# gabeur/mmt

Measured on AMD Instinct MI355X. Metric: video-text pairs/sec (fwd+bwd+Adam), MSRVTT 7-expert d512 L4, higher is better.
Workload: dtype bf16; 1 GPU; configs[1]: MSRVTT jsfusion shape, 7 experts x 30 tokens, d512, L4, H4, I3072, batch 32/GPU, dropout 0.1, train mode, Adam; text tower replaced by synthetic (B,768) vectors; global_batch=32, seq_len=218, parallelism=dp1, hip_graphs=True, inputs=resident in HBM, input_slots=8, input_format=dense fp32 dict, text_tower=synthetic, grad_sync=single, grad_wire_dtype=fp32, grad_algo=allreduce, comm_log=False, collectives_captured=False, dense_rows=6976, full=False

## Files before the change

### include/mmt_hip.h

```cpp
#ifndef MMT_HIP_H_
#define MMT_HIP_H_
#include <stdint.h>

#ifdef __cplusplus
extern "C" {
#endif

#define MMT_ABI_VERSION 6
#define MMT_ROW_ALIGN 256

#define MMT_ERR_ARG (-1)
#define MMT_ERR_ALIGN (-2)

int mmt_abi_version(void);
const char* mmt_build_info(void);

enum {
  MMT_EPI_BF16 = 0,
  MMT_EPI_BIAS_BF16 = 1,
  MMT_EPI_BIAS_GELU = 2,
  MMT_EPI_BIAS_DROP_RES = 3,
  MMT_EPI_DGELU = 4,
  MMT_EPI_ADD_F32 = 5,
  MMT_EPI_F32 = 6,
// ... 95 lines not shown
                           uint32_t drop_key, uint32_t thr16, float drop_scale, const uint32_t* seed_dev,
                           const int32_t* sched_cu, int sched_B, int sched_H, int sched_tiles, int32_t* sched_work,
                           void* stream);
int mmt_ln_fwd_scatter(const float* z, const float* gamma, const float* beta, float eps, float* h32,
                       const int32_t* dst_rows, void* h16, float* mean, float* rstd, int rows, int d, void* stream);
int mmt_rows_gather(const float* src, const int32_t* rows, int n, int d, float* dst, const int32_t* idx_in,
                    int32_t* idx_out, void* stream);
int mmt_rows_scatter(const float* src, const int32_t* rows, int n, int d, float* dst, int accumulate, void* stream);
int mmt_table_grad_direct(const float* g, const int32_t* ids, int rows, int d, int vocab, const int32_t* n_rows_dev,
                          float* dtable, void* stream);
int mmt_embedding_grad(const float* g, const int32_t* ids, int n, int d, int vocab, int padding_idx,
                       const int32_t* n_rows_dev, float* dtable, void* stream);
int mmt_text_plan(const int64_t* input_ids, const int64_t* token_type_ids, const int64_t* position_ids,
                  const int64_t* attention_mask, int B, int W, int32_t* counts, int32_t* cu_seqlens, int32_t* n_rows_dev,
                  int32_t* ids, int32_t* types, int32_t* pos, int32_t* row_index, int32_t* cls_rows, void* stream);
int mmt_gemm_splitk_geometry(int M, int N, int K, int splits_requested, int* splits, int64_t* slab_stride);
int mmt_splitk_ln_fwd(const float* slabs, int splits, int64_t slab_stride, const float* bias, const float* res,
                      const int32_t* res_rows, const int32_t* rowidx, const int32_t* row_index, int32_t* rowidx_out,
                      uint32_t drop_key, uint32_t thr16, float drop_scale, const uint32_t* seed_dev, float* z_out,
                      const float* gamma, const float* beta, float eps, float* h32, void* h16, float* mean, float* rstd,
                      int rows, int d, void* stream);
int mmt_ln_bwd_slabs(const float* slabs, int splits, int64_t slab_stride, const float* res, const float* z,
                     const float* mean, const float* rstd, const float* gamma, float* dz, void* dy, float* partials,
                     int rows, int d, int drop_mode, const int32_t* row_index, uint32_t drop_key, uint32_t thr16,
                     float drop_scale, const uint32_t* seed_dev, void* stream);
int mmt_splitk_ln_fwd_ex(const float* slabs, int splits, int64_t slab_stride, const float* bias, const float* res,
                         const int32_t* res_rows, const int32_t* rowidx, const int32_t* row_index, int32_t* rowidx_out,
                         uint32_t drop_key, uint32_t thr16, float drop_scale, const uint32_t* seed_dev, float* z_out,
                         const float* gamma, const float* beta, float eps, float* h32, void* h16, float* mean, float* rstd,
                         int rows, int d, const int32_t* n_rows_dev, void* stream);
int mmt_ln_bwd_slabs_ex(const float* slabs, int splits, int64_t slab_stride, const float* res, const float* z,
                        const float* mean, const float* rstd, const float* gamma, float* dz, void* dy, float* partials,
                        int rows, int d, int drop_mode, const int32_t* n_rows_dev, const int32_t* row_index,
                        uint32_t drop_key, uint32_t thr16, float drop_scale, const uint32_t* seed_dev, void* stream);

int mmt_ln_bwd_rows_per_block(int rows);
int mmt_ln_bwd(const float* dout, const float* z, const float* mean, const float* rstd, const float* gamma,
               float* dz, void* dy, float* partials, int rows, int d, int drop_mode,
               const int32_t* n_rows_dev, const int32_t* row_index, uint32_t drop_key, uint32_t thr16,
               float drop_scale, const uint32_t* seed_dev, void* stream);
int mmt_col_reduce(const float* partials, int nblocks, int nvec, int d, float* out0, float* out1,
                   float* out2, float* out3, int accumulate, void* stream);
#define MMT_COLRED_MAX 32
typedef struct MmtColReduceJob {
  const float* partials;
  float* out[4];
  int32_t nblocks, nvec, nout, d;
} MmtColReduceJob;
int mmt_col_reduce_multi(const MmtColReduceJob* jobs, int n, void* stream);
int64_t mmt_table_grad_scratch_floats(int vocab, int d);
int mmt_table_grad(const float* g, const int32_t* ids, int rows, int d, int vocab,
                   const int32_t* n_rows_dev, float* scratch, float* dtable, int accumulate, void* stream);
int mmt_table_grad_partials(const float* g, const int32_t* ids, int rows, int d, int vocab,
                            const int32_t* n_rows_dev, float* scratch, void* stream);
int mmt_table_grad_partials_pair(const float* g, const int32_t* ids0, int vocab0, float* scratch0, const int32_t* ids1,
                                 int vocab1, float* scratch1, int rows, int d, const int32_t* n_rows_dev, void* stream);
int mmt_table_grad_chunks(void);
int mmt_colsum_bf16(const void* x, int64_t ld, int rows, int cols, const int32_t* n_rows_dev,
                    float* partials, void* stream);

int mmt_attn_fwd(const void* qkv, const int32_t* cu_seqlens, const float* mask_bias, void* ctx, float* lse,
                 int B, int S, int H, int d, float scale, uint32_t drop_key, uint32_t thr16,
                 float drop_scale, const uint32_t* seed_dev,
                 const int32_t* row_index, void* stream);
int mmt_attn_bwd_ex(const void* qkv, const int32_t* cu_seqlens, const float* mask_bias, const void* ctx,
                    const float* lse, const void* dctx, void* dqkv, float* delta, int delta_ready, int B, int S, int H,
                    int d, float scale, uint32_t drop_key, uint32_t thr16, float drop_scale,
                    const uint32_t* seed_dev, const int32_t* row_index, const int32_t* work, void* stream);
int64_t mmt_attn_schedule_words(int B, int S, int H);
int mmt_attn_schedule(const int32_t* cu_seqlens, int B, int S, int H, int32_t* work, void* stream);
int mmt_attn_bwd(const void* qkv, const int32_t* cu_seqlens, const float* mask_bias, const void* ctx,
                 const float* lse, const void* dctx, void* dqkv, float* delta, int B, int S, int H, int d,
                 float scale, uint32_t drop_key, uint32_t thr16, float drop_scale,
                 const uint32_t* seed_dev,
                 const int32_t* row_index, void* stream);
int mmt_attn_fwd_rows(const void* qkv, const int32_t* cu_seqlens, const float* mask_bias, const int32_t* qsel, int nq,
                      void* ctx, float* lse, int B, int S, int H, int d, float scale, uint32_t drop_key, uint32_t thr16,
                      float drop_scale, const uint32_t* seed_dev,
                 const int32_t* row_index, void* stream);
int mmt_attn_bwd_rows_ex(const void* qkv, const int32_t* cu_seqlens, const float* mask_bias, const int32_t* qsel, int nq,
                         const void* ctx, const float* lse, const void* dctx, void* dqkv, float* delta, int delta_ready,
                         int B, int S, int H, int d, float scale, uint32_t drop_key, uint32_t thr16, float drop_scale,
                         const uint32_t* seed_dev, const int32_t* row_index, void* stream);
int mmt_attn_bwd_rows(const void* qkv, const int32_t* cu_seqlens, const float* mask_bias, const int32_t* qsel, int nq,
                      const void* ctx, const float* lse, const void* dctx, void* dqkv, float* delta, int B, int S, int H,
                      int d, float scale, uint32_t drop_key, uint32_t thr16, float drop_scale,
                      const uint32_t* seed_dev,
                 const int32_t* row_index, void* stream);
int mmt_attn_dropout_mask(uint8_t* out, int B, int H, int S, uint32_t drop_key, uint32_t thr16,
                          const uint32_t* seed_dev, void* stream);

#define MMT_PACK_MAX 24
typedef struct MmtPackItem {
  const float* src;
  void* dst;
  void* dst_t;
  int32_t rows, cols, dst_ld, dst_t_ld, dst_t_rows, reserved;
} MmtPackItem;
int mmt_pack_weights(const MmtPackItem* items, int n, void* stream);
int mmt_adam_step(float* params, const float* grads, float* exp_avg, float* exp_avg_sq, int64_t count,
                  float lr, float beta1, float beta2, float eps, float weight_decay,
                  const int32_t* step_dev, const float* lr_dev, void* stream);

#define MMT_ADAM_SEG_MAX 160
typedef struct MmtAdamSeg {
  int64_t offset, count;
  void* dst;
  void* dst_t;
  int32_t rows, cols, dst_ld, dst_t_ld;
} MmtAdamSeg;
int mmt_adam_fused_blocks(const MmtAdamSeg* seg);
int mmt_adam_step_fused(float* params, const float* grads, float* exp_avg, float* exp_avg_sq,
                        const MmtAdamSeg* segs_host, const MmtAdamSeg* segs_dev, int n_segs, float lr, float beta1,
                        float beta2, float eps, float weight_decay, int32_t* step_dev, const float* lr_dev,
                        int bump_step, void* stream);

#define MMT_MAX_EXPERTS 16
typedef struct MmtExpertIO {
  const float* feat;
  const float* maxpool;
  const float* ind;
  const float* t;
  void* x;
  float* y;
  void* dy;
  int32_t D, Dpad, type_idx, rows_pad;
  const float* y_part[2];
  int32_t n_part, reserved;
} MmtExpertIO;
typedef struct MmtVideoSrc {
  int32_t* src_row;
  int32_t* src_cnt;
  int32_t* xsrc;
} MmtVideoSrc;
int mmt_video_plan(const MmtExpertIO* experts, int M, int B, int T, int pack, int max_pos, int32_t* counts,
                   int32_t* cu_seqlens, int32_t* n_rows_dev, int32_t* slot, int32_t* row_index, int32_t* type_ids,
                   int32_t* pos_ids, float* mask_bias, int32_t* agg_row, uint32_t* seed_bump, const MmtVideoSrc* src,
                   void* stream);
int mmt_video_cast(const MmtExpertIO* experts, int M, int B, int T, const MmtVideoSrc* src, void* stream);
int mmt_video_scatter(const MmtExpertIO* experts, int M, int B, int T, int d, const int32_t* n_rows_dev,
                      const int32_t* row_index, const MmtVideoSrc* src, float* features, void* stream);
int mmt_video_scatter_bwd(const MmtExpertIO* experts, int M, int B, int T, int d, const int32_t* n_rows_dev,
                          const int32_t* row_index, const MmtVideoSrc* src, const float* dfeatures, void* stream);

int mmt_readout_fwd(const float* last_hidden, const int32_t* agg_row, int BM, int d, float* vid_embds,
                    float* inv_norm, void* stream);
int mmt_readout_bwd(const float* vid_embds, const float* inv_norm, const float* dvid_embds,
                    const int32_t* agg_row, int BM, int d, float* dlast_hidden, void* stream);
int mmt_sims_fwd(const float* txt, const float* vid, const float* tw, const float* vw, int NT, int NV, int M,
                 int d, float* sims, float* dots, void* stream);
int mmt_sims_bwd(const float* txt, const float* vid, const float* tw, const float* vw, float* dots,
                 const float* dsims, int NT, int NV, int M, int d, float* dtxt, float* dvid, float* dtw,
                 float* dvw, void* stream);
int mmt_simloss_small_max_n(void);
int mmt_simloss_bwd_small(const float* txt, const float* vid, const float* tw, const float* vw, const float* sims,
                          const float* dots, int n, int M, int d, int kind, float margin, int fix_norm, float* loss,
                          float* dtxt, float* dvid, float* dtw, float* dvw, const float* inv_norm,
                          const int32_t* out_rows, float* dlast, void* stream);

int mmt_maxmargin(const float* sims, int n, float margin, int fix_norm, float* partial, float* loss,
                  float* grad, void* stream);
int mmt_infonce(const float* sims, int n, float* scratch, float* loss, float* grad, void* stream);

int64_t mmt_sims_eval_workspace_floats(int NT, int NV, int M, int d);
int mmt_sims_eval(const float* txt, const float* vid, const float* tw, const float* vw, int NT, int NV, int M, int d,
                  float* ws, float* sims, void* stream);
int mmt_retrieval_ranks(const float* sims, const uint8_t* qmask, int NQ, int NV, float* t2v_rank, float* v2t_rank,
                        float* scratch, void* stream);

int mmt_search_fold(const float* x, const float* w, int N, int M, int d, float* out, void* stream);
int mmt_search_fold_bf16(const float* x, const float* w, int N, int M, int d, uint16_t* out, void* stream);
int mmt_search_fold_split_bf16(const float* x, const float* w, int N, int M, int d, uint16_t* hi, uint16_t* lo,
                               void* stream);
int mmt_search_fold_fp8(const float* x, const float* w, int N, int M, int d, uint8_t* out, float* scale, void* stream);
int mmt_rows_topk(const float* sims, int64_t ld, const int32_t* rows, int NR, int NV, int k, uint64_t* ws, float* scores,
                  int64_t* index, void* stream);

#define MMT_SEARCH_FP32 0
#define MMT_SEARCH_BF16 1
#define MMT_SEARCH_FP8 2
#define MMT_SEARCH_SETS_NONE 0
#define MMT_SEARCH_SETS_QUERY 1
#define MMT_SEARCH_SETS_ITEM 2
typedef struct MmtSearchScan {
  const void* q;
  const void* q_lo;
  const float* qw;
  const void* g;
  const float* gw;
  const float* gscale;
  const uint32_t* subset;
  const int64_t* exclude;
  const uint64_t* after;
  const float* lse;
  const float* set_weights;
  int32_t storage;
  int32_t NQ;
  int32_t NV;
  int32_t M;
  int32_t d;
  int32_t E;
  float beta;
  int32_t sets;
  int32_t set_size;
  int32_t mode;
} MmtSearchScan;
#ifdef __cplusplus
static_assert(sizeof(MmtSearchScan) == 128, "MmtSearchScan: 11 pointers, then 10 four-byte fields");
#else
_Static_assert(sizeof(MmtSearchScan) == 128, "MmtSearchScan: 11 pointers, then 10 four-byte fields");
#endif

int64_t mmt_topk_workspace_keys(int NQ, int NV, int k);
int64_t mmt_rank_workspace_ints(int NQ, int NV, int T);
int64_t mmt_count_workspace_ints(int NQ, int NV, int T);
int64_t mmt_range_workspace_ints(int NQ, int NV);
int64_t mmt_col_lse_workspace_floats(int NB, int NV);
int64_t mmt_rescore_workspace_keys(int NQ, int C);
int64_t mmt_topk_pooled_workspace_keys(int NS, int C, int NV, int k);
int64_t mmt_count_pooled_workspace_ints(int NS, int C, int NV, int T);
int64_t mmt_topk_itemsets_workspace_keys(int NQ, int NT, int C, int k);
int64_t mmt_count_itemsets_workspace_ints(int NQ, int NT, int C, int T);
int mmt_search_topk(const MmtSearchScan* scan, int k, uint64_t* ws, float* scores, int64_t* index, void* stream);
int mmt_search_topk_groups(const MmtSearchScan* scan, int k, const int32_t* group_ids, uint64_t* ws, float* scores,
                           int64_t* groups, int64_t* items, void* stream);
int mmt_search_rank(const MmtSearchScan* scan, const int64_t* targets, int T, int32_t* ws, int32_t* greater,
                    int32_t* equal, void* stream);
int mmt_search_thresholds(const MmtSearchScan* scan, const int64_t* targets, int T, float* thr, void* stream);
int mmt_search_count(const MmtSearchScan* scan, const float* thr, int T, int32_t* ws, int32_t* greater, int32_t* equal,
                     void* stream);
int mmt_search_range_count(const MmtSearchScan* scan, const float* thr, int32_t* ws, int64_t* row_counts, void* stream);
int mmt_search_range_fill(const MmtSearchScan* scan, const float* thr, const int32_t* ws, const int64_t* offsets,
                          int64_t* indices, float* scores, void* stream);
int mmt_search_rescore(const MmtSearchScan* scan, const int64_t* candidates, int C, int k, uint64_t* ws, float* scores,
                       int64_t* index, void* stream);
int mmt_search_col_lse(const MmtSearchScan* scan, float beta, float* ws, float* state, int first, float* lse,
                       void* stream);

#define MMT_SEARCH_MAX_RK 32
int64_t mmt_col_topk_workspace_keys(int NB, int NV, int k);
int mmt_search_col_topk(const MmtSearchScan* scan, int k, int row0, uint64_t* ws, uint64_t* state, int first,
                        float* scores, int64_t* rows, float* mean, float mean_weight, void* stream);

#define MMT_SEARCH_MAX_DC 128
int mmt_search_pair_scores(const void* g, const float* gw, const float* gscale, int storage, int NV, int M, int d,
                           const int64_t* items, int R, int C, float* sims, void* stream);
int mmt_search_mmr(const int64_t* items, const float* rel, const float* sims, int R, int C, int k, float a, float b,
                   float* scores, int64_t* index, float* values, void* stream);

int64_t mmt_self_topk_workspace_keys(int R, int NV, int k);
int64_t mmt_self_range_workspace_ints(int R, int NV);
int mmt_search_self_topk(const void* a_rows, const float* a_weights, const float* a_scales, int NA, const int64_t* items,
                         const int64_t* self, int R, const void* g, const float* gw, const float* gscale, int NV,
                         const uint32_t* subset, int storage, int M, int d, int k, uint64_t* ws, float* scores,
                         int64_t* index, void* stream);
int mmt_search_self_range_count(const void* a_rows, const float* a_weights, const float* a_scales, int NA,
                                const int64_t* items, const int64_t* self, int R, const void* g, const float* gw,
                                const float* gscale, int NV, const uint32_t* subset, int storage, int M, int d,
                                const float* thr, int32_t* ws, int64_t* row_counts, void* stream);
int mmt_search_self_range_fill(const void* a_rows, const float* a_weights, const float* a_scales, int NA,
                               const int64_t* items, const int64_t* self, int R, const void* g, const float* gw,
                               const float* gscale, int NV, const uint32_t* subset, int storage, int M, int d,
                               const float* thr, const int32_t* ws, const int64_t* offsets, int64_t* indices, float* scores,
                               void* stream);

int64_t mmt_row_expsum_workspace_ints64(int NQ, int NV);
int mmt_search_row_expsum(const MmtSearchScan* scan, float beta, const float* xmax, int F, int64_t* ws, void* stream);

int mmt_search_subset_pack(const uint8_t* mask, int NV, uint32_t* words, void* stream);
int mmt_search_after_keys(const float* scores, const int64_t* first, int NQ, uint64_t* keys, void* stream);
int mmt_search_merge_lists(const float* scores, const int64_t* index, const int64_t* const* ids, int S, int NQ, int kin,
                           int kout, float* out_scores, int64_t* out_index, void* stream);
int mmt_search_merge_group_lists(const float* scores, const int64_t* groups, const int64_t* index, const int64_t* const* ids,
                                 int S, int NQ, int kin, int kout, float* out_scores, int64_t* out_groups, int64_t* out_items,
                                 void* stream);

int mmt_ls_fold_bf16(const float* x, const float* w, int R, int Rpad, int M, int d, void* out16, void* stream);
int mmt_transpose_bf16(const void* src, int64_t ld_src, int rows, int cols, void* dst, int64_t ld_dst, void* stream);
int mmt_ls_finish(float* S, int64_t ld, const float* tw, const float* vw, int b, int n, int M, void* stream);
int mmt_ls_col_blocks(int n);
int mmt_ls_diag(const float* S, int64_t ld, const float* tw, const float* vw, int b, int n, int M, int r0, float* diag_local,
                void* stream);
int mmt_ls_counts_ex(float* S, int64_t ld, const float* diag, const float* tw, const float* vw, const float* vw_t, int M, int finish, int b, int n,
                     int r0, float margin, int32_t* rowcnt, int32_t* colcnt, float* loss_part, void* stream);
int mmt_ls_counts(const float* S, int64_t ld, const float* diag, int b, int n, int r0, float margin, int32_t* rowcnt,
                  int32_t* colcnt, float* loss_part, void* stream);
int mmt_ls_grad(const float* S, int64_t ld, const float* diag, const float* tw, const float* vw, const int32_t* rowcnt,
                const int32_t* colcnt_total, int b, int n, int M, int r0, float margin, float inv_norm, void* G16,
                int64_t ldg, float* gs_part, void* stream);
int mmt_ls_grad_ex(const float* S, int64_t ld, const float* diag, const float* tw, const float* vw, const float* vw_t, const int32_t* rowcnt,
                   const int32_t* colcnt_total, int b, int n, int M, int r0, float margin, float inv_norm, void* G16,
                   int64_t ldg, float* gs_part, int raw, void* stream);
int mmt_ls_unfold(const float* P, int64_t ldp, const float* x, const float* w, const float* gsub, int R, int M, int d,
                  float* dx, float* dw, void* stream);

int mmt_ls_nce_col_blocks(int n);
int mmt_ls_nce_row_groups(int b);
int mmt_ls_nce_stats(const float* S, int64_t ld, const float* tw, const float* vw, const float* vw_t, int b, int n, int M, int r0,
                     float scale, float* row_part, float* col_part, void* stream);
int mmt_ls_nce_grad(const float* S, int64_t ld, const float* tw, const float* vw, const float* vw_t, const float* row_lse,
                    const float* col_lse, int b, int n, int M, int r0, float scale, float inv_n, void* G16, int64_t ldg,
                    float* gs_part, void* stream);

typedef struct MmtSgemm {
  const float* A[MMT_MAX_EXPERTS];
  const float* B[MMT_MAX_EXPERTS];
  float* C[MMT_MAX_EXPERTS];
  const float* bias[MMT_MAX_EXPERTS];
  int64_t sai, sak, sbj, sbk, ldc;
  int32_t batch, M, N, K;
  float beta;
  int32_t reserved;
} MmtSgemm;
int mmt_sgemm_batched(const MmtSgemm* g, void* stream);

typedef struct MmtTextHeads {
  const float *w1[MMT_MAX_EXPERTS], *b1[MMT_MAX_EXPERTS];
  const float *w2[MMT_MAX_EXPERTS], *b2[MMT_MAX_EXPERTS];
  const float *bn_gamma[MMT_MAX_EXPERTS], *bn_beta[MMT_MAX_EXPERTS];
  float *running_mean[MMT_MAX_EXPERTS], *running_var[MMT_MAX_EXPERTS];
  const float *moe_w[MMT_MAX_EXPERTS], *moe_b[MMT_MAX_EXPERTS];
  float *g_w1[MMT_MAX_EXPERTS], *g_b1[MMT_MAX_EXPERTS], *g_w2[MMT_MAX_EXPERTS], *g_b2[MMT_MAX_EXPERTS];
  float *g_bn_gamma[MMT_MAX_EXPERTS], *g_bn_beta[MMT_MAX_EXPERTS], *g_moe_w[MMT_MAX_EXPERTS], *g_moe_b[MMT_MAX_EXPERTS];
} MmtTextHeads;
int64_t mmt_text_heads_workspace_floats(int N, int M, int d);
typedef struct MmtVideoFront {
  const MmtExpertIO* experts;
  int32_t M, B, T, pack, max_pos, do_cast;
  int32_t *counts, *cu_seqlens, *n_rows_dev, *slot, *row_index, *type_ids, *pos_ids;
  float* mask_bias;
  int32_t* agg_row;
  uint32_t* seed_bump;
  const MmtVideoSrc* src;
} MmtVideoFront;
typedef struct MmtTextHeadsOpts {
  uint32_t moe_drop_key, moe_drop_thr16;
  float moe_drop_scale;
  int32_t reserved;
  const uint32_t* seed_dev;
  uint32_t* key_dev;
  int64_t* num_batches_tracked;
  const MmtVideoFront* video_front;
} MmtTextHeadsOpts;
int mmt_text_heads_fast(int N, int M, int d, int K);
int mmt_text_heads_fwd(const MmtTextHeads* h, const float* text, const float* text_moe, int N, int C, int M, int d,
                       int K, int use_bn, int training, float* ws, float* text_embds, float* text_weights,
                       const MmtTextHeadsOpts* opts, void* stream);
int mmt_text_heads_bwd(const MmtTextHeads* h, const float* text, const float* text_moe, const float* w1_all, int N,
                       int C, int M, int d, int K, int use_bn, int training, float* ws, const float* dtext_embds,
                       const float* text_weights, const float* dtext_weights, float* dtext, float* dtext_moe,
                       const MmtTextHeadsOpts* opts, void* stream);

typedef struct MmtBertLayer {
  const void *wqkv, *wqkv_t, *wo, *wo_t, *w1, *w1_t, *w2, *w2_t;
  const float *bqkv, *bo, *ln1_g, *ln1_b, *b1, *b2, *ln2_g, *ln2_b;
  float *g_wqkv, *g_bqkv, *g_wo, *g_bo, *g_ln1_g, *g_ln1_b, *g_w1, *g_b1, *g_w2, *g_b2, *g_ln2_g, *g_ln2_b;
} MmtBertLayer;

typedef struct MmtBertModel {
  int32_t hidden, layers, heads, inter, max_pos, type_vocab;
  float ln_eps, p_hidden, p_attn;
  int32_t reserved;
  const float *pos_emb, *type_emb, *emb_ln_g, *emb_ln_b;
  float *g_pos_emb, *g_type_emb, *g_emb_ln_g, *g_emb_ln_b;
  const MmtBertLayer* layer;
} MmtBertModel;

typedef struct MmtBertBatch {
  const float* features;
  const int32_t* type_ids;
  const int32_t* pos_ids;
  const float* mask_bias;
  const int32_t* cu_seqlens;
  const int32_t* row_index;
  const int32_t* n_rows_dev;
  const uint32_t* seed_dev;
  int32_t rows, rows_alloc, batch, seq;
  const int32_t* out_rows;
  int32_t n_out_per_sample;
  int32_t fork;
  void* side_stream;
  int32_t live_rows_hint;
} MmtBertBatch;

enum {
  MMT_FORK_WGRAD = 1,
  MMT_FORK_EARLY = 2,
  MMT_FORK_REDUCE = 4,
  MMT_FORK_JOIN = 8,
  MMT_RANGE_LAYERS_ONLY = 16
};

int mmt_stream_fork(void* from, void* to);

int64_t mmt_bert_workspace_bytes(const MmtBertModel* m, int rows_alloc);
int mmt_bert_tail_capacity(int rows_alloc);
int mmt_bert_forward(const MmtBertModel* m, const MmtBertBatch* b, void* ws, float* out_last, int training,
                     void* stream);
int mmt_bert_backward(const MmtBertModel* m, const MmtBertBatch* b, void* ws, float* dlast, float* dfeatures,
                      int training, void* stream);
int mmt_bert_backward_range(const MmtBertModel* m, const MmtBertBatch* b, void* ws, float* dlast, float* dfeatures,
                            int training, int l_hi, int l_lo, void* stream);

int mmt_probe_arm(void** start_events, void** stop_events, int n);
int mmt_probe_arm_site(int site, void** start_events, void** stop_events, int n);
int mmt_probe_count_site(int site);
int mmt_dropout_f32(const float* x, float* y, int64_t n, uint32_t drop_key, uint32_t thr16, float scale,
                    const uint32_t* seed_dev, uint32_t* key_save, const uint32_t* key_load, void* stream);
int mmt_debug_dispatch_probe(int blocks, int threads, int lds_bytes, int spin, float* sink, void* stream);
int mmt_probe_count(void);

#ifdef __cplusplus
}
#endif
#endif
```

### mmt_amd/_lib.py

```python
import ctypes
import os

_HERE = os.path.dirname(os.path.abspath(__file__))
LIB_PATH = os.environ.get('MMT_HIP_LIB') or os.path.join(_HERE, 'lib', 'libmmt_hip.so')

c_int, c_i64, c_u32, c_f32, c_vp = ctypes.c_int, ctypes.c_int64, ctypes.c_uint32, ctypes.c_float, ctypes.c_void_p


class MmtEpilogue(ctypes.Structure):
  _fields_ = [('bias', c_vp), ('res', c_vp), ('ldres', c_i64), ('out2', c_vp), ('ldout2', c_i64),
              ('aux', c_vp), ('ldaux', c_i64), ('colsum', c_vp), ('row_index', c_vp), ('seed_dev', c_vp),
              ('drop_key', c_u32), ('drop_thr16', c_u32), ('drop_scale', c_f32), ('reserved', ctypes.c_int32),
              ('dot_src', c_vp), ('lddot', c_i64), ('dot_out', c_vp), ('live_rows_hint', ctypes.c_int32)]


class MmtPackItem(ctypes.Structure):
  _fields_ = [('src', c_vp), ('dst', c_vp), ('dst_t', c_vp), ('rows', ctypes.c_int32), ('cols', ctypes.c_int32),
              ('dst_ld', ctypes.c_int32), ('dst_t_ld', ctypes.c_int32), ('dst_t_rows', ctypes.c_int32),
              ('reserved', ctypes.c_int32)]


class MmtAdamSeg(ctypes.Structure):
  _fields_ = [('offset', c_i64), ('count', c_i64), ('dst', c_vp), ('dst_t', c_vp), ('rows', ctypes.c_int32),
              ('cols', ctypes.c_int32), ('dst_ld', ctypes.c_int32), ('dst_t_ld', ctypes.c_int32)]


class MmtGemmItem(ctypes.Structure):
  _fields_ = [('A', c_vp), ('B', c_vp), ('C', c_vp), ('bias', c_vp), ('lda', c_i64), ('ldb', c_i64), ('ldc', c_i64),
              ('M', ctypes.c_int32), ('N', ctypes.c_int32), ('K', ctypes.c_int32), ('tile_begin', ctypes.c_int32),
              ('n_rows_dev', c_vp)]


class MmtWgradItem(ctypes.Structure):
  _fields_ = [('A', c_vp), ('B', c_vp), ('out', c_vp), ('bias_out', c_vp), ('lda', c_i64), ('ldb', c_i64), ('ldo', c_i64),
              ('N', ctypes.c_int32), ('K2', ctypes.c_int32), ('N_out', ctypes.c_int32), ('K2_out', ctypes.c_int32),
              ('tile_begin', ctypes.c_int32), ('reserved', ctypes.c_int32), ('slab', c_vp), ('bias_slab', c_vp),
              ('splits', ctypes.c_int32), ('reserved2', ctypes.c_int32), ('n_rows_dev', c_vp)]


class MmtWgradGroup(ctypes.Structure):
  _fields_ = [('item', MmtWgradItem * 16), ('n_rows_dev', c_vp), ('count', ctypes.c_int32), ('rows', ctypes.c_int32)]


class MmtColReduceJob(ctypes.Structure):
  _fields_ = [('partials', c_vp), ('out', c_vp * 4), ('nblocks', ctypes.c_int32), ('nvec', ctypes.c_int32),
              ('nout', ctypes.c_int32), ('d', ctypes.c_int32)]


class MmtVideoSrc(ctypes.Structure):
  _fields_ = [('src_row', c_vp), ('src_cnt', c_vp), ('xsrc', c_vp)]


class MmtExpertIO(ctypes.Structure):
  _fields_ = [('feat', c_vp), ('maxpool', c_vp), ('ind', c_vp), ('t', c_vp), ('x', c_vp), ('y', c_vp), ('dy', c_vp),
              ('D', ctypes.c_int32), ('Dpad', ctypes.c_int32), ('type_idx', ctypes.c_int32),
              ('rows_pad', ctypes.c_int32), ('y_part', c_vp * 2), ('n_part', ctypes.c_int32),
              ('reserved', ctypes.c_int32)]


_LAYER_PTRS = ['wqkv', 'wqkv_t', 'wo', 'wo_t', 'w1', 'w1_t', 'w2', 'w2_t',
               'bqkv', 'bo', 'ln1_g', 'ln1_b', 'b1', 'b2', 'ln2_g', 'ln2_b',
               'g_wqkv', 'g_bqkv', 'g_wo', 'g_bo', 'g_ln1_g', 'g_ln1_b', 'g_w1', 'g_b1', 'g_w2', 'g_b2',
               'g_ln2_g', 'g_ln2_b']


class MmtBertLayer(ctypes.Structure):
  _fields_ = [(n, c_vp) for n in _LAYER_PTRS]


class MmtBertModel(ctypes.Structure):
  _fields_ = ([(n, ctypes.c_int32) for n in ('hidden', 'layers', 'heads', 'inter', 'max_pos', 'type_vocab')] +
              [(n, c_f32) for n in ('ln_eps', 'p_hidden', 'p_attn')] + [('reserved', ctypes.c_int32)] +
              [(n, c_vp) for n in ('pos_emb', 'type_emb', 'emb_ln_g', 'emb_ln_b', 'g_pos_emb', 'g_type_emb',
                                   'g_emb_ln_g', 'g_emb_ln_b')] +
              [('layer', ctypes.POINTER(MmtBertLayer))])


class MmtBertBatch(ctypes.Structure):
  _fields_ = ([(n, c_vp) for n in ('features', 'type_ids', 'pos_ids', 'mask_bias', 'cu_seqlens', 'row_index',
                                   'n_rows_dev', 'seed_dev')] +
              [(n, ctypes.c_int32) for n in ('rows', 'rows_alloc', 'batch', 'seq')] +
              [('out_rows', c_vp), ('n_out_per_sample', ctypes.c_int32), ('fork', ctypes.c_int32),
               ('side_stream', c_vp), ('live_rows_hint', ctypes.c_int32)])


FORK_WGRAD, FORK_EARLY, FORK_REDUCE, FORK_JOIN, RANGE_LAYERS_ONLY = 1, 2, 4, 8, 16


_PTR16 = c_vp * 16


class MmtSgemm(ctypes.Structure):
  _fields_ = [('A', _PTR16), ('B', _PTR16), ('C', _PTR16), ('bias', _PTR16),
              ('sai', c_i64), ('sak', c_i64), ('sbj', c_i64), ('sbk', c_i64), ('ldc', c_i64),
              ('batch', ctypes.c_int32), ('M', ctypes.c_int32), ('N', ctypes.c_int32), ('K', ctypes.c_int32),
              ('beta', c_f32), ('reserved', ctypes.c_int32)]


_TEXT_HEAD_FIELDS = ['w1', 'b1', 'w2', 'b2', 'bn_gamma', 'bn_beta', 'running_mean', 'running_var', 'moe_w', 'moe_b',
                     'g_w1', 'g_b1', 'g_w2', 'g_b2', 'g_bn_gamma', 'g_bn_beta', 'g_moe_w', 'g_moe_b']


class MmtTextHeads(ctypes.Structure):
  _fields_ = [(n, _PTR16) for n in _TEXT_HEAD_FIELDS]


class MmtVideoFront(ctypes.Structure):
  _fields_ = [('experts', c_vp), ('M', ctypes.c_int32), ('B', ctypes.c_int32), ('T', ctypes.c_int32), ('pack', ctypes.c_int32),
              ('max_pos', ctypes.c_int32), ('do_cast', ctypes.c_int32), ('counts', c_vp), ('cu_seqlens', c_vp),
              ('n_rows_dev', c_vp), ('slot', c_vp), ('row_index', c_vp), ('type_ids', c_vp), ('pos_ids', c_vp),
              ('mask_bias', c_vp), ('agg_row', c_vp), ('seed_bump', c_vp), ('src', c_vp)]


class MmtTextHeadsOpts(ctypes.Structure):
  _fields_ = [('moe_drop_key', c_u32), ('moe_drop_thr16', c_u32), ('moe_drop_scale', c_f32), ('reserved', ctypes.c_int32),
              ('seed_dev', c_vp), ('key_dev', c_vp), ('num_batches_tracked', c_vp), ('video_front', c_vp)]


class MmtSearchScan(ctypes.Structure):
  _fields_ = ([(n, c_vp) for n in ('q', 'q_lo', 'qw', 'g', 'gw', 'gscale', 'subset', 'exclude', 'after', 'lse',
                                   'set_weights')] +
              [(n, ctypes.c_int32) for n in ('storage', 'NQ', 'NV', 'M', 'd', 'E')] + [('beta', c_f32)] +
              [(n, ctypes.c_int32) for n in ('sets', 'set_size', 'mode')])


SEARCH_FP32, SEARCH_BF16, SEARCH_FP8 = 0, 1, 2
SEARCH_SETS_NONE, SEARCH_SETS_QUERY, SEARCH_SETS_ITEM = 0, 1, 2
_SCAN = ctypes.POINTER(MmtSearchScan)

EPI = dict(BF16=0, BIAS_BF16=1, BIAS_GELU=2, BIAS_DROP_RES=3, DGELU=4, ADD_F32=5, F32=6, BIAS_F32=7)

SIGNATURES = {
    'mmt_abi_version': (c_int, []),
    'mmt_build_info': (ctypes.c_char_p, []),
    'mmt_gemm_nt_bf16': (c_int, [c_vp, c_i64, c_vp, c_i64, c_vp, c_i64, c_int, c_int, c_int, c_int,
                                 ctypes.POINTER(MmtEpilogue), c_vp, c_vp]),
    'mmt_gemm_select_tile': (c_int, [c_int] * 9),
    'mmt_gemm_tn_bf16': (c_int, [c_vp, c_i64, c_vp, c_i64, c_vp, c_int, c_int, c_int, c_int, c_vp, c_vp]),
    'mmt_gemm_nt_splitk_workspace_floats': (c_i64, [c_int, c_int, c_int]),
    'mmt_gemm_nt_splitk': (c_int, [c_vp, c_i64, c_vp, c_i64, c_vp, c_i64, c_int, c_int, c_int, c_int,
                                   ctypes.POINTER(MmtEpilogue), c_vp, c_vp]),
    'mmt_gemm_nn_bf16': (c_int, [c_vp, c_i64, c_vp, c_i64, c_vp, c_i64, c_int, c_int, c_int, c_int,
                                 ctypes.POINTER(MmtEpilogue), c_vp, c_vp]),
    'mmt_gemm_nn_splitk_ex': (c_int, [c_vp, c_i64, c_vp, c_i64, c_vp, c_i64, c_int, c_int, c_int, c_int,
                                      ctypes.POINTER(MmtEpilogue), c_vp, c_int, c_int, c_vp, c_int, c_vp]),
    'mmt_gemm_nt_splitk_ex': (c_int, [c_vp, c_i64, c_vp, c_i64, c_vp, c_i64, c_int, c_int, c_int, c_int,
                                      ctypes.POINTER(MmtEpilogue), c_vp, c_int, c_int, c_vp, c_int, c_vp]),
    'mmt_gemm_nt_grouped': (c_int, [ctypes.POINTER(MmtGemmItem), c_int, c_int, c_vp]),
    'mmt_wgrad_grouped': (c_int, [ctypes.POINTER(MmtWgradGroup), c_vp]),
    'mmt_reduce_slabs': (c_int, [c_vp, c_int, c_i64, c_vp, c_int, c_vp]),
    'mmt_reduce_slabs_pair': (c_int, [c_vp, c_i64, c_vp, c_vp, c_i64, c_vp, c_int, c_vp]),
    'mmt_ln_fwd': (c_int, [c_vp, c_vp, c_vp, c_f32, c_vp, c_vp, c_vp, c_vp, c_int, c_int, c_vp, c_vp]),
    'mmt_embed_ln_fwd': (c_int, [c_vp, c_vp, c_vp, c_vp, c_vp, c_vp, c_vp, c_vp, c_f32, c_vp, c_vp, c_vp, c_vp,
                                 c_int, c_int, c_vp, c_vp, c_u32, c_u32, c_f32, c_vp, c_vp]),
    'mmt_embed_ln_fwd_sched': (c_int, [c_vp, c_vp, c_vp, c_vp, c_vp, c_vp, c_vp, c_vp, c_f32, c_vp, c_vp, c_vp, c_vp,
                                 c_int, c_int, c_vp, c_vp, c_u32, c_u32, c_f32, c_vp, c_vp, c_int, c_int, c_int, c_vp, c_vp]),
    'mmt_ln_bwd_rows_per_block': (c_int, [c_int]),
    'mmt_gemm_splitk_geometry': (c_int, [c_int, c_int, c_int, c_int, c_vp, c_vp]),
    'mmt_splitk_ln_fwd': (c_int, [c_vp, c_int, c_i64, c_vp, c_vp, c_vp, c_vp, c_vp, c_vp, c_u32, c_u32, c_f32, c_vp, c_vp, c_vp,
                                  c_vp, c_f32, c_vp, c_vp, c_vp, c_vp, c_int, c_int, c_vp]),
    'mmt_ln_bwd_slabs': (c_int, [c_vp, c_int, c_i64, c_vp, c_vp, c_vp, c_vp, c_vp, c_vp, c_vp, c_vp, c_int, c_int, c_int, c_vp,
                                 c_u32, c_u32, c_f32, c_vp, c_vp]),
    'mmt_splitk_ln_fwd_ex': (c_int, [c_vp, c_int, c_i64, c_vp, c_vp, c_vp, c_vp, c_vp, c_vp, c_u32, c_u32, c_f32, c_vp, c_vp, c_vp,
                                     c_vp, c_f32, c_vp, c_vp, c_vp, c_vp, c_int, c_int, c_vp, c_vp]),
    'mmt_ln_bwd_slabs_ex': (c_int, [c_vp, c_int, c_i64, c_vp, c_vp, c_vp, c_vp, c_vp, c_vp, c_vp, c_vp, c_int, c_int, c_int, c_vp,
                                    c_vp, c_u32, c_u32, c_f32, c_vp, c_vp]),
    'mmt_ln_bwd': (c_int, [c_vp, c_vp, c_vp, c_vp, c_vp, c_vp, c_vp, c_vp, c_int, c_int, c_int, c_vp, c_vp,
                           c_u32, c_u32, c_f32, c_vp, c_vp]),
    'mmt_col_reduce': (c_int, [c_vp, c_int, c_int, c_int, c_vp, c_vp, c_vp, c_vp, c_int, c_vp]),
    'mmt_col_reduce_multi': (c_int, [ctypes.POINTER(MmtColReduceJob), c_int, c_vp]),
    'mmt_table_grad_partials': (c_int, [c_vp, c_vp, c_int, c_int, c_int, c_vp, c_vp, c_vp]),
    'mmt_table_grad_chunks': (c_int, []),
    'mmt_table_grad_partials_pair': (c_int, [c_vp, c_vp, c_int, c_vp, c_vp, c_int, c_vp, c_int, c_int, c_vp, c_vp]),
    'mmt_table_grad_scratch_floats': (c_i64, [c_int, c_int]),
    'mmt_table_grad': (c_int, [c_vp, c_vp, c_int, c_int, c_int, c_vp, c_vp, c_vp, c_int, c_vp]),
    'mmt_attn_fwd': (c_int, [c_vp, c_vp, c_vp, c_vp, c_vp, c_int, c_int, c_int, c_int, c_f32, c_u32, c_u32,
                             c_f32, c_vp, c_vp, c_vp]),
    'mmt_attn_bwd': (c_int, [c_vp, c_vp, c_vp, c_vp, c_vp, c_vp, c_vp, c_vp, c_int, c_int, c_int, c_int, c_f32,
                             c_u32, c_u32, c_f32, c_vp, c_vp, c_vp]),
    'mmt_attn_bwd_ex': (c_int, [c_vp, c_vp, c_vp, c_vp, c_vp, c_vp, c_vp, c_vp, c_int, c_int, c_int, c_int, c_int, c_f32,
                                c_u32, c_u32, c_f32, c_vp, c_vp, c_vp, c_vp]),
    'mmt_attn_schedule_words': (c_i64, [c_int, c_int, c_int]),
    'mmt_attn_schedule': (c_int, [c_vp, c_int, c_int, c_int, c_vp, c_vp]),
    'mmt_attn_bwd_rows_ex': (c_int, [c_vp, c_vp, c_vp, c_vp, c_int, c_vp, c_vp, c_vp, c_vp, c_vp, c_int, c_int, c_int, c_int,
                                     c_int, c_f32, c_u32, c_u32, c_f32, c_vp, c_vp, c_vp]),
    'mmt_attn_fwd_rows': (c_int, [c_vp, c_vp, c_vp, c_vp, c_int, c_vp, c_vp, c_int, c_int, c_int, c_int, c_f32, c_u32, c_u32,
                                  c_f32, c_vp, c_vp, c_vp]),
    'mmt_attn_bwd_rows': (c_int, [c_vp, c_vp, c_vp, c_vp, c_int, c_vp, c_vp, c_vp, c_vp, c_vp, c_int, c_int, c_int, c_int,
                                  c_f32, c_u32, c_u32, c_f32, c_vp, c_vp, c_vp]),
    'mmt_ln_fwd_scatter': (c_int, [c_vp, c_vp, c_vp, c_f32, c_vp, c_vp, c_vp, c_vp, c_vp, c_int, c_int, c_vp]),
    'mmt_rows_gather': (c_int, [c_vp, c_vp, c_int, c_int, c_vp, c_vp, c_vp, c_vp]),
    'mmt_rows_scatter': (c_int, [c_vp, c_vp, c_int, c_int, c_vp, c_int, c_vp]),
    'mmt_embedding_grad': (c_int, [c_vp, c_vp, c_int, c_int, c_int, c_int, c_vp, c_vp, c_vp]),
    'mmt_text_plan': (c_int, [c_vp, c_vp, c_vp, c_vp, c_int, c_int, c_vp, c_vp, c_vp, c_vp, c_vp, c_vp, c_vp, c_vp, c_vp]),
    'mmt_table_grad_direct': (c_int, [c_vp, c_vp, c_int, c_int, c_int, c_vp, c_vp, c_vp]),
    'mmt_attn_dropout_mask': (c_int, [c_vp, c_int, c_int, c_int, c_u32, c_u32, c_vp, c_vp]),
    'mmt_reduce_slabs_2d': (c_int, [c_vp, c_int, c_int, c_int, c_int, c_vp, c_int, c_vp]),
    'mmt_colsum_bf16': (c_int, [c_vp, c_i64, c_int, c_int, c_vp, c_vp, c_vp]),
    'mmt_pack_weights': (c_int, [ctypes.POINTER(MmtPackItem), c_int, c_vp]),
    'mmt_dropout_f32': (c_int, [c_vp, c_vp, c_i64, c_u32, c_u32, c_f32, c_vp, c_vp, c_vp, c_vp]),
    'mmt_debug_dispatch_probe': (c_int, [c_int, c_int, c_int, c_int, c_vp, c_vp]),
    'mmt_adam_step': (c_int, [c_vp, c_vp, c_vp, c_vp, c_i64, c_f32, c_f32, c_f32, c_f32, c_f32, c_vp, c_vp, c_vp]),
    'mmt_adam_fused_blocks': (c_int, [ctypes.POINTER(MmtAdamSeg)]),
    'mmt_adam_step_fused': (c_int, [c_vp, c_vp, c_vp, c_vp, ctypes.POINTER(MmtAdamSeg), c_vp, c_int, c_f32, c_f32, c_f32,
                                    c_f32, c_f32, c_vp, c_vp, c_int, c_vp]),
    'mmt_video_plan': (c_int, [ctypes.POINTER(MmtExpertIO), c_int, c_int, c_int, c_int, c_int, c_vp, c_vp, c_vp, c_vp,
                               c_vp, c_vp, c_vp, c_vp, c_vp, c_vp, ctypes.POINTER(MmtVideoSrc), c_vp]),
    'mmt_video_cast': (c_int, [ctypes.POINTER(MmtExpertIO), c_int, c_int, c_int, ctypes.POINTER(MmtVideoSrc), c_vp]),
    'mmt_video_scatter': (c_int, [ctypes.POINTER(MmtExpertIO), c_int, c_int, c_int, c_int, c_vp, c_vp,
                                  ctypes.POINTER(MmtVideoSrc), c_vp, c_vp]),
    'mmt_video_scatter_bwd': (c_int, [ctypes.POINTER(MmtExpertIO), c_int, c_int, c_int, c_int, c_vp, c_vp,
                                      ctypes.POINTER(MmtVideoSrc), c_vp, c_vp]),
    'mmt_readout_fwd': (c_int, [c_vp, c_vp, c_int, c_int, c_vp, c_vp, c_vp]),
    'mmt_readout_bwd': (c_int, [c_vp, c_vp, c_vp, c_vp, c_int, c_int, c_vp, c_vp]),
    'mmt_sims_fwd': (c_int, [c_vp, c_vp, c_vp, c_vp, c_int, c_int, c_int, c_int, c_vp, c_vp, c_vp]),
    'mmt_sims_bwd': (c_int, [c_vp, c_vp, c_vp, c_vp, c_vp, c_vp, c_int, c_int, c_int, c_int, c_vp, c_vp, c_vp, c_vp,
                             c_vp]),
    'mmt_sims_eval_workspace_floats': (c_i64, [c_int, c_int, c_int, c_int]),
    'mmt_sims_eval': (c_int, [c_vp, c_vp, c_vp, c_vp, c_int, c_int, c_int, c_int, c_vp, c_vp, c_vp]),
    'mmt_retrieval_ranks': (c_int, [c_vp, c_vp, c_int, c_int, c_vp, c_vp, c_vp, c_vp]),
    'mmt_search_fold': (c_int, [c_vp, c_vp, c_int, c_int, c_int, c_vp, c_vp]),
    'mmt_topk_workspace_keys': (c_i64, [c_int, c_int, c_int]),
    'mmt_rows_topk': (c_int, [c_vp, c_i64, c_vp, c_int, c_int, c_int, c_vp, c_vp, c_vp, c_vp]),
    'mmt_search_fold_bf16': (c_int, [c_vp, c_vp, c_int, c_int, c_int, c_vp, c_vp]),
    'mmt_search_fold_split_bf16': (c_int, [c_vp, c_vp, c_int, c_int, c_int, c_vp, c_vp, c_vp]),
    'mmt_rank_workspace_ints': (c_i64, [c_int, c_int, c_int]),
    'mmt_search_subset_pack': (c_int, [c_vp, c_int, c_vp, c_vp]),
    'mmt_count_workspace_ints': (c_i64, [c_int, c_int, c_int]),
    'mmt_search_merge_lists': (c_int, [c_vp, c_vp, c_vp, c_int, c_int, c_int, c_int, c_vp, c_vp, c_vp]),
    'mmt_col_lse_workspace_floats': (c_i64, [c_int, c_int]),
    'mmt_range_workspace_ints': (c_i64, [c_int, c_int]),
    'mmt_search_fold_fp8': (c_int, [c_vp, c_vp, c_int, c_int, c_int, c_vp, c_vp, c_vp]),
    'mmt_search_merge_group_lists': (c_int, [c_vp, c_vp, c_vp, c_vp, c_int, c_int, c_int, c_int, c_vp, c_vp, c_vp, c_vp]),
    'mmt_topk_pooled_workspace_keys': (c_i64, [c_int, c_int, c_int, c_int]),
    'mmt_count_pooled_workspace_ints': (c_i64, [c_int, c_int, c_int, c_int]),
    'mmt_topk_itemsets_workspace_keys': (c_i64, [c_int, c_int, c_int, c_int]),
    'mmt_count_itemsets_workspace_ints': (c_i64, [c_int, c_int, c_int, c_int]),
    'mmt_rescore_workspace_keys': (c_i64, [c_int, c_int]),
    'mmt_search_after_keys': (c_int, [c_vp, c_vp, c_int, c_vp, c_vp]),
    'mmt_search_topk': (c_int, [_SCAN, c_int, c_vp, c_vp, c_vp, c_vp]),
    'mmt_search_topk_groups': (c_int, [_SCAN, c_int, c_vp, c_vp, c_vp, c_vp, c_vp, c_vp]),
    'mmt_search_rank': (c_int, [_SCAN, c_vp, c_int, c_vp, c_vp, c_vp, c_vp]),
    'mmt_search_thresholds': (c_int, [_SCAN, c_vp, c_int, c_vp, c_vp]),
    'mmt_search_count': (c_int, [_SCAN, c_vp, c_int, c_vp, c_vp, c_vp, c_vp]),
    'mmt_search_range_count': (c_int, [_SCAN, c_vp, c_vp, c_vp, c_vp]),
    'mmt_search_range_fill': (c_int, [_SCAN, c_vp, c_vp, c_vp, c_vp, c_vp, c_vp]),
    'mmt_search_rescore': (c_int, [_SCAN, c_vp, c_int, c_int, c_vp, c_vp, c_vp, c_vp]),
    'mmt_search_col_lse': (c_int, [_SCAN, c_f32, c_vp, c_vp, c_int, c_vp, c_vp]),
    'mmt_col_topk_workspace_keys': (c_i64, [c_int, c_int, c_int]),
    'mmt_search_col_topk': (c_int, [_SCAN, c_int, c_int, c_vp, c_vp, c_int, c_vp, c_vp, c_vp, c_f32, c_vp]),
    'mmt_search_pair_scores': (c_int, [c_vp, c_vp, c_vp, c_int, c_int, c_int, c_int, c_vp, c_int, c_int, c_vp, c_vp]),
    'mmt_search_mmr': (c_int, [c_vp, c_vp, c_vp, c_int, c_int, c_int, c_f32, c_f32, c_vp, c_vp, c_vp, c_vp]),
    'mmt_self_topk_workspace_keys': (c_i64, [c_int, c_int, c_int]),
    'mmt_self_range_workspace_ints': (c_i64, [c_int, c_int]),
    'mmt_search_self_topk': (c_int, [c_vp, c_vp, c_vp, c_int, c_vp, c_vp, c_int, c_vp, c_vp, c_vp, c_int, c_vp, c_int, c_int,
                                     c_int, c_int, c_vp, c_vp, c_vp, c_vp]),
    'mmt_search_self_range_count': (c_int, [c_vp, c_vp, c_vp, c_int, c_vp, c_vp, c_int, c_vp, c_vp, c_vp, c_int, c_vp, c_int,
                                            c_int, c_int, c_vp, c_vp, c_vp, c_vp]),
    'mmt_search_self_range_fill': (c_int, [c_vp, c_vp, c_vp, c_int, c_vp, c_vp, c_int, c_vp, c_vp, c_vp, c_int, c_vp, c_int,
                                           c_int, c_int, c_vp, c_vp, c_vp, c_vp, c_vp, c_vp]),
    'mmt_row_expsum_workspace_ints64': (c_i64, [c_int, c_int]),
    'mmt_search_row_expsum': (c_int, [_SCAN, c_f32, c_vp, c_int, c_vp, c_vp]),
    'mmt_ls_fold_bf16': (c_int, [c_vp, c_vp, c_int, c_int, c_int, c_int, c_vp, c_vp]),
    'mmt_transpose_bf16': (c_int, [c_vp, c_i64, c_int, c_int, c_vp, c_i64, c_vp]),
    'mmt_ls_finish': (c_int, [c_vp, c_i64, c_vp, c_vp, c_int, c_int, c_int, c_vp]),
    'mmt_ls_col_blocks': (c_int, [c_int]),
    'mmt_ls_diag': (c_int, [c_vp, c_i64, c_vp, c_vp, c_int, c_int, c_int, c_int, c_vp, c_vp]),
    'mmt_ls_counts_ex': (c_int, [c_vp, c_i64, c_vp, c_vp, c_vp, c_vp, c_int, c_int, c_int, c_int, c_int, c_f32, c_vp, c_vp, c_vp, c_vp]),
    'mmt_ls_counts': (c_int, [c_vp, c_i64, c_vp, c_int, c_int, c_int, c_f32, c_vp, c_vp, c_vp, c_vp]),
    'mmt_ls_grad': (c_int, [c_vp, c_i64, c_vp, c_vp, c_vp, c_vp, c_vp, c_int, c_int, c_int, c_int, c_f32, c_f32, c_vp, c_i64,
                            c_vp, c_vp]),
    'mmt_ls_grad_ex': (c_int, [c_vp, c_i64, c_vp, c_vp, c_vp, c_vp, c_vp, c_vp, c_int, c_int, c_int, c_int, c_f32, c_f32, c_vp, c_i64,
                            c_vp, c_int, c_vp]),
    'mmt_ls_unfold': (c_int, [c_vp, c_i64, c_vp, c_vp, c_vp, c_int, c_int, c_int, c_vp, c_vp, c_vp]),
    'mmt_ls_nce_col_blocks': (c_int, [c_int]),
    'mmt_ls_nce_row_groups': (c_int, [c_int]),
    'mmt_ls_nce_stats': (c_int, [c_vp, c_i64, c_vp, c_vp, c_vp, c_int, c_int, c_int, c_int, c_f32, c_vp, c_vp, c_vp]),
    'mmt_ls_nce_grad': (c_int, [c_vp, c_i64, c_vp, c_vp, c_vp, c_vp, c_vp, c_int, c_int, c_int, c_int, c_f32, c_f32, c_vp, c_i64,
                                c_vp, c_vp]),
    'mmt_simloss_small_max_n': (c_int, []),
    'mmt_simloss_bwd_small': (c_int, [c_vp, c_vp, c_vp, c_vp, c_vp, c_vp, c_int, c_int, c_int, c_int, c_f32, c_int, c_vp, c_vp,
                                      c_vp, c_vp, c_vp, c_vp, c_vp, c_vp, c_vp]),
    'mmt_maxmargin': (c_int, [c_vp, c_int, c_f32, c_int, c_vp, c_vp, c_vp, c_vp]),
    'mmt_infonce': (c_int, [c_vp, c_int, c_vp, c_vp, c_vp, c_vp]),
    'mmt_bert_tail_capacity': (c_int, [c_int]),
    'mmt_bert_workspace_bytes': (c_i64, [ctypes.POINTER(MmtBertModel), c_int]),
    'mmt_bert_forward': (c_int, [ctypes.POINTER(MmtBertModel), ctypes.POINTER(MmtBertBatch), c_vp, c_vp, c_int, c_vp]),
    'mmt_bert_backward': (c_int, [ctypes.POINTER(MmtBertModel), ctypes.POINTER(MmtBertBatch), c_vp, c_vp, c_vp, c_int,
                                  c_vp]),
    'mmt_bert_backward_range': (c_int, [ctypes.POINTER(MmtBertModel), ctypes.POINTER(MmtBertBatch), c_vp, c_vp, c_vp,
                                        c_int, c_int, c_int, c_vp]),
    'mmt_stream_fork': (c_int, [c_vp, c_vp]),
    'mmt_sgemm_batched': (c_int, [ctypes.POINTER(MmtSgemm), c_vp]),
    'mmt_text_heads_workspace_floats': (c_i64, [c_int, c_int, c_int]),
    'mmt_text_heads_fast': (c_int, [c_int, c_int, c_int, c_int]),
    'mmt_text_heads_fwd': (c_int, [ctypes.POINTER(MmtTextHeads), c_vp, c_vp, c_int, c_int, c_int, c_int, c_int, c_int,
                                   c_int, c_vp, c_vp, c_vp, ctypes.POINTER(MmtTextHeadsOpts), c_vp]),
    'mmt_text_heads_bwd': (c_int, [ctypes.POINTER(MmtTextHeads), c_vp, c_vp, c_vp, c_int, c_int, c_int, c_int, c_int,
                                   c_int, c_int, c_vp, c_vp, c_vp, c_vp, c_vp, c_vp, ctypes.POINTER(MmtTextHeadsOpts),
                                   c_vp]),
    'mmt_probe_arm': (c_int, [c_vp, c_vp, c_int]),
    'mmt_probe_count': (c_int, []),
    'mmt_probe_arm_site': (c_int, [c_int, c_vp, c_vp, c_int]),
    'mmt_probe_count_site': (c_int, [c_int]),
}

_lib = None


def lib():
  global _lib
  if _lib is None:
    if not os.path.exists(LIB_PATH):
      raise RuntimeError(
          'libmmt_hip.so is missing (%s): run `python -m mmt_amd.build` (hipcc, gfx950). '
          'There is no CPU fallback for the MMT hot path.' % LIB_PATH)
    handle = ctypes.CDLL(LIB_PATH)
    for name, (res, args) in SIGNATURES.items():
      fn = getattr(handle, name)
      fn.restype = res
      fn.argtypes = args
    if handle.mmt_abi_version() != 6:
      raise RuntimeError('libmmt_hip.so ABI mismatch')
    _lib = handle
  return _lib


def check(rc, what):
  if rc != 0:
    raise RuntimeError('%s failed with code %d' % (what, rc))
```

### mmt_amd/csrc/simloss.hip

```cpp
#include "mmt_common.h"
#include "../../include/mmt_hip.h"

#define MAXM MMT_MAX_EXPERTS

__global__ __launch_bounds__(256) void readout_fwd_kernel(const float* __restrict__ last, const int32_t* __restrict__ agg_row,
                                                          int BM, int d, float* __restrict__ out, float* __restrict__ inv_norm) {
  const int lane = threadIdx.x & 63, wave = threadIdx.x >> 6;
  for (int i = blockIdx.x * 4 + wave; i < BM; i += gridDim.x * 4) {
    const float* src = last + (int64_t)agg_row[i] * d;
    float ss = 0.f;
    for (int c = lane * 4; c < d; c += 256) {
      const f32x4 v = *(const f32x4*)(src + c);
      ss += v[0] * v[0] + v[1] * v[1] + v[2] * v[2] + v[3] * v[3];
    }
    const float inv = 1.0f / fmaxf(sqrtf(wave_sum(ss)), 1e-12f);
    for (int c = lane * 4; c < d; c += 256) *(f32x4*)(out + (int64_t)i * d + c) = *(const f32x4*)(src + c) * inv;
    if (lane == 0) inv_norm[i] = inv;
  }
}

__global__ __launch_bounds__(256) void readout_bwd_kernel(const float* __restrict__ emb, const float* __restrict__ inv_norm,
                                                          const float* __restrict__ demb, const int32_t* __restrict__ agg_row,
                                                          int BM, int d, float* __restrict__ dlast) {
  const int lane = threadIdx.x & 63, wave = threadIdx.x >> 6;
  for (int i = blockIdx.x * 4 + wave; i < BM; i += gridDim.x * 4) {
    float dot = 0.f;
    for (int c = lane * 4; c < d; c += 256) {
      const f32x4 y = *(const f32x4*)(emb + (int64_t)i * d + c), g = *(const f32x4*)(demb + (int64_t)i * d + c);
      dot += y[0] * g[0] + y[1] * g[1] + y[2] * g[2] + y[3] * g[3];
    }
    dot = wave_sum(dot);
    const float inv = inv_norm[i];
    float* dst = dlast + (int64_t)agg_row[i] * d;
    for (int c = lane * 4; c < d; c += 256) {
      const f32x4 y = *(const f32x4*)(emb + (int64_t)i * d + c), g = *(const f32x4*)(demb + (int64_t)i * d + c);
      *(f32x4*)(dst + c) = (g - y * dot) * inv;
    }
  }
}

__global__ __launch_bounds__(256) void sims_fwd_kernel(const float* __restrict__ txt, const float* __restrict__ vid,
                                                       const float* __restrict__ tw, const float* __restrict__ vw, int NT,
                                                       int NV, int M, int d, float* __restrict__ sims,
                                                       float* __restrict__ dots) {
  extern __shared__ __attribute__((aligned(16))) float ts[];
  const int t = blockIdx.x, lane = threadIdx.x & 63, wave = threadIdx.x >> 6;
  for (int i = threadIdx.x * 4; i < M * d; i += 1024) *(f32x4*)(ts + i) = *(const f32x4*)(txt + (int64_t)t * M * d + i);
  __syncthreads();
  for (int v = blockIdx.y * 4 + wave; v < NV; v += gridDim.y * 4) {
    float nrm = 0.f;
    for (int m = 0; m < M; ++m) nrm += tw[t * M + m] * vw[v * M + m];
    if (nrm == 0.f) nrm = 1e-5f;
    float s = 0.f;
    for (int m = 0; m < M; ++m) {
      float acc = 0.f;
      for (int c = lane * 4; c < d; c += 256) {
        const f32x4 x = *(const f32x4*)(ts + m * d + c), y = *(const f32x4*)(vid + ((int64_t)v * M + m) * d + c);
        acc += x[0] * y[0] + x[1] * y[1] + x[2] * y[2] + x[3] * y[3];
      }
      const float dm = wave_sum(acc);
      s += tw[t * M + m] * vw[v * M + m] / nrm * dm;
      if (lane == 0) dots[((int64_t)t * NV + v) * M + m] = dm;
    }
    if (lane == 0) sims[(int64_t)t * NV + v] = s;
  }
}

#define SF_WAVES 16
#define SF_VCHUNK 8
__global__ __launch_bounds__(64 * SF_WAVES) void sims_fwd_small_kernel(const float* __restrict__ txt, const float* __restrict__ vid,
                                                                       const float* __restrict__ tw, const float* __restrict__ vw,
                                                                       int NT, int NV, int M, int d, float* __restrict__ sims,
                                                                       float* __restrict__ dots) {
  extern __shared__ __attribute__((aligned(16))) float ts[];
  float* drow = ts + M * d;
  const int t = blockIdx.x, v0 = blockIdx.y * SF_VCHUNK, lane = threadIdx.x & 63, wave = threadIdx.x >> 6;
  const int nv = min(SF_VCHUNK, NV - v0);
  for (int i = threadIdx.x * 4; i < M * d; i += 256 * SF_WAVES) *(f32x4*)(ts + i) = *(const f32x4*)(txt + (int64_t)t * M * d + i);
  __syncthreads();
  const int npair = nv * M;
  for (int p = wave; p < npair; p += 2 * SF_WAVES) {
    const int p1 = p + SF_WAVES;
    const bool two = p1 < npair;
    const int m0 = p % M, m1 = two ? p1 % M : 0;
    const float* y0 = vid + ((int64_t)v0 * M + p) * d;
    const float* y1 = vid + ((int64_t)v0 * M + (two ? p1 : p)) * d;
    float a0 = 0.f, a1 = 0.f;
    for (int c = lane * 4; c < d; c += 256) {
      const f32x4 u0 = *(const f32x4*)(y0 + c), u1 = *(const f32x4*)(y1 + c);
      const f32x4 x0 = *(const f32x4*)(ts + m0 * d + c), x1 = *(const f32x4*)(ts + m1 * d + c);
      a0 += x0[0] * u0[0] + x0[1] * u0[1] + x0[2] * u0[2] + x0[3] * u0[3];
      a1 += x1[0] * u1[0] + x1[1] * u1[1] + x1[2] * u1[2] + x1[3] * u1[3];
    }
#pragma unroll
    for (int o = 32; o > 0; o >>= 1) { a0 += __shfl_xor(a0, o, 64); a1 += __shfl_xor(a1, o, 64); }
    if (lane == 0) {
      drow[p] = a0;
      dots[((int64_t)t * NV + v0) * M + p] = a0;
      if (two) { drow[p1] = a1; dots[((int64_t)t * NV + v0) * M + p1] = a1; }
    }
  }
  __syncthreads();
  if ((int)threadIdx.x < nv) {
    const int v = v0 + threadIdx.x;
    float nrm = 0.f, sacc = 0.f;
    for (int m = 0; m < M; ++m) nrm += tw[t * M + m] * vw[v * M + m];
    if (nrm == 0.f) nrm = 1e-5f;
    for (int m = 0; m < M; ++m) sacc += tw[t * M + m] * vw[v * M + m] / nrm * drow[threadIdx.x * M + m];
    sims[(int64_t)t * NV + v] = sacc;
  }
}

#define SB_WAVES 8
struct SimLossArgs {
  const float *txt, *vid, *tw, *vw, *sims, *dots;
  int n, M, d, kind, fix_norm;
  float margin;
  float *loss, *dtxt, *dvid, *dtw, *dvw;
  const float* inv_norm; const int32_t* out_rows; float* dlast;
};
__global__ __launch_bounds__(64 * SB_WAVES) void simloss_bwd_small_kernel(SimLossArgs a) {
  extern __shared__ __attribute__((aligned(16))) float sl[];
  const int n = a.n, M = a.M, d = a.d;
  float* S = sl;
  float* lse_r = S + n * n;
  float* lse_c = lse_r + n;
  float* gself = lse_c + n;
  float* racc = sl + ((n * n + 3 * n + 3) & ~3) + 4;
  float* rw = racc + SB_WAVES * d;
  float* twl = rw + SB_WAVES;
  float* vwl = twl + n * M;
  const int side = blockIdx.z, self = blockIdx.x, m = blockIdx.y;
  const int tid = threadIdx.x, lane = tid & 63, wave = tid >> 6;
  for (int i = tid; i < n * n; i += 64 * SB_WAVES) S[i] = a.sims[i];
  for (int i = tid; i < n * M; i += 64 * SB_WAVES) { twl[i] = a.tw[i]; vwl[i] = a.vw[i]; }
  __syncthreads();
  const float norm = a.kind == 0 ? (a.fix_norm ? 2.0f * n * (n - 1) : 2.0f * n * n) : (float)n;
  if (a.kind == 1) {
    for (int k = tid; k < 2 * n; k += 64 * SB_WAVES) {
      const int r = k % n;
      const bool col = k >= n;
      float mx = -INFINITY;
      for (int c = 0; c < n; ++c) mx = fmaxf(mx, col ? S[c * n + r] : S[r * n + c]);
      float sum = 0.f;
      for (int c = 0; c < n; ++c) sum += expf((col ? S[c * n + r] : S[r * n + c]) - mx);
      (col ? lse_c : lse_r)[r] = mx + logf(sum);
    }
    __syncthreads();
  }
  auto g_entry = [&](int t, int v) -> float {
    const float stv = S[t * n + v];
    if (a.kind == 1) return (expf(stv - lse_r[t]) + expf(stv - lse_c[v]) - (t == v ? 2.f : 0.f)) / norm;
    if (t != v) return ((a.margin - S[t * n + t] + stv > 0.f ? 1.f : 0.f) + (a.margin - S[v * n + v] + stv > 0.f ? 1.f : 0.f)) / norm;
    int cnt = 0;
    for (int c = 0; c < n; ++c) {
      if (c == t) continue;
      cnt += (a.margin - stv + S[t * n + c] > 0.f) + (a.margin - stv + S[c * n + t] > 0.f);
    }
    return -(float)cnt / norm;
  };
  for (int o = tid; o < n; o += 64 * SB_WAVES) gself[o] = side == 0 ? g_entry(self, o) : g_entry(o, self);
  if (side == 0 && self == 0 && m == 0 && wave == 0) {
    float acc = 0.f;
    if (a.kind == 1) {
      for (int k = lane; k < n; k += 64) acc += (lse_r[k] + lse_c[k] - 2.0f * S[k * n + k]) / norm;
    } else {
      for (int e = lane; e < n * n; e += 64) {
        const int r = e / n, c = e % n;
        if (r == c && a.fix_norm) continue;
        acc += (fmaxf(a.margin - S[r * n + r] + S[e], 0.f) + fmaxf(a.margin - S[c * n + c] + S[e], 0.f)) / norm;
      }
    }
    acc = wave_sum(acc);
    if (lane == 0) *a.loss = acc;
  }
  __syncthreads();
  float* __restrict__ dx = side == 0 ? a.dtxt : a.dvid;
  float* __restrict__ dwt = side == 0 ? a.dtw : a.dvw;
  const float* other = side == 0 ? a.vid : a.txt;
  f32x4 acc[4];
#pragma unroll
  for (int c = 0; c < 4; ++c) acc[c] = (f32x4){0.f, 0.f, 0.f, 0.f};
  float dws = 0.f;
  const float* wo = side == 0 ? vwl : twl;
  for (int o0 = wave; o0 < n; o0 += 2 * SB_WAVES) {
    float coef[2];
    f32x4 rowv[2][4];
#pragma unroll
    for (int q = 0; q < 2; ++q) {
      const int o = o0 + q * SB_WAVES;
      coef[q] = 0.f;
#pragma unroll
      for (int c = 0; c < 4; ++c) rowv[q][c] = (f32x4){0.f, 0.f, 0.f, 0.f};
      if (o >= n) continue;
      const int t = side == 0 ? self : o, v = side == 0 ? o : self;
      const float g = gself[o];
      const float* dm = a.dots + ((int64_t)t * n + v) * M;
      float nrm = 0.f, gw = 0.f;
      for (int j = 0; j < M; ++j) nrm += twl[t * M + j] * vwl[v * M + j];
      const bool zero = nrm == 0.f;
      if (zero) nrm = 1e-5f;
      for (int j = 0; j < M; ++j) gw += g * dm[j] * twl[t * M + j] * vwl[v * M + j] / nrm;
      const float w = twl[t * M + m] * vwl[v * M + m] / nrm;
      const float da = zero ? g * dm[m] / nrm : (g * dm[m] - gw) / nrm;
      dws += da * wo[o * M + m];
      coef[q] = g * w;
#pragma unroll
      for (int c = 0; c < 4; ++c) {
        const int col = c * 256 + lane * 4;
        if (col < d) rowv[q][c] = *(const f32x4*)(other + ((int64_t)o * M + m) * d + col);
      }
    }
#pragma unroll
    for (int q = 0; q < 2; ++q)
#pragma unroll
      for (int c = 0; c < 4; ++c) acc[c] += rowv[q][c] * coef[q];
  }
#pragma unroll
  for (int c = 0; c < 4; ++c) {
    const int col = c * 256 + lane * 4;
    if (col < d) *(f32x4*)(racc + wave * d + col) = acc[c];
  }
  if (lane == 0) rw[wave] = dws;
  __syncthreads();
  const bool readout = side == 1 && a.dlast != nullptr;
  const int64_t row = (int64_t)self * M + m;
  float part = 0.f;
  float gx[2] = {0.f, 0.f};
#pragma unroll
  for (int u = 0; u < 2; ++u) {
    const int i = tid + u * 64 * SB_WAVES;
    if (i < d) {
      float sum = 0.f;
#pragma unroll
      for (int w = 0; w < SB_WAVES; ++w) sum += racc[w * d + i];
      if (dx) dx[row * d + i] = sum;
      if (readout) part += sum * a.vid[row * d + i];
      gx[u] = sum;
    }
  }
  if (tid == 0 && dwt) {
    float sum = 0.f;
    for (int w = 0; w < SB_WAVES; ++w) sum += rw[w];
    dwt[self * M + m] = sum;
  }
  if (readout) {
    part = wave_sum(part);
    __syncthreads();
    if (lane == 0) racc[wave] = part;
    __syncthreads();
    float dot = 0.f;
    for (int w = 0; w < SB_WAVES; ++w) dot += racc[w];
// ... 111 lines not shown
  }
#pragma unroll
  for (int m = 0; m < MAXM; ++m) {
    const float r = wave_sum(acc[m]);
    if (lane == 0) red[wave][m] = r;
  }
  __syncthreads();
  if (threadIdx.x < M) dw[self * M + threadIdx.x] = red[0][threadIdx.x] + red[1][threadIdx.x] + red[2][threadIdx.x] +
                                                    red[3][threadIdx.x];
}

static int sims_fwd_large(const float* txt, const float* vid, const float* tw, const float* vw, int NT, int NV, int M, int d,
                          float* sims, float* dots, void* stream) {
  MmtSgemm g = {};
  g.batch = M; g.M = NT; g.N = NV; g.K = d;
  g.sai = (int64_t)M * d; g.sak = 1; g.sbj = (int64_t)M * d; g.sbk = 1; g.ldc = NV;
  for (int m = 0; m < M; ++m) { g.A[m] = txt + (int64_t)m * d; g.B[m] = vid + (int64_t)m * d; g.C[m] = dots + (int64_t)m * NT * NV; }
  int rc = mmt_sgemm_batched(&g, stream);
  if (rc) return rc;
  hipLaunchKernelGGL(sims_combine_kernel, dim3((NV + 255) / 256, NT), dim3(256), 0, (hipStream_t)stream, dots, tw, vw, NT, NV,
                     M, sims);
  return (int)hipGetLastError();
}

static int sims_bwd_large(const float* txt, const float* vid, const float* tw, const float* vw, float* dots,
                          const float* dsims, int NT, int NV, int M, int d, float* dtxt, float* dvid, float* dtw,
                          float* dvw, void* stream) {
  hipStream_t s = (hipStream_t)stream;
  hipLaunchKernelGGL(sims_weights_bwd_kernel<0>, dim3(NV), dim3(256), 0, s, dots, dsims, tw, vw, NT, NV, M, dvw);
  hipLaunchKernelGGL(sims_weights_bwd_kernel<1>, dim3(NT), dim3(256), 0, s, dots, dsims, tw, vw, NT, NV, M, dtw);
  const int64_t plane = (int64_t)NT * NV;
  MmtSgemm g = {};
  g.batch = M; g.M = NT; g.N = d; g.K = NV;
  g.sai = NV; g.sak = 1; g.sbj = 1; g.sbk = (int64_t)M * d; g.ldc = (int64_t)M * d;
  for (int m = 0; m < M; ++m) { g.A[m] = dots + m * plane; g.B[m] = vid + (int64_t)m * d; g.C[m] = dtxt + (int64_t)m * d; }
  int rc = mmt_sgemm_batched(&g, stream);
  if (rc) return rc;
  g = {};
  g.batch = M; g.M = NV; g.N = d; g.K = NT;
  g.sai = 1; g.sak = NV; g.sbj = 1; g.sbk = (int64_t)M * d; g.ldc = (int64_t)M * d;
  for (int m = 0; m < M; ++m) { g.A[m] = dots + m * plane; g.B[m] = txt + (int64_t)m * d; g.C[m] = dvid + (int64_t)m * d; }
  return mmt_sgemm_batched(&g, stream);
}

__global__ __launch_bounds__(256) void maxmargin_kernel(const float* __restrict__ s, int n, float margin, int fix_norm,
                                                        float* __restrict__ partial, float* __restrict__ G) {
  __shared__ float redf[4];
  __shared__ int redi[4];
  const int k = blockIdx.x, lane = threadIdx.x & 63, wave = threadIdx.x >> 6;
  const float skk = s[(int64_t)k * n + k];
  const float norm = fix_norm ? 2.0f * n * (n - 1) : 2.0f * n * n;
  float acc = 0.f;
  int cnt = 0;
  for (int c = threadIdx.x; c < n; c += 256) {
    const bool diag = c == k;
    if (diag && fix_norm) continue;
    const float h1 = margin - skk + s[(int64_t)k * n + c];
    const float h2 = margin - skk + s[(int64_t)c * n + k];
    const float h2g = margin - s[(int64_t)c * n + c] + s[(int64_t)k * n + c];
    acc += fmaxf(h1, 0.f) + fmaxf(h2, 0.f);
    cnt += (h1 > 0.f) + (h2 > 0.f);
    if (!diag) G[(int64_t)k * n + c] = ((h1 > 0.f ? 1.f : 0.f) + (h2g > 0.f ? 1.f : 0.f)) / norm;
  }
  acc = wave_sum(acc);
  for (int o = 32; o > 0; o >>= 1) cnt += __shfl_xor(cnt, o, 64);
  if (lane == 0) { redf[wave] = acc; redi[wave] = cnt; }
  __syncthreads();
  if (threadIdx.x == 0) {
    partial[k] = (redf[0] + redf[1] + redf[2] + redf[3]) / norm;
    const int total = redi[0] + redi[1] + redi[2] + redi[3];
    const int self_terms = fix_norm ? 0 : (margin > 0.f ? 2 : 0);
    G[(int64_t)k * n + k] = -(float)(total - self_terms) / norm;
  }
}

__global__ void sum_partials_kernel(const float* __restrict__ partial, int n, float* __restrict__ out) {
  __shared__ float red[4];
  float acc = 0.f;
  for (int i = threadIdx.x; i < n; i += 256) acc += partial[i];
  acc = wave_sum(acc);
  if ((threadIdx.x & 63) == 0) red[threadIdx.x >> 6] = acc;
  __syncthreads();
  if (threadIdx.x == 0) *out = red[0] + red[1] + red[2] + red[3];
}

__global__ __launch_bounds__(256) void infonce_lse_kernel(const float* __restrict__ s, int n, float* __restrict__ lse_row,
                                                          float* __restrict__ lse_col, float* __restrict__ partial) {
  __shared__ float red[2][4];
  const int k = blockIdx.x, lane = threadIdx.x & 63, wave = threadIdx.x >> 6;
  float mr = -INFINITY, mc = -INFINITY;
  for (int c = threadIdx.x; c < n; c += 256) { mr = fmaxf(mr, s[(int64_t)k * n + c]); mc = fmaxf(mc, s[(int64_t)c * n + k]); }
  mr = wave_max(mr); mc = wave_max(mc);
  if (lane == 0) { red[0][wave] = mr; red[1][wave] = mc; }
  __syncthreads();
  mr = fmaxf(fmaxf(red[0][0], red[0][1]), fmaxf(red[0][2], red[0][3]));
  mc = fmaxf(fmaxf(red[1][0], red[1][1]), fmaxf(red[1][2], red[1][3]));
  __syncthreads();
  float sr = 0.f, sc = 0.f;
  for (int c = threadIdx.x; c < n; c += 256) { sr += expf(s[(int64_t)k * n + c] - mr); sc += expf(s[(int64_t)c * n + k] - mc); }
  sr = wave_sum(sr); sc = wave_sum(sc);
  if (lane == 0) { red[0][wave] = sr; red[1][wave] = sc; }
  __syncthreads();
  if (threadIdx.x == 0) {
    const float lr = mr + logf(red[0][0] + red[0][1] + red[0][2] + red[0][3]);
    const float lc = mc + logf(red[1][0] + red[1][1] + red[1][2] + red[1][3]);
    lse_row[k] = lr; lse_col[k] = lc;
    partial[k] = (lr + lc - 2.0f * s[(int64_t)k * n + k]) / n;
  }
}
__global__ void infonce_grad_kernel(const float* __restrict__ s, int n, const float* __restrict__ lse_row,
                                    const float* __restrict__ lse_col, float* __restrict__ G) {
  const int64_t i = blockIdx.x * (int64_t)blockDim.x + threadIdx.x;
  if (i >= (int64_t)n * n) return;
  const int r = (int)(i / n), c = (int)(i % n);
  G[i] = (expf(s[i] - lse_row[r]) + expf(s[i] - lse_col[c]) - (r == c ? 2.f : 0.f)) / n;
}

extern "C" int mmt_readout_fwd(const float* last_hidden, const int32_t* agg_row, int BM, int d, float* vid_embds,
                               float* inv_norm, void* stream) {
  if (!last_hidden || !agg_row || !vid_embds || !inv_norm || BM <= 0 || d % 4) return MMT_ERR_ARG;
  hipLaunchKernelGGL(readout_fwd_kernel, dim3((BM + 3) / 4), dim3(256), 0, (hipStream_t)stream, last_hidden, agg_row,
                     BM, d, vid_embds, inv_norm);
  return (int)hipGetLastError();
}

extern "C" int mmt_readout_bwd(const float* vid_embds, const float* inv_norm, const float* dvid_embds,
                               const int32_t* agg_row, int BM, int d, float* dlast_hidden, void* stream) {
  if (!vid_embds || !inv_norm || !dvid_embds || !agg_row || !dlast_hidden || BM <= 0 || d % 4) return MMT_ERR_ARG;
  hipLaunchKernelGGL(readout_bwd_kernel, dim3((BM + 3) / 4), dim3(256), 0, (hipStream_t)stream, vid_embds, inv_norm,
                     dvid_embds, agg_row, BM, d, dlast_hidden);
  return (int)hipGetLastError();
}

extern "C" int mmt_sims_fwd(const float* txt, const float* vid, const float* tw, const float* vw, int NT, int NV, int M,
                            int d, float* sims, float* dots, void* stream) {
  if (!txt || !vid || !tw || !vw || !sims || !dots || NT <= 0 || NV <= 0 || M <= 0 || M > MAXM || d % 4 || d > 1024)
    return MMT_ERR_ARG;
  if (NT >= LARGE_N || NV >= LARGE_N) return sims_fwd_large(txt, vid, tw, vw, NT, NV, M, d, sims, dots, stream);
  const size_t lds = (size_t)M * d * sizeof(float);
  if (lds > 64 * 1024) return MMT_ERR_ARG;
  if (lds + (size_t)SF_VCHUNK * M * sizeof(float) <= 64 * 1024) {
    hipLaunchKernelGGL(sims_fwd_small_kernel, dim3(NT, (NV + SF_VCHUNK - 1) / SF_VCHUNK), dim3(64 * SF_WAVES),
                       lds + (size_t)SF_VCHUNK * M * sizeof(float), (hipStream_t)stream, txt, vid, tw, vw, NT, NV, M, d, sims,
                       dots);
    return (int)hipGetLastError();
  }
  int gy = (NV + 3) / 4;
  if (gy > 16) gy = 16;
  hipLaunchKernelGGL(sims_fwd_kernel, dim3(NT, gy), dim3(256), lds, (hipStream_t)stream, txt, vid, tw, vw, NT, NV, M, d,
                     sims, dots);
  return (int)hipGetLastError();
}

extern "C" int mmt_simloss_small_max_n(void) { return LARGE_N - 1; }

extern "C" int mmt_simloss_bwd_small(const float* txt, const float* vid, const float* tw, const float* vw, const float* sims,
                                     const float* dots, int n, int M, int d, int kind, float margin, int fix_norm,
                                     float* loss, float* dtxt, float* dvid, float* dtw, float* dvw, const float* inv_norm,
                                     const int32_t* out_rows, float* dlast, void* stream) {
  if (!txt || !vid || !tw || !vw || !sims || !dots || !loss || n <= 1 || n >= LARGE_N || M <= 0 || M > MAXM || d % 4 ||
      d > 1024 || (kind != 0 && kind != 1))
    return MMT_ERR_ARG;
  if (dlast && !inv_norm) return MMT_ERR_ARG;
  SimLossArgs a = {txt, vid, tw, vw, sims, dots, n, M, d, kind, fix_norm, margin, loss, dtxt, dvid, dtw, dvw, inv_norm, out_rows,
                   dlast};
  const size_t lds = ((size_t)(((n * n + 3 * n + 3) & ~3) + 4) + (size_t)SB_WAVES * d + SB_WAVES + 2 * (size_t)n * M) * sizeof(float);
  static bool configured = false;
  if (!configured) {
    hipError_t rc = hipFuncSetAttribute((const void*)simloss_bwd_small_kernel, hipFuncAttributeMaxDynamicSharedMemorySize,
                                        (int)((63 * 63 + 2 * 63 + 64 + SB_WAVES * 1024 + SB_WAVES + 2 * 63 * MAXM) * sizeof(float)));
    if (rc != hipSuccess) return (int)rc;
    configured = true;
  }
  hipLaunchKernelGGL(simloss_bwd_small_kernel, dim3(n, M, 2), dim3(64 * SB_WAVES), lds, (hipStream_t)stream, a);
  return (int)hipGetLastError();
}

extern "C" int mmt_sims_bwd(const float* txt, const float* vid, const float* tw, const float* vw, float* dots,
                            const float* dsims, int NT, int NV, int M, int d, float* dtxt, float* dvid, float* dtw,
                            float* dvw, void* stream) {
  if (!txt || !vid || !tw || !vw || !dots || !dsims || !dtxt || !dvid || !dtw || !dvw) return MMT_ERR_ARG;
  if (NT <= 0 || NV <= 0 || M <= 0 || M > MAXM || d % 4 || d > 1024) return MMT_ERR_ARG;
  if (NT >= LARGE_N || NV >= LARGE_N)
    return sims_bwd_large(txt, vid, tw, vw, dots, dsims, NT, NV, M, d, dtxt, dvid, dtw, dvw, stream);
  hipLaunchKernelGGL(sims_bwd_kernel, dim3(NT > NV ? NT : NV, M, 2), dim3(256), 0, (hipStream_t)stream, txt, vid, tw, vw, dots,
                     dsims, NT, NV, M, d, dtxt, dtw, dvid, dvw);
  return (int)hipGetLastError();
}

extern "C" int mmt_maxmargin(const float* sims, int n, float margin, int fix_norm, float* partial, float* loss,
                             float* grad, void* stream) {
  if (!sims || !partial || !loss || !grad || n <= 1) return MMT_ERR_ARG;
  hipLaunchKernelGGL(maxmargin_kernel, dim3(n), dim3(256), 0, (hipStream_t)stream, sims, n, margin, fix_norm, partial,
                     grad);
  hipLaunchKernelGGL(sum_partials_kernel, dim3(1), dim3(256), 0, (hipStream_t)stream, partial, n, loss);
  return (int)hipGetLastError();
}

extern "C" int mmt_infonce(const float* sims, int n, float* scratch, float* loss, float* grad, void* stream) {
  if (!sims || !scratch || !loss || !grad || n <= 0) return MMT_ERR_ARG;
  hipLaunchKernelGGL(infonce_lse_kernel, dim3(n), dim3(256), 0, (hipStream_t)stream, sims, n, scratch, scratch + n,
                     scratch + 2 * n);
  hipLaunchKernelGGL(sum_partials_kernel, dim3(1), dim3(256), 0, (hipStream_t)stream, scratch + 2 * n, n, loss);
  const int64_t nn = (int64_t)n * n;
  hipLaunchKernelGGL(infonce_grad_kernel, dim3((unsigned)((nn + 255) / 256)), dim3(256), 0, (hipStream_t)stream, sims, n,
                     scratch, scratch + n, grad);
  return (int)hipGetLastError();
}
```

### mmt_amd/csrc/texthead2.hip

```cpp
#include "mmt_common.h"
#include "../../include/mmt_hip.h"
#include "video_front.h"

typedef __attribute__((ext_vector_type(16))) float f32x16;

#define TH_W 16
#define TH_T (64 * TH_W)
#define TH_TMAX 8

struct ThArgs {
  MmtTextHeads h;
  const float* text; const float* text_moe;
  float* ws;
  float* text_embds; float* text_weights;
  const float* de; const float* tw; const float* dtw;
  float* dtext_moe;
  int N, C, M, d, K, use_bn, training;
  uint32_t drop_key, thr16; float drop_scale;
  const uint32_t* seed_dev; uint32_t* key_dev; long long* nbt;
};

struct ThWs { float *y, *x1, *mean, *rstd, *dyg, *dz, *dlogit, *sg, *o, *part; };
__host__ __device__ inline ThWs th_layout(float* ws, int N, int M, int d) {
  const int64_t nmd = (int64_t)N * M * d, md = (int64_t)M * d;
// ... 99 lines not shown
  const int n = bid - gemm_blocks;
  unsigned key = 0;
  if (!a.text_moe && a.thr16) {
    key = eff_key(a.drop_key, a.seed_dev);
    if (n == 0 && tid == 0 && a.key_dev) *a.key_dev = key;
  }
  float* logit = sm.colv[0];
  for (int m = wave; m < a.M; m += TH_W) {
    float s = 0.f;
    for (int k4 = lane * 4; k4 < a.K; k4 += 256) {
      const f32x4 x = moe_input4(a, key, n, k4), ww = *(const f32x4*)(a.h.moe_w[m] + k4);
      s += x[0] * ww[0] + x[1] * ww[1] + x[2] * ww[2] + x[3] * ww[3];
    }
    s = wave_sum(s);
    if (lane == 0) logit[m] = s + a.h.moe_b[m][0];
  }
  __syncthreads();
  if (tid == 0) {
    float mx = -INFINITY, sum = 0.f, l1 = 0.f;
    for (int m = 0; m < a.M; ++m) mx = fmaxf(mx, logit[m]);
    for (int m = 0; m < a.M; ++m) sum += __expf(logit[m] - mx);
    for (int m = 0; m < a.M; ++m) { logit[m] = __expf(logit[m] - mx) / sum; l1 += fabsf(logit[m]); }
    for (int m = 0; m < a.M; ++m) a.text_weights[(int64_t)n * a.M + m] = logit[m] / fmaxf(l1, 1e-12f);
  }
}

__global__ __launch_bounds__(TH_T) void th_fwd1_kernel(ThArgs a) {
  extern __shared__ __attribute__((aligned(16))) unsigned char th_smem_raw[];
  th_fwd1_block(a, (int)blockIdx.x, *(ThSmem*)th_smem_raw);
}

struct CastSplit { int32_t begin[MMT_MAX_EXPERTS + 1]; };
static_assert(sizeof(ThArgs) + sizeof(VideoPlanArgs) + 64 <= 4096 && sizeof(ThArgs) + sizeof(VideoCastArgs) + sizeof(CastSplit) + 64 <= 4096,
              "kernel arguments: 4 KiB");
__global__ __launch_bounds__(TH_T) void th_fwd1_plan_kernel(ThArgs a, VideoPlanArgs p, int th_blocks) {
  extern __shared__ __attribute__((aligned(16))) unsigned char th_smem_raw[];
  if ((int)blockIdx.x < th_blocks) {
    th_fwd1_block(a, (int)blockIdx.x, *(ThSmem*)th_smem_raw);
    return;
  }
  if (threadIdx.x >= 256) return;
  video_plan_block(p, (int)blockIdx.x - th_blocks, (int)threadIdx.x, (float*)th_smem_raw);
}

__device__ __forceinline__ void th_fwd2_block(const ThArgs& a, const int bid, ThSmem& sm) {
  const int tid = threadIdx.x, lane = tid & 63, wave = tid >> 6, l31 = lane & 31, h = lane >> 5;
  const int ct = a.d / 32;
  const int m = bid / ct, jt = bid % ct, j0 = jt * 32;
  const ThWs w = th_layout(a.ws, a.N, a.M, a.d);
  if (bid == 0 && tid < a.M && a.nbt && a.use_bn && a.training) a.nbt[tid] += 1;
  const int per = k_slice(a.d), kbeg = wave * per, kend = min(a.d, kbeg + per);
  const f32x16 acc = mm_nt_slice(w.y + ((int64_t)min(l31, a.N - 1) * a.M + m) * a.d, l31 < a.N,
                                 a.h.w2[m] + (int64_t)(j0 + l31) * a.d, true, kbeg, kend, h);
  float v = splitk_reduce(sm, acc, wave, lane);
  {
    const int n = tile_row(wave, lane);
    v += a.h.b2[m][j0 + l31];
    sm.tile[0][n][l31] = n < a.N ? v : 0.f;
    if (n < a.N) w.x1[((int64_t)n * a.M + m) * a.d + j0 + l31] = v;
  }
  __syncthreads();
  if (a.use_bn) {
    const int r = tid & 31, c = tid >> 5, col = j0 + c;
    float mean, rstd;
    if (a.training) {
      const float x = r < a.N ? sm.tile[0][r][c] : 0.f;
      mean = half_wave_sum(x) / a.N;
      const float dev = r < a.N ? x - mean : 0.f;
      const float q = half_wave_sum(dev * dev);
      const float var = q / a.N;
      rstd = 1.0f / sqrtf(var + 1e-5f);
      if (r == 0 && a.h.running_mean[m]) {
        a.h.running_mean[m][col] = 0.9f * a.h.running_mean[m][col] + 0.1f * mean;
        a.h.running_var[m][col] = 0.9f * a.h.running_var[m][col] + 0.1f * (a.N > 1 ? q / (a.N - 1) : var);
      }
    } else {
      mean = a.h.running_mean[m][col];
      rstd = 1.0f / sqrtf(a.h.running_var[m][col] + 1e-5f);
    }
    if (r == 0) {
      w.mean[(int64_t)m * a.d + col] = mean;
      w.rstd[(int64_t)m * a.d + col] = rstd;
      sm.colv[0][c] = mean;
      sm.colv[1][c] = rstd;
    }
  }
  __syncthreads();
  const int n = tid >> 5, j = tid & 31, col = j0 + j;
  float o = 0.f;
  if (n < a.N) {
    float z = sm.tile[0][n][j];
    if (a.use_bn) z = (z - sm.colv[0][j]) * sm.colv[1][j] * a.h.bn_gamma[m][col] + a.h.bn_beta[m][col];
    const float sg = 1.0f / (1.0f + __expf(-z));
    const int64_t p = ((int64_t)n * a.M + m) * a.d + col;
    o = w.y[p] * sg;
    w.sg[p] = sg;
    w.o[p] = o;
  }
  float sq = o * o;
#pragma unroll
  for (int s = 16; s > 0; s >>= 1) sq += __shfl_xor(sq, s, 64);
  if (j == 0 && n < a.N) w.part[((int64_t)n * a.M + m) * ct + jt] = sq;
}

__global__ __launch_bounds__(TH_T) void th_fwd2_kernel(ThArgs a) {
  extern __shared__ __attribute__((aligned(16))) unsigned char th_smem_raw[];
  th_fwd2_block(a, (int)blockIdx.x, *(ThSmem*)th_smem_raw);
}

__global__ __launch_bounds__(TH_T) void th_fwd2_cast_kernel(ThArgs a, VideoCastArgs c, int th_blocks, CastSplit cs, int M,
                                                            uint32_t* seed_bump) {
  extern __shared__ __attribute__((aligned(16))) unsigned char th_smem_raw[];
  if (blockIdx.x == 0 && threadIdx.x == 0 && seed_bump) *seed_bump += 1u;
  if ((int)blockIdx.x < th_blocks) {
    th_fwd2_block(a, (int)blockIdx.x, *(ThSmem*)th_smem_raw);
    return;
  }
  const int r = (int)blockIdx.x - th_blocks;
  int ex = 0;
#pragma unroll 1
  for (int q = 1; q < M; ++q)
    if (r >= cs.begin[q]) ex = q;
  video_cast_block(c, ex, r - cs.begin[ex], cs.begin[ex + 1] - cs.begin[ex], (int)threadIdx.x, TH_T, 0, 2);
}

__device__ __forceinline__ void th_fwd3_block(const ThArgs& a, const int bid) {
  const int lane = threadIdx.x & 63, wave = threadIdx.x >> 6;
  const int ct = a.d / 32;
  const ThWs w = th_layout(a.ws, a.N, a.M, a.d);
  const int r = bid * 4 + wave;
  if (r >= a.N * a.M) return;
  const int n = r / a.M, m = r % a.M;
  const float ss = wave_sum(lane < ct ? w.part[(int64_t)r * ct + lane] : 0.f);
  const float inv = 1.0f / fmaxf(sqrtf(ss), 1e-12f);
  const int64_t src = (int64_t)r * a.d, dst = (((int64_t)(n / a.C) * a.M + m) * a.C + n % a.C) * a.d;
  for (int c = lane * 4; c < a.d; c += 256) *(f32x4*)(a.text_embds + dst + c) = *(const f32x4*)(w.o + src + c) * inv;
}

__global__ __launch_bounds__(256) void th_fwd3_kernel(ThArgs a) { th_fwd3_block(a, (int)blockIdx.x); }

__global__ __launch_bounds__(256) void th_fwd3_cast_kernel(ThArgs a, VideoCastArgs c, int th_blocks, CastSplit cs, int M) {
  if ((int)blockIdx.x < th_blocks) {
    th_fwd3_block(a, (int)blockIdx.x);
    return;
  }
  const int r = (int)blockIdx.x - th_blocks;
  int ex = 0;
#pragma unroll 1
  for (int q = 1; q < M; ++q)
    if (r >= cs.begin[q]) ex = q;
  video_cast_block(c, ex, r - cs.begin[ex], cs.begin[ex + 1] - cs.begin[ex], (int)threadIdx.x, 256, 1, 2);
}

__global__ __launch_bounds__(256) void th_bwd1_kernel(ThArgs a) {
  __shared__ float dl[MMT_MAX_EXPERTS];
  const int tid = threadIdx.x, lane = tid & 63, wave = tid >> 6;
  const ThWs w = th_layout(a.ws, a.N, a.M, a.d);
  const int row_blocks = (a.N * a.M + 3) / 4;
  if ((int)blockIdx.x < row_blocks) {
    const int r = blockIdx.x * 4 + wave;
    if (r >= a.N * a.M) return;
    const int n = r / a.M, m = r % a.M;
    const int64_t src = (int64_t)r * a.d, dst = (((int64_t)(n / a.C) * a.M + m) * a.C + n % a.C) * a.d;
    f32x4 o[4], g[4];
    float ss = 0.f, dot = 0.f;
#pragma unroll
    for (int c = 0; c < 4; ++c) {
      const int col = c * 256 + lane * 4;
      o[c] = g[c] = (f32x4){0.f, 0.f, 0.f, 0.f};
      if (col < a.d) {
        o[c] = *(const f32x4*)(w.o + src + col);
        g[c] = *(const f32x4*)(a.de + dst + col);
      }
#pragma unroll
      for (int k = 0; k < 4; ++k) { ss += o[c][k] * o[c][k]; dot += g[c][k] * o[c][k]; }
    }
    const float nrm = sqrtf(wave_sum(ss));
    const float inv = 1.0f / fmaxf(nrm, 1e-12f);
    const float proj = nrm > 1e-12f ? wave_sum(dot) * inv * inv : 0.f;
#pragma unroll
    for (int c = 0; c < 4; ++c) {
      const int col = c * 256 + lane * 4;
      if (col < a.d) {
        const f32x4 sg = *(const f32x4*)(w.sg + src + col), yy = *(const f32x4*)(w.y + src + col);
        f32x4 dy_, dz_;
#pragma unroll
        for (int k = 0; k < 4; ++k) {
          const float dox = (g[c][k] - o[c][k] * proj) * inv;
          dy_[k] = dox * sg[k];
          dz_[k] = dox * yy[k] * sg[k] * (1.0f - sg[k]);
        }
        *(f32x4*)(w.dyg + src + col) = dy_;
        *(f32x4*)(w.dz + src + col) = dz_;
      }
    }
    return;
  }
  const int n = blockIdx.x - row_blocks;
  if (wave == 0) {
    const float t = lane < a.M ? a.tw[(int64_t)n * a.M + lane] : 0.f, dv = lane < a.M ? a.dtw[(int64_t)n * a.M + lane] : 0.f;
    const float dot = wave_sum(t * dv);
    if (lane < a.M) {
      dl[lane] = t * (dv - dot);
      w.dlogit[(int64_t)n * a.M + lane] = dl[lane];
    }
  }
  __syncthreads();
  if (!a.dtext_moe) return;
  const unsigned key = (!a.text_moe && a.thr16 && a.key_dev) ? *a.key_dev : 0u;
  for (int k4 = tid * 4; k4 < a.K; k4 += 1024) {
    f32x4 s = {0.f, 0.f, 0.f, 0.f};
    for (int m = 0; m < a.M; ++m) s += *(const f32x4*)(a.h.moe_w[m] + k4) * dl[m];
    if (!a.text_moe && a.thr16) {
      bool kp[4];
      keep4(key, (unsigned long long)n * (unsigned)a.K + (unsigned)k4, a.thr16, kp);
#pragma unroll
      for (int e = 0; e < 4; ++e) s[e] = kp[e] ? s[e] * a.drop_scale : 0.f;
    }
    *(f32x4*)(a.dtext_moe + (int64_t)n * a.K + k4) = s;
  }
}

__device__ __forceinline__ void tn_load(float (&b)[16], const float* __restrict__ G, int64_t ldg, int N, int l31, int h) {
#pragma unroll
  for (int kk = 0; kk < 16; ++kk) {
    const int k = 2 * kk + h;
    const float g = G[(int64_t)min(k, N - 1) * ldg + l31];
    b[kk] = k < N ? g : 0.f;
  }
}
__device__ __forceinline__ f32x16 tn_mma(const float (*T)[33], const float (&b)[16], int l31, int h) {
  f32x16 acc;
#pragma unroll
  for (int r = 0; r < 16; ++r) acc[r] = 0.f;
#pragma unroll
  for (int kk = 0; kk < 16; ++kk) acc = __builtin_amdgcn_mfma_f32_32x32x2f32(T[2 * kk + h][l31], b[kk], acc, 0, 0, 0);
  return acc;
}
__device__ __forceinline__ void store_tile(const f32x16& acc, float* __restrict__ out, int64_t ldo, int l31, int h) {
#pragma unroll
  for (int r = 0; r < 16; ++r) out[(int64_t)((r & 3) + 8 * (r >> 2) + 4 * h) * ldo + l31] = acc[r];
}

__global__ __launch_bounds__(TH_T) void th_bwd2_kernel(ThArgs a) {
  extern __shared__ __attribute__((aligned(16))) unsigned char th_smem_raw[];
  ThSmem& sm = *(ThSmem*)th_smem_raw;
  const int tid = threadIdx.x, lane = tid & 63, wave = tid >> 6, l31 = lane & 31, h = lane >> 5;
  const int ct = a.d / 32;
  const int m = blockIdx.x / ct, j0 = (blockIdx.x % ct) * 32;
  const ThWs w = th_layout(a.ws, a.N, a.M, a.d);
  const int n = tid >> 5, j = tid & 31, col = j0 + j;
  const int64_t p = ((int64_t)n * a.M + m) * a.d + col;
  const bool live = n < a.N;
  const float dzv = live ? w.dz[p] : 0.f;
  float dx = dzv;
  const bool gw2 = a.h.g_w2[m] != nullptr;
  float yb0[16], yb1[16];
  if (gw2 && wave < ct) tn_load(yb0, w.y + (int64_t)m * a.d + wave * 32, (int64_t)a.M * a.d, a.N, l31, h);
  if (gw2 && wave + TH_W < ct) tn_load(yb1, w.y + (int64_t)m * a.d + (wave + TH_W) * 32, (int64_t)a.M * a.d, a.N, l31, h);
  if (a.use_bn) {
    const float mu = w.mean[(int64_t)m * a.d + col], rs = w.rstd[(int64_t)m * a.d + col], ga = a.h.bn_gamma[m][col];
    const float xh = live ? (w.x1[p] - mu) * rs : 0.f;
    sm.tile[0][n][j] = dzv;
    sm.tile[1][n][j] = dzv * xh;
    __syncthreads();
    {
      const int r = tid & 31, c = tid >> 5;
      const float s1 = half_wave_sum(sm.tile[0][r][c]), s2 = half_wave_sum(sm.tile[1][r][c]);
      if (r == 0) {
        sm.colv[0][c] = s1;
        sm.colv[1][c] = s2;
        if (a.h.g_bn_beta[m]) a.h.g_bn_beta[m][j0 + c] = s1;
        if (a.h.g_bn_gamma[m]) a.h.g_bn_gamma[m][j0 + c] = s2;
      }
    }
    __syncthreads();
    if (a.training) dx = ga * rs * (dzv - sm.colv[0][j] / a.N - xh * sm.colv[1][j] / a.N);
    else dx = ga * rs * dzv;
    if (!live) dx = 0.f;
  }
  if (live) w.dz[p] = dx;
  sm.tile[2][n][j] = dx;
  __syncthreads();
  {
    const float sb = half_wave_sum(sm.tile[2][tid & 31][tid >> 5]);
    if ((tid & 31) == 0 && a.h.g_b2[m]) a.h.g_b2[m][j0 + (tid >> 5)] = sb;
  }
  if (gw2) {
    if (wave < ct) store_tile(tn_mma(sm.tile[2], yb0, l31, h), a.h.g_w2[m] + (int64_t)j0 * a.d + wave * 32, a.d, l31, h);
    if (wave + TH_W < ct)
      store_tile(tn_mma(sm.tile[2], yb1, l31, h), a.h.g_w2[m] + (int64_t)j0 * a.d + (wave + TH_W) * 32, a.d, l31, h);
  }
}

__global__ __launch_bounds__(TH_T) void th_bwd3_kernel(ThArgs a) {
  extern __shared__ __attribute__((aligned(16))) unsigned char th_smem_raw[];
  ThSmem& sm = *(ThSmem*)th_smem_raw;
  const int tid = threadIdx.x, lane = tid & 63, wave = tid >> 6, l31 = lane & 31, h = lane >> 5;
  const int ct = a.d / 32, gemm_blocks = a.M * ct;
  const ThWs w = th_layout(a.ws, a.N, a.M, a.d);
  if ((int)blockIdx.x >= gemm_blocks) {
    const int kb_n = (a.K + 4 * TH_T - 1) / (4 * TH_T);
    const int q = blockIdx.x - gemm_blocks, m = q / kb_n, k4 = ((q % kb_n) * TH_T + tid) * 4;
    const unsigned key = (!a.text_moe && a.thr16 && a.key_dev) ? *a.key_dev : 0u;
    if (k4 < a.K && a.h.g_moe_w[m]) {
      f32x4 s = {0.f, 0.f, 0.f, 0.f};
#pragma unroll 8
      for (int n = 0; n < a.N; ++n) s += moe_input4(a, key, n, k4) * w.dlogit[(int64_t)n * a.M + m];
      *(f32x4*)(a.h.g_moe_w[m] + k4) = s;
    }
    if (q % kb_n == 0 && tid == 0 && a.h.g_moe_b[m]) {
      float s = 0.f;
      for (int n = 0; n < a.N; ++n) s += w.dlogit[(int64_t)n * a.M + m];
      a.h.g_moe_b[m][0] = s;
    }
    return;
  }
  const int m = blockIdx.x / ct, j0 = (blockIdx.x % ct) * 32;
  const int per = k_slice(a.d), kbeg = wave * per, kend = min(a.d, kbeg + per);
  const bool gw1 = a.h.g_w1[m] != nullptr;
  const int kt_n = a.K / 32;
  float tb0[16], tb1[16];
  {
    const float* ap = w.dz + ((int64_t)min(l31, a.N - 1) * a.M + m) * a.d;
    const bool iok = l31 < a.N;
    const float* bp = a.h.w2[m] + j0 + l31;
    f32x4 av[TH_TMAX], bv[TH_TMAX];
#pragma unroll
    for (int t = 0; t < TH_TMAX; ++t) {
      const int k0 = kbeg + 8 * t + 4 * h;
      av[t] = bv[t] = (f32x4){0.f, 0.f, 0.f, 0.f};
      if (k0 + 3 < kend) {
        if (iok) av[t] = *(const f32x4*)(ap + k0);
#pragma unroll
        for (int u = 0; u < 4; ++u) bv[t][u] = bp[(int64_t)(k0 + u) * a.d];
      }
    }
    f32x16 acc;
#pragma unroll
    for (int r = 0; r < 16; ++r) acc[r] = 0.f;
#pragma unroll
    for (int t = 0; t < TH_TMAX; ++t) {
      if (kbeg + 8 * t < kend) {
#pragma unroll
        for (int u = 0; u < 4; ++u) acc = __builtin_amdgcn_mfma_f32_32x32x2f32(av[t][u], bv[t][u], acc, 0, 0, 0);
      }
    }
    const int n = tile_row(wave, lane);
    const int64_t p = ((int64_t)n * a.M + m) * a.d + j0 + l31;
    const float dyg0 = n < a.N ? w.dyg[p] : 0.f;
    if (gw1 && wave < kt_n) tn_load(tb0, a.text + wave * 32, a.K, a.N, l31, h);
    if (gw1 && wave + TH_W < kt_n) tn_load(tb1, a.text + (wave + TH_W) * 32, a.K, a.N, l31, h);
    float v = splitk_reduce_then(sm, acc, wave, lane, dyg0);
    if (n < a.N) {
      w.dyg[p] = v;
    } else {
      v = 0.f;
    }
    sm.tile[2][n][l31] = v;
  }
  __syncthreads();
  {
    const float sb = half_wave_sum(sm.tile[2][tid & 31][tid >> 5]);
    if ((tid & 31) == 0 && a.h.g_b1[m]) a.h.g_b1[m][j0 + (tid >> 5)] = sb;
  }
  if (gw1) {
    if (wave < kt_n) store_tile(tn_mma(sm.tile[2], tb0, l31, h), a.h.g_w1[m] + (int64_t)j0 * a.K + wave * 32, a.K, l31, h);
    if (wave + TH_W < kt_n)
      store_tile(tn_mma(sm.tile[2], tb1, l31, h), a.h.g_w1[m] + (int64_t)j0 * a.K + (wave + TH_W) * 32, a.K, l31, h);
  }
}

extern "C" int mmt_text_heads_fast(int N, int M, int d, int K) {
  return N >= 1 && N <= 32 && M >= 1 && M <= MMT_MAX_EXPERTS && d % 32 == 0 && d >= 32 && d <= 1024 && K % 32 == 0 &&
         K >= 32 && K <= 1024;
}

static int th_configure() {
  static bool done = false;
  if (done) return 0;
  const void* fns[] = {(const void*)th_fwd1_kernel, (const void*)th_fwd2_kernel, (const void*)th_bwd2_kernel,
                       (const void*)th_bwd3_kernel, (const void*)th_fwd1_plan_kernel, (const void*)th_fwd2_cast_kernel};
  for (const void* f : fns) {
    hipError_t rc = hipFuncSetAttribute(f, hipFuncAttributeMaxDynamicSharedMemorySize, (int)sizeof(ThSmem));
    if (rc != hipSuccess) return (int)rc;
  }
  done = true;
  return 0;
}

static void th_fill(ThArgs& a, const MmtTextHeads* h, const float* text, const float* text_moe, int N, int C, int M, int d,
                    int K, int use_bn, int training, float* ws, const MmtTextHeadsOpts* o) {
  a = {};
  a.h = *h;
  a.text = text; a.text_moe = text_moe; a.ws = ws;
  a.N = N; a.C = C; a.M = M; a.d = d; a.K = K; a.use_bn = use_bn; a.training = training;
  if (o) {
    a.drop_key = o->moe_drop_key; a.thr16 = o->moe_drop_thr16; a.drop_scale = o->moe_drop_scale;
    a.seed_dev = o->seed_dev; a.key_dev = o->key_dev; a.nbt = (long long*)o->num_batches_tracked;
  }
}

int mmt_text_heads_fwd_small(const MmtTextHeads* h, const float* text, const float* text_moe, int N, int C, int M, int d,
                             int K, int use_bn, int training, float* ws, float* text_embds, float* text_weights,
                             const MmtTextHeadsOpts* opts, hipStream_t s) {
  if (int rc = th_configure()) return rc;
  ThArgs a;
  th_fill(a, h, text, text_moe, N, C, M, d, K, use_bn, training, ws, opts);
  a.text_embds = text_embds; a.text_weights = text_weights;
  if (!text_moe && a.thr16 && (!a.seed_dev || !a.key_dev)) return MMT_ERR_ARG;
  const int gemm_blocks = M * (d / 32);
  const int blocks1 = gemm_blocks + (text_weights ? N : 0);
  const MmtVideoFront* vf = opts ? opts->video_front : nullptr;
  if (vf) {
    VideoPlanArgs p;
    if (int e = video_plan_args(p, vf->experts, vf->M, vf->B, vf->T, vf->pack, vf->max_pos, vf->counts, vf->cu_seqlens,
                                vf->n_rows_dev, vf->slot, vf->row_index, vf->type_ids, vf->pos_ids, vf->mask_bias, vf->agg_row,
                                nullptr, vf->src))
      return e;
    if ((size_t)vf->M * vf->T * sizeof(float) > sizeof(ThSmem)) return MMT_ERR_ARG;
    VideoCastArgs c = {};
    CastSplit cs = {};
    int cast_blocks = 0;
    if (vf->do_cast) {
      if (int e = video_cast_args(c, vf->experts, vf->M, vf->B, vf->T, vf->src)) return e;
      int64_t wsum = 0;
      for (int i = 0; i < vf->M; ++i) wsum += vf->experts[i].Dpad;
      for (int i = 0; i < vf->M; ++i) {
        cs.begin[i] = cast_blocks;
        const int64_t share = (400 * (int64_t)vf->experts[i].Dpad + wsum - 1) / wsum;
        cast_blocks += (int)(share < 1 ? 1 : share);
      }
      cs.begin[vf->M] = cast_blocks;
    }
    hipLaunchKernelGGL(th_fwd1_plan_kernel, dim3(blocks1 + vf->B), dim3(TH_T), sizeof(ThSmem), s, a, p, blocks1);
    hipLaunchKernelGGL(th_fwd2_cast_kernel, dim3(gemm_blocks + cast_blocks), dim3(TH_T), sizeof(ThSmem), s, a, c, gemm_blocks,
                       cs, vf->M, vf->seed_bump);
    if (cast_blocks) {
      CastSplit c3 = cs;
      for (int i = 0; i <= vf->M; ++i) c3.begin[i] = cs.begin[i] * 4;
      hipLaunchKernelGGL(th_fwd3_cast_kernel, dim3((N * M + 3) / 4 + 4 * cast_blocks), dim3(256), 0, s, a, c, (N * M + 3) / 4, c3,
                         vf->M);
      return (int)hipGetLastError();
    }
  } else {
    hipLaunchKernelGGL(th_fwd1_kernel, dim3(blocks1), dim3(TH_T), sizeof(ThSmem), s, a);
    hipLaunchKernelGGL(th_fwd2_kernel, dim3(gemm_blocks), dim3(TH_T), sizeof(ThSmem), s, a);
  }
  hipLaunchKernelGGL(th_fwd3_kernel, dim3((N * M + 3) / 4), dim3(256), 0, s, a);
  return (int)hipGetLastError();
}

int mmt_text_heads_bwd_small(const MmtTextHeads* h, const float* text, const float* text_moe, int N, int C, int M, int d,
                             int K, int use_bn, int training, float* ws, const float* dtext_embds, const float* text_weights,
                             const float* dtext_weights, float* dtext_moe, const MmtTextHeadsOpts* opts, hipStream_t s) {
  if (int rc = th_configure()) return rc;
  ThArgs a;
  th_fill(a, h, text, text_moe, N, C, M, d, K, use_bn, training, ws, opts);
  a.de = dtext_embds; a.tw = text_weights; a.dtw = dtext_weights; a.dtext_moe = dtext_moe;
  const bool moe = text_weights && dtext_weights;
  const int gemm_blocks = M * (d / 32);
  hipLaunchKernelGGL(th_bwd1_kernel, dim3((N * M + 3) / 4 + (moe ? N : 0)), dim3(256), 0, s, a);
  hipLaunchKernelGGL(th_bwd2_kernel, dim3(gemm_blocks), dim3(TH_T), sizeof(ThSmem), s, a);
  const int kb_n = (K + 4 * TH_T - 1) / (4 * TH_T);
  hipLaunchKernelGGL(th_bwd3_kernel, dim3(gemm_blocks + (moe ? M * kb_n : 0)), dim3(TH_T), sizeof(ThSmem), s, a);
  return (int)hipGetLastError();
}
```

### mmt_amd/model.py

```python
import collections
import ctypes
import re
import types

import torch
import torch.nn.functional as F
from torch import nn

from . import _lib, ops
from ._lib import MmtExpertIO, MmtTextHeads, MmtTextHeadsOpts, MmtVideoFront, MmtVideoSrc, check
from .bert import BertModel, EngineBatch
from .feature_store import RaggedFeatures
from .flat import FlatParams


def _round_up(x, m):
  return (x + m - 1) // m * m


class ReduceDim(nn.Module):

  def __init__(self, input_dimension, output_dimension):
    super().__init__()
    self.fc = nn.Linear(input_dimension, output_dimension)

  def forward(self, x):
    return F.normalize(self.fc(x), dim=-1)


class ContextGating(nn.Module):

  def __init__(self, dimension, add_batch_norm=True):
    super().__init__()
    self.fc = nn.Linear(dimension, dimension)
    self.add_batch_norm = add_batch_norm
    self.batch_norm = nn.BatchNorm1d(dimension)

  def forward(self, x):
    x1 = self.fc(x)
    if self.add_batch_norm:
      x1 = self.batch_norm(x1)
    return F.glu(torch.cat((x, x1), 1), 1)


class GatedEmbeddingUnit(nn.Module):

  def __init__(self, input_dimension, output_dimension, use_bn, normalize):
    super().__init__()
    self.fc = nn.Linear(input_dimension, output_dimension)
    self.cg = ContextGating(output_dimension, add_batch_norm=use_bn)
    self.normalize = normalize

  def forward(self, x):
    x = self.cg(self.fc(x))
    if self.normalize:
      x = F.normalize(x, dim=-1)
    return x


class _VideoTokensFn(torch.autograd.Function):

  @staticmethod
  def forward(ctx, net, plan, *params):
    ctx.net, ctx.plan, ctx.generation = net, plan, plan.generation
    return net._video_tokens_forward(plan)

  @staticmethod
  def backward(ctx, dfeat):
    if ctx.plan.generation != ctx.generation:
      raise RuntimeError('mmt_amd.CENet: video-token buffers were overwritten by a later forward')
    return (None, None) + tuple(ctx.net._video_tokens_backward(ctx.plan, dfeat.contiguous()))


class _ReadoutFn(torch.autograd.Function):

  @staticmethod
  def forward(ctx, last, agg_row, bm, compact=False, stash=None):
    ctx.compact = compact
    d = last.shape[1]
    out = torch.empty(bm, d, device=last.device, dtype=torch.float32)
    inv = torch.empty(bm, device=last.device, dtype=torch.float32)
    check(_lib.lib().mmt_readout_fwd(ops._p(last), ops._p(agg_row), bm, d, ops._p(out), ops._p(inv), ops._stream()),
          'mmt_readout_fwd')
    ctx.save_for_backward(out, inv, agg_row)
    ctx.shape = last.shape
    if stash is not None:
      stash.update(readout_inv=inv, readout_rows=None if compact else agg_row, readout_compact=compact)
    return out

  @staticmethod
  def backward(ctx, dout):
    out, inv, agg_row = ctx.saved_tensors
    dlast = (torch.empty if ctx.compact else torch.zeros)(ctx.shape, device=out.device, dtype=torch.float32)
    check(_lib.lib().mmt_readout_bwd(ops._p(out), ops._p(inv), ops._p(dout.contiguous()), ops._p(agg_row),
                                     out.shape[0], out.shape[1], ops._p(dlast), ops._stream()), 'mmt_readout_bwd')
    return dlast, None, None, None, None


class _SimsFn(torch.autograd.Function):

  @staticmethod
  def forward(ctx, txt, vid, tw, vw):
    nt, m, d = txt.shape
    nv = vid.shape[0]
    txt, vid, tw, vw = (x.detach().contiguous().float() for x in (txt, vid, tw, vw))
    sims = torch.empty(nt, nv, device=txt.device, dtype=torch.float32)
    dots = torch.empty(nt, nv, m, device=txt.device, dtype=torch.float32)
    check(_lib.lib().mmt_sims_fwd(ops._p(txt), ops._p(vid), ops._p(tw), ops._p(vw), nt, nv, m, d, ops._p(sims),
                                  ops._p(dots), ops._stream()), 'mmt_sims_fwd')
    ctx.save_for_backward(txt, vid, tw, vw, dots)
    return sims

  @staticmethod
  def backward(ctx, dsims):
    txt, vid, tw, vw, dots = ctx.saved_tensors
    nt, m, d = txt.shape
    nv = vid.shape[0]
    dtxt, dvid, dtw, dvw = (torch.empty_like(x) for x in (txt, vid, tw, vw))
    check(_lib.lib().mmt_sims_bwd(ops._p(txt), ops._p(vid), ops._p(tw), ops._p(vw), ops._p(dots),
                                  ops._p(dsims.contiguous().float()), nt, nv, m, d, ops._p(dtxt), ops._p(dvid),
                                  ops._p(dtw), ops._p(dvw), ops._stream()), 'mmt_sims_bwd')
    return dtxt, dvid, dtw, dvw


class _MoeDropoutFn(torch.autograd.Function):
  SITE_KEY = 0x7e57d0a1

  @staticmethod
  def forward(ctx, x, p, seed_dev):
    x = x.contiguous().float()
    y = torch.empty_like(x)
    ctx.key = torch.empty(1, dtype=torch.int32, device=x.device)
    ctx.thr, ctx.scale = ops.dropout_params(p)
    check(_lib.lib().mmt_dropout_f32(ops._p(x), ops._p(y), x.numel(), _MoeDropoutFn.SITE_KEY, ctx.thr, ctx.scale,
                                     ops._p(seed_dev), ops._p(ctx.key), None, ops._stream()), 'mmt_dropout_f32')
    return y

  @staticmethod
  def backward(ctx, g):
    g = g.contiguous().float()
    gx = torch.empty_like(g)
    check(_lib.lib().mmt_dropout_f32(ops._p(g), ops._p(gx), g.numel(), _MoeDropoutFn.SITE_KEY, ctx.thr, ctx.scale, None,
                                     None, ops._p(ctx.key), ops._stream()), 'mmt_dropout_f32')
    return gx, None, None


class _TextHeadsFn(torch.autograd.Function):

  @staticmethod
  def forward(ctx, net, text, text_moe, caps, moe_drop_p, *params):
    tm = None if text_moe is None else text_moe.detach().contiguous().float()
    out = net._text_heads_forward(text.detach().contiguous().float(), tm, caps, moe_drop_p)
    ctx.net, ctx.caps, ctx.generation, ctx.training = net, caps, net._th_generation, net.training
    ctx.need_dtext = text.requires_grad
    ctx.need_dmoe = text_moe is not None and text_moe.requires_grad
    net._th_needs_input_grad = ctx.need_dtext or ctx.need_dmoe
    return out

  @staticmethod
  def backward(ctx, de, dtw):
    net = ctx.net
    if net._th_generation != ctx.generation:
      raise RuntimeError('mmt_amd.CENet: text-head buffers were overwritten by a later forward')
    dtext, dmoe, grads = net._text_heads_backward(ctx.caps, de, dtw, ctx.need_dtext, ctx.need_dmoe, ctx.training)
    return (None, dtext, dmoe, None, None) + tuple(grads)


def cross_view_similarity(vid_embds, text_embds, vid_weights, text_weights, merge='avg'):
  b, m, d = vid_embds.shape
  c = text_embds.shape[2]
  dev = vid_embds.device
  on_cpu = not vid_embds.is_cuda
  if on_cpu:
    if not torch.cuda.is_available():
      raise RuntimeError('mmt_amd similarity needs a GPU (no CPU fallback)')
    vid_embds, text_embds, vid_weights, text_weights = (x.cuda() for x in (vid_embds, text_embds, vid_weights,
                                                                           text_weights))
  txt = text_embds.permute(0, 2, 1, 3).reshape(b * c, m, d)
  sims = _SimsFn.apply(txt, vid_embds, text_weights.reshape(b * c, m), vid_weights.reshape(b, m))
  if c > 1:
    if merge == 'avg':
      sims = sims.view(b, c, b).mean(1)
    elif merge != 'indep':
      raise ValueError('unrecognised merge mode: {}'.format(merge))
  return sims.to(dev) if on_cpu else sims


def sharded_cross_view_inner_product(vid_embds, text_embds, vid_weights, text_weights, subspaces,
                                     merge_caption_similiarities='avg'):
  vid = torch.stack([vid_embds[mod] for mod in subspaces], 1)
  b = vid.shape[0]
  txt = torch.stack([text_embds[mod].reshape(b, -1, vid.shape[-1]) for mod in subspaces], 1)
  c = txt.shape[2]
  return cross_view_similarity(vid, txt, vid_weights.reshape(b, -1), text_weights.reshape(b, c, -1),
                               merge_caption_similiarities)


class _VideoPlan:
  KSPLIT = 768

  def __init__(self, net, bsz, t, device):
    mods, dims = net.modalities, net.expert_dims
    m = len(mods)
    self.batch, self.tokens, self.seq = bsz, t, 1 + m * (t + 1)
    self.rows = bsz * self.seq
    self.rows_alloc = ops.pad_rows(self.rows)
    self.generation = 0
    self.front_done = -1
    i32 = dict(device=device, dtype=torch.int32)
    self.counts = torch.zeros(bsz, **i32)
    self.cu = torch.zeros(bsz + 1, **i32)
    self.n_rows = torch.zeros(1, **i32)
    self.slot = torch.zeros(self.rows, **i32)
    self.row_index = torch.zeros(self.rows_alloc, **i32)
    self.type_ids = torch.zeros(self.rows_alloc, **i32)
    self.pos_ids = torch.zeros(self.rows_alloc, **i32)
    self.mask_bias = torch.zeros(self.rows_alloc, device=device, dtype=torch.float32)
    self.agg_row = torch.zeros(bsz * m, **i32)
    self.src_row = torch.zeros(self.rows_alloc, **i32)
    self.src_cnt = torch.zeros(m, **i32)
    self.xsrc = torch.zeros(m, bsz * t, **i32)
    self.src = MmtVideoSrc()
    self.src.src_row, self.src.src_cnt, self.src.xsrc = (x.data_ptr() for x in (self.src_row, self.src_cnt, self.xsrc))
    self.compact_rows = None
    self.features = None
    self.src_rows = bsz * (t + 1)
    self.src_rows_pad = _round_up(self.src_rows, 128)
    d = net.same_dim
    self.x, self.y, self.dy, self.y_part = {}, {}, {}, {}
    self.zero_bias = torch.zeros(d, device=device, dtype=torch.float32)
    chunks = {mod: min(3, -(-_round_up(dims[mod]['dim'], 128) // self.KSPLIT)) for mod in mods}
    if sum(chunks.values()) > 16:
      chunks = {mod: 1 for mod in mods}
    self.xin = {}
    self.precast = False
    for mod in mods:
      dpad = _round_up(dims[mod]['dim'], 128)
      self.x[mod] = torch.zeros(self.src_rows_pad, dpad, device=device, dtype=torch.bfloat16)
      self.y[mod] = torch.zeros(self.src_rows_pad, d, device=device, dtype=torch.float32)
      self.dy[mod] = torch.zeros(self.src_rows_pad, d, device=device, dtype=torch.bfloat16)
      self.y_part[mod] = [torch.zeros(self.src_rows_pad, d, device=device, dtype=torch.float32)
                          for _ in range(chunks[mod] - 1)]
    self.io = (MmtExpertIO * m)()
    self.inputs = None


class CENet(nn.Module):

  def __init__(self, l2renorm, expert_dims, tokenizer, keep_missing_modalities, test_caption_mode,
# ... 118 lines not shown
    self._flat = FlatParams(named)
    self._th_generation = 0
    self._th_ws = {}
    self._nbt = None
    self.vid_bert.register_shadows(self._flat)
    for mod in self.modalities:
      dim = expert_dims[mod]['dim']
      self._flat.add_shadow(('reduce', mod), [self.video_dim_reduce[mod].fc.weight], same_dim, dim,
                            k_pad=_round_up(dim, 128))
    self.vid_bert.attach_flat(self._flat)
    self._plans = {}
    self._stages = None

  def __str__(self):
    n = sum(p.numel() for p in self.parameters() if p.requires_grad)
    return super().__str__() + '\nTrainable parameters: {}'.format(n)

  def grad_regions(self, split_bottom=False):
    f, vb = self._flat, self.vid_bert
    n_layers = vb.config.num_hidden_layers
    named = vb.engine_named_params()
    per_layer = [[p for n, p in named if n.startswith('encoder.layer.%d.' % l)] for l in range(n_layers)]
    emb = [p for n, p in named if n.startswith('embeddings.')]
    top = list(self._text_head_params()) if self._native_text_heads else []
    if n_layers >= 2:
      top = per_layer[n_layers - 1] + top
    out = [('top', f.span(top))] if top else []
    for l in range(n_layers - 2, 0, -1):
      out.append(('layer%d' % l, f.span(per_layer[l])))
    if split_bottom and n_layers >= 2:
      out.append(('layer0', f.span(per_layer[0])))
      out.append(('bottom', f.span(self._reduce_params() + emb)))
    else:
      out.append(('bottom', f.span(self._reduce_params() + emb + per_layer[0])))
    return out

  @staticmethod
  def count_live_rows(features_ind):
    first = next(iter(features_ind.values()))
    total = int(first.shape[0])
    for ind in features_ind.values():
      total += int(ind.shape[0]) + int((torch.as_tensor(ind) != 0).sum())
    return total

  @staticmethod
  def count_live_tokens(token_ids):
    return int((torch.as_tensor(token_ids)[..., 1] != 0).sum())

  def engine_params(self):
    return self._flat.params

  def flats(self):
    out = [self._flat]
    if self._native_text_tower:
      out.append(self.txt_bert.build_flat())
    return out

  def _reduce_params(self):
    out = []
    for mod in self.modalities:
      out += [self.video_dim_reduce[mod].fc.weight, self.video_dim_reduce[mod].fc.bias]
    return out

  def _prepare(self, device):
    if self._flat.ensure(device):
      self.vid_bert._structs = {}
      self._th_ws = {}
    self._flat.pack()
    if torch.is_grad_enabled():
      self._flat.select_grad_buffer()
    self.vid_bert._ensure_ready(device)

  def _video_tokens_forward(self, plan):
    L, m, d = _lib.lib(), len(self.modalities), self.same_dim
    io, stream = plan.io, ops._stream()
    max_pos = self.vid_bert_params['max_position_embeddings'] - 1
    vb = self.vid_bert
    bump = vb._seed_dev if (plan.bump_seed and vb._seed_dev is not None) else None
    vb._seed_bumped = bump is not None
    if plan.front_done != plan.generation:
      check(L.mmt_video_plan(io, m, plan.batch, plan.tokens, int(self.pack_tokens), max_pos, ops._p(plan.counts),
                             ops._p(plan.cu), ops._p(plan.n_rows), ops._p(plan.slot), ops._p(plan.row_index),
                             ops._p(plan.type_ids), ops._p(plan.pos_ids), ops._p(plan.mask_bias), ops._p(plan.agg_row),
                             ops._p(bump), ctypes.byref(plan.src), stream), 'mmt_video_plan')
      if not plan.precast:
        check(L.mmt_video_cast(io, m, plan.batch, plan.tokens, ctypes.byref(plan.src), stream), 'mmt_video_cast')
    items, index = [], []
    for i, mod in enumerate(self.modalities):
      x, w = plan.xin[mod], self._flat.shadow(('reduce', mod))[0]
      outs = [plan.y[mod]] + plan.y_part[mod]
      step = _round_up(-(-x.shape[1] // len(outs)), 64)
      for c, out in enumerate(outs):
        k0 = c * step
        k1 = x.shape[1] if c == len(outs) - 1 else k0 + step
        items.append((x[:, k0:k1], w[:, k0:k1], out, self.video_dim_reduce[mod].fc.bias if c == 0 else plan.zero_bias))
        index.append(i)
    ops.gemm_nt_grouped(items, m=plan.src_rows, n_rows_dev=plan.src_cnt, n_rows_index=index)
    feats = torch.empty(plan.rows_alloc, d, device=plan.slot.device, dtype=torch.float32)
    check(L.mmt_video_scatter(io, m, plan.batch, plan.tokens, d, ops._p(plan.n_rows), ops._p(plan.row_index),
                              ctypes.byref(plan.src), ops._p(feats), stream), 'mmt_video_scatter')
    return feats

  def _video_front(self, plan):
    vb = self.vid_bert
    bump = vb._seed_dev if (plan.bump_seed and vb._seed_dev is not None) else None
    f = MmtVideoFront()
    f.experts = ctypes.addressof(plan.io)
    f.M, f.B, f.T, f.pack = len(self.modalities), plan.batch, plan.tokens, int(self.pack_tokens)
    f.max_pos, f.do_cast = self.vid_bert_params['max_position_embeddings'] - 1, int(not plan.precast)
    for name, t in (('counts', plan.counts), ('cu_seqlens', plan.cu), ('n_rows_dev', plan.n_rows), ('slot', plan.slot),
                    ('row_index', plan.row_index), ('type_ids', plan.type_ids), ('pos_ids', plan.pos_ids),
                    ('mask_bias', plan.mask_bias), ('agg_row', plan.agg_row)):
      setattr(f, name, t.data_ptr())
    f.seed_bump = bump.data_ptr() if bump is not None else None
    f.src = ctypes.addressof(plan.src)
    return f

  def _video_tokens_backward(self, plan, dfeat, side_stream=None):
    L, m, d = _lib.lib(), len(self.modalities), self.same_dim
    stream = ops._stream()
    check(L.mmt_video_scatter_bwd(plan.io, m, plan.batch, plan.tokens, d, ops._p(plan.n_rows), ops._p(plan.row_index),
                                  ctypes.byref(plan.src), ops._p(dfeat), stream), 'mmt_video_scatter_bwd')
    grad_buf = self._flat.current_grad()
    grads, items = [], []
    for mod in self.modalities:
      fc = self.video_dim_reduce[mod].fc
      gw, gb = self._flat.view(fc.weight, grad_buf), self._flat.view(fc.bias, grad_buf)
      items.append((plan.dy[mod], plan.xin[mod], gw, gb))
      grads += [gw if fc.weight.requires_grad else None, gb if fc.bias.requires_grad else None]
    if side_stream is not None:
      side_stream.wait_stream(torch.cuda.current_stream())
      with torch.cuda.stream(side_stream):
        ops.wgrad_grouped(items, plan.src_rows, item_rows_dev=plan.src_cnt)
    else:
      ops.wgrad_grouped(items, plan.src_rows, item_rows_dev=plan.src_cnt)
    return grads

  def video_embeddings(self, features, features_t, features_ind, features_maxpool, plan=None):
    if plan is None:
      plan = self._video_prepare(features, features_t, features_ind, features_maxpool)
    mods, bsz, dev = self.modalities, plan.batch, plan.slot.device
    feats = _VideoTokensFn.apply(self, plan, *self._reduce_params())
    batch = EngineBatch(None, plan.type_ids, plan.pos_ids if self.pos_enc != 'none' else None, plan.mask_bias,
                        plan.rows, bsz, plan.seq, cu_seqlens=plan.cu,
                        row_index=plan.row_index if self.pack_tokens else None,
                        n_rows_dev=plan.n_rows if self.pack_tokens else None,
                        out_rows=plan.agg_row if self.tail_rows_only else None, n_out_per_sample=len(mods))
    hint = self.live_rows_hint
    if hint is None and isinstance(features, RaggedFeatures):
      hint = bsz + sum(int(v) for v in features.live.values())
    batch.live_rows_hint = int(hint or 0) if self.pack_tokens else 0
    last = self.vid_bert.run_engine(batch, feats)
    self._stages = dict(plan=plan, feats=feats, batch=batch, last=last) if last.requires_grad else None
    if self.vid_bert.compact_output(batch, plan.rows_alloc):
      if plan.compact_rows is None:
        plan.compact_rows = torch.arange(bsz * len(mods), device=dev, dtype=torch.int32)
      vid = _ReadoutFn.apply(last, plan.compact_rows, bsz * len(mods), True, self._stages)
    else:
      vid = _ReadoutFn.apply(last, plan.agg_row, bsz * len(mods), False, self._stages)
    vid = vid.view(bsz, len(mods), self.same_dim)
    if self._stages is not None:
      self._stages['vid_embds'] = vid
    return vid

  def _video_prepare(self, features, features_t, features_ind, features_maxpool):
    mods = self.modalities
    ragged = features if isinstance(features, RaggedFeatures) else None
    if ragged is not None:
      if not self.pack_tokens:
        raise NotImplementedError('RaggedFeatures carry no padded rows: they need pack_tokens=True')
      if [n for n, _ in ragged.layout.experts] != mods or any(
          d != self.expert_dims[n]['dim'] for n, d in ragged.layout.experts):
        raise ValueError('RaggedFeatures experts %r do not match the model\'s %r' % (ragged.layout.experts, mods))
      dev, bsz, t = ragged.device, ragged.batch, ragged.tokens
      if dev.type != 'cuda':
        raise RuntimeError('mmt_amd.CENet runs on the GPU only (no CPU fallback)')
      features_ind, features_t = ragged.ind, ragged.t
    else:
      f0 = features[mods[0]]
      if not f0.is_cuda:
        raise RuntimeError('mmt_amd.CENet runs on the GPU only (no CPU fallback)')
      dev = f0.device
      bsz, t = f0.shape[0], f0.shape[1]
      for mod in mods:
        if features[mod].shape[1] != t:
          raise NotImplementedError('all experts must share max_expert_tokens (as in every published config)')
    self._prepare(dev)
    key = (bsz, t, dev)
    plan = self._plans.get(key)
    if plan is None:
      plan = self._plans[key] = _VideoPlan(self, bsz, t, dev)
    plan.generation += 1
    keep = []
    for i, mod in enumerate(mods):
      io = plan.io[i]
      if ragged is not None:
        tensors = [x.detach().to(device=dev, dtype=torch.float32).contiguous() for x in (features_ind[mod], features_t[mod])]
        x = ragged.x[mod]
        if x.shape != plan.x[mod].shape:
          raise ValueError('RaggedFeatures layout does not match the model (rows/K padding)')
        keep.append(tensors + [x])
        io.feat = io.maxpool = None
        io.ind, io.t = (v.data_ptr() for v in tensors)
      else:
        tensors = [features[mod], features_maxpool[mod], features_ind[mod], features_t[mod]]
        tensors = [x.detach().to(device=dev, dtype=torch.float32).contiguous() for x in tensors]
        keep.append(tensors)
        x = plan.x[mod]
        io.feat, io.maxpool, io.ind, io.t = (v.data_ptr() for v in tensors)
      plan.xin[mod] = x
      io.x, io.y, io.dy = x.data_ptr(), plan.y[mod].data_ptr(), plan.dy[mod].data_ptr()
      io.D, io.Dpad = self.expert_dims[mod]['dim'], x.shape[1]
      io.n_part = len(plan.y_part[mod])
      for c, part in enumerate(plan.y_part[mod]):
        io.y_part[c] = part.data_ptr()
      io.type_idx, io.rows_pad = self.expert_dims[mod]['idx'], plan.src_rows_pad
    plan.inputs = keep
    plan.precast = ragged is not None
    plan.bump_seed = self.vid_bert.training and torch.is_grad_enabled()
    return plan

  def _text_head_params(self):
    out = [self.text_GU[mod].fc.weight for mod in self.modalities]
    for mod in self.modalities:
      gu = self.text_GU[mod]
      out += [gu.fc.bias, gu.cg.fc.weight, gu.cg.fc.bias, gu.cg.batch_norm.weight, gu.cg.batch_norm.bias]
    if self.txt_wgh == 'emb':
      for mod in self.modalities:
        out += [self.moe_fc_txt[mod].weight, self.moe_fc_txt[mod].bias]
    return out

  def _text_heads_struct(self, grad_buf):
    f, h = self._flat, MmtTextHeads()
    for i, mod in enumerate(self.modalities):
      gu, bn = self.text_GU[mod], self.text_GU[mod].cg.batch_norm
      pairs = dict(w1=gu.fc.weight, b1=gu.fc.bias, w2=gu.cg.fc.weight, b2=gu.cg.fc.bias, bn_gamma=bn.weight,
                   bn_beta=bn.bias)
      if self.txt_wgh == 'emb':
        pairs.update(moe_w=self.moe_fc_txt[mod].weight, moe_b=self.moe_fc_txt[mod].bias)
      for name, p in pairs.items():
        getattr(h, name)[i] = f.ptr(p)
        if grad_buf is not None and p.requires_grad:
          getattr(h, 'g_' + name)[i] = f.ptr(p, grad_buf)
      h.running_mean[i] = bn.running_mean.data_ptr()
      h.running_var[i] = bn.running_var.data_ptr()
    return h

  def _text_heads_fast(self, n, k):
    return bool(_lib.lib().mmt_text_heads_fast(n, len(self.modalities), self.same_dim, k))

  def _text_heads_opts(self, moe_drop_p, nbt):
    o = MmtTextHeadsOpts()
    if moe_drop_p > 0.0:
      if self._th_key is None or self._th_key.device != self.vid_bert._seed_dev.device:
        self._th_key = torch.zeros(1, dtype=torch.int32, device=self.vid_bert._seed_dev.device)
      o.moe_drop_key = _MoeDropoutFn.SITE_KEY
      o.moe_drop_thr16, o.moe_drop_scale = ops.dropout_params(moe_drop_p)
      o.seed_dev, o.key_dev = self.vid_bert._seed_dev.data_ptr(), self._th_key.data_ptr()
    if nbt is not None:
      o.num_batches_tracked = nbt.data_ptr()
    return o

  _th_key = None
  _pending_front = None
  _th_front = None
  front_fuse = True

  def _text_heads_forward(self, text, text_moe, caps, moe_drop_p=0.0):
    n, k = text.shape
    m, d = len(self.modalities), self.same_dim
    L = _lib.lib()
    key = (n, text.device)
    ws = self._th_ws.get(key)
    if ws is None:
      ws = self._th_ws[key] = torch.zeros(L.mmt_text_heads_workspace_floats(n, m, d), device=text.device)
    self._th_generation += 1
    self._th_text, self._th_text_moe = text, text_moe
    use_bn = int(self.txt_pro == 'gbn')
    fast = self._text_heads_fast(n, k)
    if moe_drop_p > 0.0 and not fast:
      raise RuntimeError('on-the-fly MoE dropout needs the small-batch text-head kernels')
    nbt = None
    if self.training and use_bn:
      if n <= 1:
        raise ValueError('Expected more than 1 value per channel when training')
      if self._nbt is None or self._nbt.device != text.device or any(
          self.text_GU[mod].cg.batch_norm.num_batches_tracked.data_ptr() != self._nbt[i].data_ptr()
          for i, mod in enumerate(self.modalities)):
        vals = [int(self.text_GU[mod].cg.batch_norm.num_batches_tracked) for mod in self.modalities]
        self._nbt = torch.tensor(vals, dtype=torch.long, device=text.device)
        for i, mod in enumerate(self.modalities):
          self.text_GU[mod].cg.batch_norm.num_batches_tracked.data = self._nbt[i]
      if fast:
        nbt = self._nbt
      else:
        self._nbt.add_(1)
    embds = torch.empty(n // caps, m, caps, d, device=text.device, dtype=torch.float32)
    tw = torch.empty(n // caps, caps, m, device=text.device, dtype=torch.float32) if self.txt_wgh == 'emb' else None
    h = self._text_heads_struct(None)
    self._th_opts = self._text_heads_opts(moe_drop_p, nbt)
    front_plan, self._pending_front = self._pending_front, None
    if front_plan is not None and fast:
      self._th_front = self._video_front(front_plan)
      self._th_opts.video_front = ctypes.addressof(self._th_front)
      front_plan.front_done = front_plan.generation
    check(L.mmt_text_heads_fwd(ctypes.byref(h), ops._p(text), ops._p(text_moe), n, caps, m, d, k, use_bn, int(self.training), ops._p(ws),
                               ops._p(embds), ops._p(tw), ctypes.byref(self._th_opts), ops._stream()), 'mmt_text_heads_fwd')
    if tw is None:
      tw = torch.full((n // caps, caps, m), 1.0 / m, device=text.device)
    self._th_tw = tw
    return embds, tw

  def _text_heads_backward(self, caps, de, dtw, need_dtext, need_dmoe, training):
    text, text_moe = self._th_text, self._th_text_moe
    n, k = text.shape
    m, d = len(self.modalities), self.same_dim
    L = _lib.lib()
    grad_buf = self._flat.current_grad()
    h = self._text_heads_struct(grad_buf)
    dtext = torch.empty_like(text) if need_dtext else None
    dmoe = torch.empty_like(text) if (need_dmoe and text_moe is not None) else None
    w1_all = self._flat.ptr(self.text_GU[self.modalities[0]].fc.weight)
    has_moe = self.txt_wgh == 'emb'
    opts = self._th_opts
    fused_drop = opts.moe_drop_thr16 != 0 and text_moe is None
    dmoe_fused = torch.empty_like(text) if (fused_drop and need_dtext and has_moe) else None
    bwd_opts = MmtTextHeadsOpts.from_buffer_copy(opts)
    bwd_opts.num_batches_tracked = None
    bwd_opts.video_front = None
    check(L.mmt_text_heads_bwd(ctypes.byref(h), ops._p(text), ops._p(text_moe), ctypes.c_void_p(w1_all), n, caps, m, d, k,
                               int(self.txt_pro == 'gbn'), int(training), ops._p(self._th_ws[(n, text.device)]),
                               ops._p(de.contiguous()), ops._p(self._th_tw) if has_moe else None,
                               ops._p(dtw.contiguous()) if has_moe and dtw is not None else None, ops._p(dtext),
                               ops._p(dmoe_fused if dmoe_fused is not None else dmoe), ctypes.byref(bwd_opts), ops._stream()),
          'mmt_text_heads_bwd')
    if dmoe_fused is not None and dtw is not None:
      dtext.add_(dmoe_fused)
    grads = [self._flat.view(p, grad_buf) if p.requires_grad else None for p in self._text_head_params()]
    return dtext, dmoe, grads

  def text_features(self, token_ids, device):
    b, c, w, f = token_ids.size()
    if getattr(self.txt_bert, 'ignores_token_inputs', False):
      out = self.txt_bert(None)
      return out[0][:, 0] if self.post_agg == 'cls' else (torch.max(out[0][:, 1:], 1)[0] if self.post_agg == 'mxp'
                                                          else torch.mean(out[0][:, 1:], 1))
    if self._native_text_tower:
      hint = self.text_live_rows_hint
      if hint is None and not token_ids.is_cuda:
        hint = self.count_live_tokens(token_ids)
      self.txt_bert.live_rows_hint = hint
    tok = token_ids.view(b * c, w, f).to(device)
    input_ids = tok[:, :, 0].long()
    attention_mask = tok[:, :, 1].long()
    position_ids = torch.arange(w, device=device).unsqueeze(0).expand(b * c, w)
    token_type_ids = torch.zeros_like(input_ids)
    out = self.txt_bert(input_ids, attention_mask=attention_mask, token_type_ids=token_type_ids,
                        position_ids=position_ids, head_mask=None)
    last_layer = out[0]
    if self.post_agg == 'cls':
      return last_layer[:, 0]
    if self.post_agg == 'mxp':
      return torch.max(last_layer[:, 1:], 1)[0]
    return torch.mean(last_layer[:, 1:], 1)

  def compute_weights_from_emb(self, embd):
    embd = self.moe_txt_dropout(embd)
    b, k, d = embd.size()
    flat = embd.view(b * k, d)
    w = torch.cat([self.moe_fc_txt[mod](flat) for mod in self.modalities], dim=-1)
    return F.softmax(w, dim=1).view(b, k, len(self.modalities))

  def forward(self, token_ids, features, features_t, features_ind, features_avgpool, features_maxpool,
              query_masks, out='conf', device=None, debug=None):
    dev = (features.device if isinstance(features, RaggedFeatures) else features[self.modalities[0]].device) \
        if device is None else torch.device(device)
    if dev.type != 'cuda':
      raise RuntimeError('mmt_amd.CENet runs on the GPU only (no CPU fallback)')
    b, c = token_ids.size(0), token_ids.size(1)
    m = len(self.modalities)
    text = self.text_features(token_ids, dev)
    self._prepare(dev)
    plan = self._video_prepare(features, features_t, features_ind, features_maxpool)
    side = None
    self._pending_front = None
    if self._native_text_heads:
      cur = torch.cuda.current_stream(dev)
      if self.overlap_text_heads:
        side = self._side_streams.get(dev)
        if side is None:
          side = self._side_streams[dev] = torch.cuda.Stream(device=dev)
        side.wait_stream(cur)
      with torch.cuda.stream(side if side is not None else cur):
        text_moe, moe_drop_p = None, 0.0
        if self.txt_wgh == 'emb' and self.training and self.moe_txt_dropout.training and self.moe_txt_dropout.p > 0:
          if self.vid_bert._seed_dev is not None and self._text_heads_fast(text.shape[0], text.shape[1]):
            moe_drop_p = float(self.moe_txt_dropout.p)
          elif text.numel() % 4 == 0 and self.vid_bert._seed_dev is not None:
            text_moe = _MoeDropoutFn.apply(text, self.moe_txt_dropout.p, self.vid_bert._seed_dev)
          else:
            text_moe = self.moe_txt_dropout(text)
        if self.front_fuse and side is None:
          self._pending_front = plan
        text_embds, text_weights = _TextHeadsFn.apply(self, text, text_moe, c, moe_drop_p, *self._text_head_params())
        self._pending_front = None
    else:
      text_embd = [self.text_GU[mod](text).view(b, c, -1) for mod in self.modalities]
      tv = text.view(b, c, -1)
      text_weights = self.compute_weights_from_emb(tv) if self.txt_wgh == 'emb' else torch.ones(b, c, m, device=dev)
      text_weights = F.normalize(text_weights, p=1, dim=-1)
      text_embds = torch.stack([F.normalize(t, dim=-1) for t in text_embd], 1)
    vid_embds = self.video_embeddings(features, features_t, features_ind, features_maxpool, plan=plan)
    if side is not None:
      cur.wait_stream(side)
      for t in (text_embds, text_weights):
        t.record_stream(cur)
    vw_key = (b, m, dev)
    vid_weights = self._vid_weights.get(vw_key)
    if vid_weights is None:
      vid_weights = self._vid_weights[vw_key] = torch.full((b, m), 1.0 / m, device=dev)
    merge = 'avg' if self.training else self.test_caption_mode
    self.merge_caption_similarities = merge
    if out == 'conf':
      return {'modalities': self.modalities,
              'cross_view_conf_matrix': cross_view_similarity(vid_embds, text_embds, vid_weights, text_weights, merge)}
    return {'vid_embds': vid_embds, 'text_embds': text_embds, 'vid_weights': vid_weights,
            'text_weights': text_weights}
```

### mmt_amd/train_step.py

```python
import time
import torch
import torch.distributed as dist

import os

from . import dist as mdist
from . import _lib
from .feature_store import RaggedFeatures
from .model import cross_view_similarity
from .optim import FlatAdam


_QUIESCE_WARNED = False


def _pending_nccl_works():
  import pickle
  try:
    from torch._C._distributed_c10d import _dump_nccl_trace
    if int(os.environ.get('TORCH_NCCL_TRACE_BUFFER_SIZE', '2000')) <= 0:
      return None
    active = pickle.loads(_dump_nccl_trace(True, False, True)).get('entries', [])
    if active:
      return len(active)
    seen = pickle.loads(_dump_nccl_trace(True, False, False)).get('entries', [])
    return 0 if seen else None
  except Exception:
    return None


class FlatMinibatch(dict):

  def __init__(self, minibatch, device, pin_memory=False):
    super().__init__()
    leaves = []
    self.ragged = []

    def walk(d, out):
      for k, v in d.items():
        if isinstance(v, dict):
          out[k] = {}
          walk(v, out[k])
        elif torch.is_tensor(v):
          leaves.append((out, k, v))
        elif isinstance(v, RaggedFeatures):
          out[k] = RaggedFeatures(v.layout, device, pin_memory).copy_from(v, non_blocking=False)
          self.ragged.append(k)
        else:
          out[k] = v

    walk(minibatch, self)
    off = 0
    spans = []
    for _, _, v in leaves:
      off = (off + 255) // 256 * 256
      spans.append(off)
      off += v.numel() * v.element_size()
    self.flat = torch.zeros(max(off, 1), dtype=torch.uint8, device=device,
                            pin_memory=bool(pin_memory) and torch.device(device).type == 'cpu')
    for (out, k, v), o in zip(leaves, spans):
      n = v.numel() * v.element_size()
      view = self.flat[o:o + n].view(v.dtype).view(v.shape)
      view.copy_(v)
      out[k] = view


def _clone_tree(src):
  if isinstance(src, FlatMinibatch):
    return FlatMinibatch(src, src.flat.device)
  out = {}
  for k, v in src.items():
    if isinstance(v, dict):
      out[k] = _clone_tree(v)
    elif torch.is_tensor(v):
      out[k] = v.clone()
    elif isinstance(v, RaggedFeatures):
      out[k] = RaggedFeatures(v.layout, v.device).copy_from(v, non_blocking=False)
    else:
      out[k] = v
  return out


def _copy_tree(dst, src):
  for k, v in src.items():
    if isinstance(v, dict):
      _copy_tree(dst[k], v)
    elif torch.is_tensor(v):
      dst[k].copy_(v, non_blocking=True)
    elif isinstance(v, RaggedFeatures):
      dst[k].copy_from(v)


FORK_WGRAD, FORK_EARLY, FORK_REDUCE = _lib.FORK_WGRAD, _lib.FORK_EARLY, _lib.FORK_REDUCE
FORK_ADAM = 16
FORK_TEXT = 32
FORK_TOKENS = 64
FORK_ALL = FORK_WGRAD | FORK_REDUCE | FORK_ADAM | FORK_TEXT | FORK_TOKENS
FORK_DEFAULT = 0


class GraphedTrainStep:
  _rider_on = False

  def __init__(self, model, loss_fn, minibatch, lr=5e-5, group=None, use_graphs=True, warmup_steps=3,
               overlap_grad_sync=None, force_collectives=False, grad_dtype=None, capture_collectives=False, fork=None,
               grad_algo='allreduce', split_bottom=True, input_slots=1, bind_inputs=None, shard_optimizer=False,
               host_feed=None, adam_riders=None, live_rows=None):
    if adam_riders:
      raise ValueError('adam_riders: removed; measured slower, see DESIGN §7')
    self.model, self.loss_fn, self.group = model, loss_fn, group
    if fork is None:
      fork = FORK_DEFAULT
    self.fork = int(fork)
    self._side = None
    self._fork_on = False
    self._keep = []
    self.world = dist.get_world_size(group) if dist.is_initialized() else 1
    self.rank = dist.get_rank(group) if dist.is_initialized() else 0
    if live_rows is not None and hasattr(model, 'live_rows_hint'):
      model.live_rows_hint = int(live_rows)
    self._sig, self._by_sig, self._sig_cache = None, {}, {}
    self._force_coll = bool(force_collectives) and dist.is_initialized()
    self._multi = self.world > 1 or self._force_coll
    self._want_stages = self._multi if overlap_grad_sync is None else bool(overlap_grad_sync)
    self.staged = False
    self.static = minibatch
    self._statics = [minibatch]
    self._bind = bind_inputs
    self._caps = None
    self._slot_ev = None
    self._host_feed = list(host_feed) if host_feed else None
    self._feed_stream = None
    self._next_upload = None
    self._done_ev = None
    self.capture_collectives = bool(capture_collectives)
    self._cap_mode = 'thread_local' if dist.is_initialized() else 'global'
    self._one_graph = False
    self._pool = None
    self._staging = None
    flats = model.flats() if hasattr(model, 'flats') else [model._flat]
    flat_ids = {id(p) for f in flats for p in f.params}
    rest = [p for p in model.parameters() if p.requires_grad and id(p) not in flat_ids]
    self.opt_flats = [FlatAdam(f, lr=lr) for f in flats]
    self.opt_flat = self.opt_flats[0]
    self._rest_lr = None
    if rest:
      dev0 = rest[0].device
      if use_graphs and dev0.type == 'cuda':
        self._rest_lr = torch.tensor(float(lr), device=dev0, dtype=torch.float32)
      self.opt_rest = torch.optim.Adam(rest, lr=self._rest_lr if self._rest_lr is not None else lr, capturable=use_graphs)
    else:
      self.opt_rest = None
    self.grad_dtype = grad_dtype
    self.grad_algo, self._split_bottom = grad_algo, bool(split_bottom)
    self.shard_opt = bool(shard_optimizer) and self.world > 1
    if shard_optimizer and grad_algo != 'rs_ag':
      raise ValueError("shard_optimizer needs grad_algo='rs_ag' (the shards are what the reduce-scatter leaves on a rank)")
    self._wire = mdist.WireBuffer(grad_dtype, grad_algo)
    self.syncs = [mdist.GradSync(f, rest if i == 0 else (), group, grad_dtype=grad_dtype, algo=grad_algo)
                  for i, f in enumerate(flats)]
    self._opt_of = {id(o.flat): o for o in self.opt_flats}
    self._whole_regions = {'flat%d' % i: (o.flat, 0, o.flat.count) for i, o in enumerate(self.opt_flats)}
    self._rest_sync = mdist.GradSync(None, rest, group) if self.shard_opt else None
    self._shard_spans = []
    self._exposed = []
    self.sync = self.syncs[0]
    self._extra_flats = flats[1:]
    self.use_graphs = use_graphs
    self.loss = None
    self._graphs = None
    self._stream = torch.cuda.Stream()
    self._stream.wait_stream(torch.cuda.current_stream())
    with torch.cuda.stream(self._stream):
      snap = self._snapshot() if warmup_steps > 0 else None
      for i in range(warmup_steps):
        self._eager_step()
        if i == 0 and (self._want_stages or self.fork):
          ok = self._stageable([p for p in rest if p.grad is not None])
          self.staged = ok and self._want_stages
          if not ok or len(flats) > 1 or not hasattr(model, '_text_heads_backward'):
            self.fork = 0
          if self.fork:
            self._side = torch.cuda.Stream()
            if self.fork & FORK_TEXT:
              model.overlap_text_heads = True
              model._side_streams[next(model.parameters()).device] = self._side
            self._fork_on = True
      if snap is not None:
        self._restore(snap)
    torch.cuda.current_stream().wait_stream(self._stream)
    if use_graphs:
      if int(input_slots) > 1:
        self._statics += [_clone_tree(minibatch) for _ in range(int(input_slots) - 1)]
        if self._host_feed is not None and len(self._host_feed) != len(self._statics):
          raise ValueError('host_feed: one pinned FlatMinibatch per input slot')
      self._capture_slots()
      self._sig = self._tile_signature(getattr(model, 'live_rows_hint', None))

  def _capture_slots(self):
    self._n_capture_sets = getattr(self, '_n_capture_sets', 0) + 1
    if len(self._statics) > 1:
      self._caps = []
      for si, st in enumerate(self._statics):
        self.static = st
        if self._host_feed is not None:
          nx = (si + 1) % len(self._statics)
          self._next_upload = (self._statics[nx], self._host_feed[nx])
        if self._bind:
          self._bind(st)
        self._capture()
        if self._pool is None:
          g0 = self._graphs[0]
          self._pool = g0.pool()
        self._caps.append((self._graphs, self._e, self.loss, self._one_graph))
      self.static = self._statics[0]
      if self._bind:
        self._bind(self.static)
      self._graphs, self._e, self.loss, self._one_graph = self._caps[0]
    else:
      self._capture()

  def _tile_signature(self, live_rows):
    m = self.model
    vb = getattr(m, 'vid_bert', None)
    if live_rows is None or vb is None or not getattr(m, 'pack_tokens', False) or not getattr(m, '_plans', None):
      return None
    hit = self._sig_cache.get(int(live_rows))
    if hit is not None:
      return hit
    L, E = _lib.lib(), _lib.EPI
    rows = next(iter(m._plans.values())).rows
    d, I = vb.config.hidden_size, vb.config.intermediate_size
    shapes = [(E['BIAS_BF16'], 3 * d, d, 0), (E['BIAS_DROP_RES'], d, d, 0), (E['BIAS_GELU'], I, d, 0), (E['BIAS_DROP_RES'], d, I, 0),
              (E['DGELU'], I, d, 0), (E['ADD_F32'], d, I, 0), (E['BF16'], d, d, 1), (E['ADD_F32'], d, 3 * d, 0)]
    sig = tuple(L.mmt_gemm_select_tile(e, rows, n, k, 1, int(live_rows), 0, dot, 0) for e, n, k, dot in shapes)
    self._sig_cache[int(live_rows)] = sig
    return sig

  def _switch_tiles(self, sig, live_rows):
    self._by_sig[self._sig] = (self._caps, self._graphs, self._e, self.loss, self._one_graph)
    self.model.live_rows_hint = int(live_rows)
    hit = self._by_sig.get(sig)
    if hit is not None:
      self._caps, self._graphs, self._e, self.loss, self._one_graph = hit
    else:
      cur = torch.cuda.current_stream()
      self._stream.wait_stream(cur)
      with torch.cuda.stream(self._stream):
        self._capture_slots()
      cur.wait_stream(self._stream)
    self._sig = sig

  def _snapshot(self):
    m = self.model
    snap = dict(buffers=[(b, b.detach().clone()) for b in m.buffers()], flats=[], rest=[], seeds=[])
    for f in (m.flats() if hasattr(m, 'flats') else [m._flat]):
      if f.master is None or not f.is_flat():
        f.ensure(f.params[0].device)
      snap['flats'].append((f, f.master.detach().clone()))
    flat_ids = {id(p) for f, _ in snap['flats'] for p in f.params}
    snap['rest'] = [(p, p.detach().clone()) for p in m.parameters() if id(p) not in flat_ids]
    for mod in m.modules():
      sd = getattr(mod, '_seed_dev', None)
      if torch.is_tensor(sd):
        snap['seeds'].append((mod, sd.detach().clone()))
    return snap

  @torch.no_grad()
  def _restore(self, snap):
    for b, v in snap['buffers']:
      b.copy_(v)
    for f, v in snap['flats']:
      f.master.copy_(v)
      f._dirty = True
      f.pack()
    for p, v in snap['rest']:
      p.copy_(v)
    for mod, v in snap['seeds']:
      mod._seed_dev.copy_(v)
    for o in self.opt_flats:
      if o.exp_avg is not None:
        o.exp_avg.zero_()
        o.exp_avg_sq.zero_()
        o.step_dev.zero_()
    if self.opt_rest is not None:
      for st in self.opt_rest.state.values():
        for v in st.values():
          if torch.is_tensor(v):
            v.zero_()
    self._zero()

  def _upload_branch_begin(self):
    if self._next_upload is None or not torch.cuda.is_current_stream_capturing():
      return
    dst, src = self._next_upload
    if self._feed_stream is None:
      self._feed_stream = torch.cuda.Stream()
    self._feed_stream.wait_stream(torch.cuda.current_stream())
    with torch.cuda.stream(self._feed_stream):
      dst.flat.copy_(src.flat, non_blocking=True)

  def _upload_branch_end(self):
    if self._next_upload is None or not torch.cuda.is_current_stream_capturing():
      return
    torch.cuda.current_stream().wait_stream(self._feed_stream)

  def prime(self, slot=0):
    if self._host_feed is None:
      raise RuntimeError('prime() needs host_feed')
    self._statics[slot].flat.copy_(self._host_feed[slot].flat, non_blocking=False)
    torch.cuda.synchronize()

  def step_done(self, slot):
    if self._done_ev is not None and self._done_ev[slot] is not None:
      self._done_ev[slot].synchronize()

  def _forward(self):
    self._upload_branch_begin()
    mb = self.static
    e = self.model(mb['token_ids'], mb['features'], mb.get('features_t'), mb.get('features_ind'),
                   mb.get('features_avgpool'), mb.get('features_maxpool'), mb['query_masks'], out='embds')
    self._pack_local(e)
    return e

  _send = _recv = _gkeys = None

  def _pack_local(self, e):
    if not self._multi:
      return
    if self._send is None:
      self._gkeys = [(k, tuple(e[k].shape), e[k].numel()) for k in sorted(e)]
      total = sum(n for _, _, n in self._gkeys)
      dev = e[self._gkeys[0][0]].device
      self._send = torch.empty(total, device=dev, dtype=torch.float32)
      self._recv = torch.empty(self.world * total, device=dev, dtype=torch.float32)
    off = 0
    for k, _, n in self._gkeys:
      self._send[off:off + n].copy_(e[k].detach().reshape(-1))
      off += n

  def _gather(self, e):
    if not self._multi:
      return {k: v.detach() for k, v in e.items()}
    dist.all_gather_into_tensor(self._recv, self._send, group=self.group)
    recv, out, off = self._recv.view(self.world, -1), {}, 0
    for k, _, n in self._gkeys:
      out[k] = recv[:, off:off + n]
      off += n
    return out

  def _globalize(self, e, g):
    if not self._multi:
      return g
    shapes = {k: shape for k, shape, _ in self._gkeys}
    return {k: v.reshape((self.world * shapes[k][0],) + shapes[k][1:]) for k, v in g.items()}

  def _loss_backward(self, e, g):
    g = self._globalize(e, g)
    fast = self._fast_loss_grads(e, g, fuse_readout=True)
    if fast is not None:
      loss, outs, grads = fast
      torch.autograd.backward(outs, grads)
      return loss
    leaves = {k: v.detach().requires_grad_(e[k].requires_grad) for k, v in g.items()}
    sims = cross_view_similarity(leaves['vid_embds'], leaves['text_embds'], leaves['vid_weights'],
                                 leaves['text_weights'], 'avg')
    loss = self.loss_fn(sims)
    need = [k for k in leaves if leaves[k].requires_grad]
    grads = torch.autograd.grad(loss, [leaves[k] for k in need])
    b = e['vid_embds'].shape[0]
    sl = slice(self.rank * b, (self.rank + 1) * b)
    torch.autograd.backward([e[k] for k in need], [gr[sl] for gr in grads])
    return loss.detach()

  def _fast_loss_grads(self, e, g, fuse_readout=False):
    import ctypes

    from . import _lib, ops
    from .loss import InfoNceLoss, MaxMarginRankingLoss
    from ._lib import check
    if not isinstance(self.loss_fn, (MaxMarginRankingLoss, InfoNceLoss)) or g['text_embds'].shape[2] != 1:
      return None
    if g['vid_weights'].requires_grad or e['vid_weights'].requires_grad:
      return None
    L = _lib.lib()
    vid = g['vid_embds'].detach().contiguous().float()
    n, m, d = vid.shape
    txt = g['text_embds'].detach().reshape(n, m, d).contiguous().float()
    tw = g['text_weights'].detach().reshape(n, m).contiguous().float()
    vw = g['vid_weights'].detach().reshape(n, m).contiguous().float()
    dev = vid.device
    sims = torch.empty(n, n, device=dev, dtype=torch.float32)
    dots = torch.empty(n, n, m, device=dev, dtype=torch.float32)
    check(L.mmt_sims_fwd(ops._p(txt), ops._p(vid), ops._p(tw), ops._p(vw), n, n, m, d, ops._p(sims), ops._p(dots),
                         ops._stream()), 'mmt_sims_fwd')
    loss = torch.empty((), device=dev, dtype=torch.float32)
    b = e['vid_embds'].shape[0]
    sl = slice(self.rank * b, (self.rank + 1) * b)
    if 2 <= n <= L.mmt_simloss_small_max_n():
      kind = 0 if isinstance(self.loss_fn, MaxMarginRankingLoss) else 1
      margin = float(getattr(self.loss_fn, 'margin', 0.0))
      fix_norm = int(getattr(self.loss_fn, 'fix_norm', True))
      st = getattr(self.model, '_stages', None) if (n == b and fuse_readout) else None
      fused = st is not None and st.get('vid_embds') is e['vid_embds'] and st.get('readout_inv') is not None
      dtxt, dtw = torch.empty_like(txt), torch.empty_like(tw)
      dvid = dlast = None
      if fused:
        last = st['last']
        dlast = (torch.empty if st['readout_compact'] else torch.zeros)(last.shape, device=dev, dtype=torch.float32)
      else:
        dvid = torch.empty_like(vid)
      check(L.mmt_simloss_bwd_small(ops._p(txt), ops._p(vid), ops._p(tw), ops._p(vw), ops._p(sims), ops._p(dots), n, m, d, kind,
                                    margin, fix_norm, ops._p(loss), ops._p(dtxt), ops._p(dvid), ops._p(dtw), None,
                                    ops._p(st['readout_inv']) if fused else None,
                                    ops._p(st['readout_rows']) if fused and st['readout_rows'] is not None else None,
                                    ops._p(dlast), ops._stream()), 'mmt_simloss_bwd_small')
      outs, grads = [], []
      pairs = [('text_embds', dtxt.view(n, m, 1, d)), ('text_weights', dtw.view(n, 1, m))]
      if fused:
        outs.append(st['last'])
        grads.append(dlast)
      else:
        pairs.insert(0, ('vid_embds', dvid))
      for k, gfull in pairs:
        if e[k].requires_grad:
          outs.append(e[k])
          grads.append(gfull[sl])
      return loss, outs, grads
    grad = torch.empty(n, n, device=dev, dtype=torch.float32)
    scratch = torch.empty(3 * n, device=dev, dtype=torch.float32)
    if isinstance(self.loss_fn, MaxMarginRankingLoss):
      check(L.mmt_maxmargin(ops._p(sims), n, float(self.loss_fn.margin), int(self.loss_fn.fix_norm), ops._p(scratch),
                            ops._p(loss), ops._p(grad), ops._stream()), 'mmt_maxmargin')
    else:
      check(L.mmt_infonce(ops._p(sims), n, ops._p(scratch), ops._p(loss), ops._p(grad), ops._stream()), 'mmt_infonce')
    dtxt, dvid, dtw, dvw = (torch.empty_like(x) for x in (txt, vid, tw, vw))
    check(L.mmt_sims_bwd(ops._p(txt), ops._p(vid), ops._p(tw), ops._p(vw), ops._p(dots), ops._p(grad), n, n, m, d,
                         ops._p(dtxt), ops._p(dvid), ops._p(dtw), ops._p(dvw), ops._stream()), 'mmt_sims_bwd')
    outs, grads = [], []
    for k, gfull in (('vid_embds', dvid), ('text_embds', dtxt.view(n, m, 1, d)), ('text_weights', dtw.view(n, 1, m))):
      if e[k].requires_grad:
        outs.append(e[k])
        grads.append(gfull[sl])
    return loss, outs, grads

  def _stageable(self, rest):
    m = self.model
    st = getattr(m, '_stages', None)
    if rest or st is None or not getattr(m, '_native_text_heads', False):
      return False
    from .loss import InfoNceLoss, MaxMarginRankingLoss
    if not isinstance(self.loss_fn, (MaxMarginRankingLoss, InfoNceLoss)):
      return False
    return all(p.requires_grad for p in m._flat.params)

  def _stage_list(self, e, g):
    model, vb = self.model, self.model.vid_bert
    st = {}

    def head():
      fast = self._fast_loss_grads(e, self._globalize(e, g), fuse_readout=True)
      if fast is None:
        raise RuntimeError('staged backward needs one caption per video and the native losses')
      self.loss, outs, grads = fast
      pairs = list(zip(outs, grads))
      h = model._stages
      txt = [(o, gr) for o, gr in pairs if o is not e['vid_embds'] and o is not h['last']]
      if txt and not self._text_heads_backward_forked(e, txt):
        torch.autograd.backward([o for o, _ in txt], [gr for _, gr in txt])
      dlast = next((gr for o, gr in pairs if o is h['last']), None)
      if dlast is None:
        gvid = next(gr for o, gr in pairs if o is e['vid_embds'])
        dlast, = torch.autograd.grad([e['vid_embds']], [h['last']], [gvid])
      if self._fork_on:
        h['batch'].side_stream = self._side
        h['batch'].fork = (self.fork & (FORK_WGRAD | FORK_EARLY | FORK_REDUCE)) | (_lib.FORK_JOIN if self._multi else 0)
      st['run'] = vb.backward_ranges(h['batch'], dlast, vb.training)

    def bottom():
      st['run'](0, 0)
      side = self._side if (self._fork_on and self.fork & FORK_TOKENS) else None
      model._video_tokens_backward(model._stages['plan'], st['run'].dfeat, side_stream=side)
      if side is not None and self._multi:
        self._join()

    n_layers = vb.config.num_hidden_layers

    def top():
      head()
      if n_layers >= 2:
        st['run'](n_layers - 1, n_layers - 1)

    names = dict(self._grad_regions())
    stages = [(top, (['top'] if 'top' in names else []) + ['flat%d' % (i + 1) for i in range(len(self._extra_flats))])]
    for l in range(n_layers - 2, 0, -1):
      stages.append((lambda l=l: st['run'](l, l), ['layer%d' % l]))
    if 'layer0' in names:
      def bottom_split():
        st['run'](-1, -1)
        side = self._side if (self._fork_on and self.fork & FORK_TOKENS) else None
        model._video_tokens_backward(model._stages['plan'], st['run'].dfeat, side_stream=side)
        if side is not None and self._multi:
          self._join()
      stages.append((lambda: st['run'](0, 0, embed=False), ['layer0']))
      stages.append((bottom_split, ['bottom']))
    else:
      stages.append((bottom, ['bottom']))
    return stages

  def _grad_regions(self):
    return self.model.grad_regions(split_bottom=self._split_bottom and self.staged)

  def _text_heads_backward_forked(self, e, txt):
    m = self.model
    if not (self._fork_on and self.fork & FORK_TEXT) or self._multi:
      return False
    text = getattr(m, '_th_text', None)
    fn = getattr(e['text_embds'], 'grad_fn', None)
    if text is None or fn is None or any(t is not None and t.requires_grad for t in (text, m._th_text_moe)):
      return False
    if getattr(m, '_th_needs_input_grad', True):
      return False
    grads = {id(o): gr for o, gr in txt}
    de, dtw = grads.get(id(e['text_embds'])), grads.get(id(e['text_weights']))
    if de is None:
      return False
    cur = torch.cuda.current_stream()
    self._side.wait_stream(cur)
    self._keep += [de, dtw]
    with torch.cuda.stream(self._side):
      m._text_heads_backward(e['text_embds'].shape[2], de, dtw, False, False, m.training)
    return True

  def _join(self):
    if self._side is not None:
      torch.cuda.current_stream().wait_stream(self._side)

  def _adam_regions(self, names, last):
    cur = torch.cuda.current_stream()
    self._side.wait_stream(cur)
    with torch.cuda.stream(self._side):
      for i, n in enumerate(names):
        flat, off, cnt = self._regions[n]
        self.opt_flat.step_span(off, cnt, bump=last and i == len(names) - 1)

  def _region_table(self):
    tab = {n: (self.model._flat, off, cnt) for n, (off, cnt) in self._grad_regions()}
    for i, f in enumerate(self._extra_flats):
      tab['flat%d' % (i + 1)] = (f, 0, f.count)
    return tab
# ... 406 lines not shown
```

Measured before the change: 25160 pairs/s.

## Fuse video readout into sims forward and fold text-head bwd1 into bwd2

Result: no change. 25210 pairs/s (median of 6 runs) (+0.2%).

```diff
diff --git a/include/mmt_hip.h b/include/mmt_hip.h
--- a/include/mmt_hip.h
+++ b/include/mmt_hip.h
@@ -271,6 +271,10 @@
 int mmt_sims_bwd(const float* txt, const float* vid, const float* tw, const float* vw, float* dots,
                  const float* dsims, int NT, int NV, int M, int d, float* dtxt, float* dvid, float* dtw,
                  float* dvw, void* stream);
+int mmt_sims_readout_fast(int NT, int NV, int M, int d);
+int mmt_sims_readout_fwd(const float* txt, const float* last_hidden, const int32_t* agg_row, const float* tw,
+                         const float* vw, int NT, int NV, int M, int d, float* vid_embds, float* inv_norm, float* sims,
+                         float* dots, void* stream);
 int mmt_simloss_small_max_n(void);
 int mmt_simloss_bwd_small(const float* txt, const float* vid, const float* tw, const float* vw, const float* sims,
                           const float* dots, int n, int M, int d, int kind, float margin, int fix_norm, float* loss,
@@ -455,7 +459,7 @@
 typedef struct MmtTextHeadsOpts {
   uint32_t moe_drop_key, moe_drop_thr16;
   float moe_drop_scale;
-  int32_t reserved;
+  int32_t fold_bwd;
   const uint32_t* seed_dev;
   uint32_t* key_dev;
   int64_t* num_batches_tracked;
diff --git a/mmt_amd/_lib.py b/mmt_amd/_lib.py
--- a/mmt_amd/_lib.py
+++ b/mmt_amd/_lib.py
@@ -113,7 +113,7 @@
 
 
 class MmtTextHeadsOpts(ctypes.Structure):
-  _fields_ = [('moe_drop_key', c_u32), ('moe_drop_thr16', c_u32), ('moe_drop_scale', c_f32), ('reserved', ctypes.c_int32),
+  _fields_ = [('moe_drop_key', c_u32), ('moe_drop_thr16', c_u32), ('moe_drop_scale', c_f32), ('fold_bwd', ctypes.c_int32),
               ('seed_dev', c_vp), ('key_dev', c_vp), ('num_batches_tracked', c_vp), ('video_front', c_vp)]
 
 
@@ -214,6 +214,8 @@
     'mmt_readout_fwd': (c_int, [c_vp, c_vp, c_int, c_int, c_vp, c_vp, c_vp]),
     'mmt_readout_bwd': (c_int, [c_vp, c_vp, c_vp, c_vp, c_int, c_int, c_vp, c_vp]),
     'mmt_sims_fwd': (c_int, [c_vp, c_vp, c_vp, c_vp, c_int, c_int, c_int, c_int, c_vp, c_vp, c_vp]),
+    'mmt_sims_readout_fast': (c_int, [c_int, c_int, c_int, c_int]),
+    'mmt_sims_readout_fwd': (c_int, [c_vp, c_vp, c_vp, c_vp, c_vp, c_int, c_int, c_int, c_int, c_vp, c_vp, c_vp, c_vp, c_vp]),
     'mmt_sims_bwd': (c_int, [c_vp, c_vp, c_vp, c_vp, c_vp, c_vp, c_int, c_int, c_int, c_int, c_vp, c_vp, c_vp, c_vp,
                              c_vp]),
     'mmt_sims_eval_workspace_floats': (c_i64, [c_int, c_int, c_int, c_int]),
diff --git a/mmt_amd/csrc/simloss.hip b/mmt_amd/csrc/simloss.hip
--- a/mmt_amd/csrc/simloss.hip
+++ b/mmt_amd/csrc/simloss.hip
@@ -98,6 +98,91 @@
       drow[p] = a0;
       dots[((int64_t)t * NV + v0) * M + p] = a0;
       if (two) { drow[p1] = a1; dots[((int64_t)t * NV + v0) * M + p1] = a1; }
+    }
+  }
+  __syncthreads();
+  if ((int)threadIdx.x < nv) {
+    const int v = v0 + threadIdx.x;
+    float nrm = 0.f, sacc = 0.f;
+    for (int m = 0; m < M; ++m) nrm += tw[t * M + m] * vw[v * M + m];
+    if (nrm == 0.f) nrm = 1e-5f;
+    for (int m = 0; m < M; ++m) sacc += tw[t * M + m] * vw[v * M + m] / nrm * drow[threadIdx.x * M + m];
+    sims[(int64_t)t * NV + v] = sacc;
+  }
+}
+
+__global__ __launch_bounds__(64 * SF_WAVES) void sims_readout_fwd_small_kernel(
+    const float* __restrict__ txt, const float* __restrict__ last, const int32_t* __restrict__ agg_row,
+    const float* __restrict__ tw, const float* __restrict__ vw, int NT, int NV, int M, int d, float* __restrict__ sims,
+    float* __restrict__ dots, float* __restrict__ vid_out, float* __restrict__ inv_norm) {
+  extern __shared__ __attribute__((aligned(16))) float ts[];
+  float* drow = ts + M * d;
+  const int t = blockIdx.x, v0 = blockIdx.y * SF_VCHUNK, lane = threadIdx.x & 63, wave = threadIdx.x >> 6;
+  const int nv = min(SF_VCHUNK, NV - v0);
+  const int npair = nv * M;
+  f32x4 u[2][4];
+  auto load_rows = [&](int p) {
+    const int p1 = p + SF_WAVES;
+    const int pq[2] = {p, p1 < npair ? p1 : p};
+#pragma unroll
+    for (int q = 0; q < 2; ++q) {
+      const float* src = last + (int64_t)agg_row[v0 * M + pq[q]] * d;
+#pragma unroll
+      for (int c = 0; c < 4; ++c) {
+        const int col = c * 256 + lane * 4;
+        u[q][c] = (f32x4){0.f, 0.f, 0.f, 0.f};
+        if (col < d) u[q][c] = *(const f32x4*)(src + col);
+      }
+    }
+  };
+  if (wave < npair) load_rows(wave);
+  for (int i = threadIdx.x * 4; i < M * d; i += 256 * SF_WAVES) *(f32x4*)(ts + i) = *(const f32x4*)(txt + (int64_t)t * M * d + i);
+  __syncthreads();
+  for (int p = wave; p < npair; p += 2 * SF_WAVES) {
+#pragma clang fp reassociate(off)
+    const int p1 = p + SF_WAVES;
+    const bool two = p1 < npair;
+    const int mq[2] = {p % M, two ? p1 % M : 0};
+    if (p != wave) load_rows(p);
+    float ss[2] = {0.f, 0.f};
+#pragma unroll
+    for (int c = 0; c < 4; ++c) {
+      if (c * 256 + lane * 4 < d) {
+#pragma unroll
+        for (int q = 0; q < 2; ++q) {
+          const f32x4 v = u[q][c];
+          ss[q] = ss[q] + (__builtin_fmaf(v[0], v[0], v[2] * v[2]) + __builtin_fmaf(v[1], v[1], v[3] * v[3]));
+        }
+      }
+    }
+#pragma unroll
+    for (int o = 32; o > 0; o >>= 1) { ss[0] += __shfl_xor(ss[0], o, 64); ss[1] += __shfl_xor(ss[1], o, 64); }
+    const float inv[2] = {1.0f / fmaxf(sqrtf(ss[0]), 1e-12f), 1.0f / fmaxf(sqrtf(ss[1]), 1e-12f)};
+    float acc[2] = {0.f, 0.f};
+#pragma unroll
+    for (int c = 0; c < 4; ++c) {
+      const int col = c * 256 + lane * 4;
+      if (col < d) {
+#pragma unroll
+        for (int q = 0; q < 2; ++q) {
+          const f32x4 y = u[q][c] * inv[q];
+          const f32x4 x = *(const f32x4*)(ts + mq[q] * d + col);
+          acc[q] = __builtin_fmaf(x[3], y[3], __builtin_fmaf(x[2], y[2], __builtin_fmaf(x[0], y[0], __builtin_fmaf(x[1], y[1], acc[q]))));
+          if (t == 0 && (q == 0 || two)) *(f32x4*)(vid_out + ((int64_t)v0 * M + (q ? p1 : p)) * d + col) = y;
+        }
+      }
+    }
+#pragma unroll
+    for (int o = 32; o > 0; o >>= 1) { acc[0] += __shfl_xor(acc[0], o, 64); acc[1] += __shfl_xor(acc[1], o, 64); }
+    if (lane == 0) {
+      drow[p] = acc[0];
+      dots[((int64_t)t * NV + v0) * M + p] = acc[0];
+      if (t == 0) inv_norm[v0 * M + p] = inv[0];
+      if (two) {
+        drow[p1] = acc[1];
+        dots[((int64_t)t * NV + v0) * M + p1] = acc[1];
+        if (t == 0) inv_norm[v0 * M + p1] = inv[1];
+      }
     }
   }
   __syncthreads();
@@ -515,6 +600,23 @@
   return (int)hipGetLastError();
 }
 
+extern "C" int mmt_sims_readout_fast(int NT, int NV, int M, int d) {
+  return NT > 0 && NV > 0 && NT < LARGE_N && NV < LARGE_N && M > 0 && M <= MAXM && d > 0 && d % 4 == 0 && d <= 1024 &&
+         ((size_t)M * d + (size_t)SF_VCHUNK * M) * sizeof(float) <= 64 * 1024;
+}
+
+extern "C" int mmt_sims_readout_fwd(const float* txt, const float* last_hidden, const int32_t* agg_row, const float* tw,
+                                    const float* vw, int NT, int NV, int M, int d, float* vid_embds, float* inv_norm,
+                                    float* sims, float* dots, void* stream) {
+  if (!txt || !last_hidden || !agg_row || !tw || !vw || !vid_embds || !inv_norm || !sims || !dots ||
+      !mmt_sims_readout_fast(NT, NV, M, d))
+    return MMT_ERR_ARG;
+  hipLaunchKernelGGL(sims_readout_fwd_small_kernel, dim3(NT, (NV + SF_VCHUNK - 1) / SF_VCHUNK), dim3(64 * SF_WAVES),
+                     ((size_t)M * d + (size_t)SF_VCHUNK * M) * sizeof(float), (hipStream_t)stream, txt, last_hidden, agg_row, tw,
+                     vw, NT, NV, M, d, sims, dots, vid_embds, inv_norm);
+  return (int)hipGetLastError();
+}
+
 extern "C" int mmt_simloss_small_max_n(void) { return LARGE_N - 1; }
 
 extern "C" int mmt_simloss_bwd_small(const float* txt, const float* vid, const float* tw, const float* vw, const float* sims,
diff --git a/mmt_amd/csrc/texthead2.hip b/mmt_amd/csrc/texthead2.hip
--- a/mmt_amd/csrc/texthead2.hip
+++ b/mmt_amd/csrc/texthead2.hip
@@ -275,6 +275,65 @@
   video_cast_block(c, ex, r - cs.begin[ex], cs.begin[ex + 1] - cs.begin[ex], (int)threadIdx.x, 256, 1, 2);
 }
 
+__device__ __forceinline__ float th_rounded(float v) {
+  asm volatile("" : "+v"(v));
+  return v;
+}
+__device__ __forceinline__ void th_row_scalars(const f32x4 (&o)[4], const f32x4 (&g)[4], float& inv, float& proj) {
+#pragma clang fp reassociate(off)
+  float S[4], D[4];
+#pragma unroll
+  for (int k = 0; k < 4; ++k) {
+    const float s3 = th_rounded(o[3][k] * o[3][k]), s2 = th_rounded(o[2][k] * o[2][k]), s1 = th_rounded(o[1][k] * o[1][k]);
+    S[k] = __builtin_fmaf(o[0][k], o[0][k], (s3 + s2) + s1);
+    const float d2 = th_rounded(g[2][k] * o[2][k]), d1 = th_rounded(g[1][k] * o[1][k]);
+    D[k] = __builtin_fmaf(g[0][k], o[0][k], __builtin_fmaf(g[3][k], o[3][k], d2) + d1);
+  }
+  const float nrm = sqrtf(wave_sum((S[0] + S[2]) + (S[1] + S[3])));
+  inv = 1.0f / fmaxf(nrm, 1e-12f);
+  const float dot = wave_sum((D[0] + D[2]) + (D[1] + D[3]));
+  proj = nrm > 1e-12f ? (inv * inv) * dot : 0.f;
+}
+__device__ __forceinline__ void th_gate_bwd(float g, float o, float proj, float inv, float sg, float yy, float& dy, float& dz) {
+#pragma clang fp reassociate(off)
+  const float dox = __builtin_fmaf(-o, proj, g) * inv;
+  dy = dox * sg;
+  dz = th_rounded((dy * yy) * (1.0f - sg));
+}
+
+__device__ __forceinline__ void th_moe_bwd_row(const ThArgs& a, const ThWs& w, const int n, float* dl) {
+#pragma clang fp reassociate(off)
+  const int tid = threadIdx.x, lane = tid & 63, wave = tid >> 6;
+  if (wave == 0) {
+    const float t = lane < a.M ? a.tw[(int64_t)n * a.M + lane] : 0.f, dv = lane < a.M ? a.dtw[(int64_t)n * a.M + lane] : 0.f;
+    float dot = __builtin_fmaf(t, dv, __shfl_xor(th_rounded(t * dv), 32, 64));
+#pragma unroll
+    for (int o = 16; o > 0; o >>= 1) dot += __shfl_xor(dot, o, 64);
+    if (lane < a.M) {
+      dl[lane] = t * (dv - dot);
+      w.dlogit[(int64_t)n * a.M + lane] = dl[lane];
+    }
+  }
+  __syncthreads();
+  if (!a.dtext_moe) return;
+  const unsigned key = (!a.text_moe && a.thr16 && a.key_dev) ? *a.key_dev : 0u;
+  for (int k4 = tid * 4; k4 < a.K; k4 += 1024) {
+    f32x4 s = {0.f, 0.f, 0.f, 0.f};
+    for (int m = 0; m < a.M; ++m) {
+      const f32x4 ww = *(const f32x4*)(a.h.moe_w[m] + k4);
+#pragma unroll
+      for (int e = 0; e < 4; ++e) s[e] = __builtin_fmaf(dl[m], ww[e], s[e]);
+    }
+    if (!a.text_moe && a.thr16) {
+      bool kp[4];
+      keep4(key, (unsigned long long)n * (unsigned)a.K + (unsigned)k4, a.thr16, kp);
+#pragma unroll
+      for (int e = 0; e < 4; ++e) s[e] = kp[e] ? s[e] * a.drop_scale : 0.f;
+    }
+    *(f32x4*)(a.dtext_moe + (int64_t)n * a.K + k4) = s;
+  }
+}
+
 __global__ __launch_bounds__(256) void th_bwd1_kernel(ThArgs a) {
   __shared__ float dl[MMT_MAX_EXPERTS];
   const int tid = threadIdx.x, lane = tid & 63, wave = tid >> 6;
@@ -286,7 +345,6 @@
     const int n = r / a.M, m = r % a.M;
     const int64_t src = (int64_t)r * a.d, dst = (((int64_t)(n / a.C) * a.M + m) * a.C + n % a.C) * a.d;
     f32x4 o[4], g[4];
-    float ss = 0.f, dot = 0.f;
 #pragma unroll
     for (int c = 0; c < 4; ++c) {
       const int col = c * 256 + lane * 4;
@@ -295,12 +353,9 @@
         o[c] = *(const f32x4*)(w.o + src + col);
         g[c] = *(const f32x4*)(a.de + dst + col);
       }
-#pragma unroll
-      for (int k = 0; k < 4; ++k) { ss += o[c][k] * o[c][k]; dot += g[c][k] * o[c][k]; }
-    }
-    const float nrm = sqrtf(wave_sum(ss));
-    const float inv = 1.0f / fmaxf(nrm, 1e-12f);
-    const float proj = nrm > 1e-12f ? wave_sum(dot) * inv * inv : 0.f;
+    }
+    float inv, proj;
+    th_row_scalars(o, g, inv, proj);
 #pragma unroll
     for (int c = 0; c < 4; ++c) {
       const int col = c * 256 + lane * 4;
@@ -309,9 +364,10 @@
         f32x4 dy_, dz_;
 #pragma unroll
         for (int k = 0; k < 4; ++k) {
-          const float dox = (g[c][k] - o[c][k] * proj) * inv;
-          dy_[k] = dox * sg[k];
-          dz_[k] = dox * yy[k] * sg[k] * (1.0f - sg[k]);
+          float dy1, dz1;
+          th_gate_bwd(g[c][k], o[c][k], proj, inv, sg[k], yy[k], dy1, dz1);
+          dy_[k] = dy1;
+          dz_[k] = dz1;
         }
         *(f32x4*)(w.dyg + src + col) = dy_;
         *(f32x4*)(w.dz + src + col) = dz_;
@@ -319,29 +375,7 @@
     }
     return;
   }
-  const int n = blockIdx.x - row_blocks;
-  if (wave == 0) {
-    const float t = lane < a.M ? a.tw[(int64_t)n * a.M + lane] : 0.f, dv = lane < a.M ? a.dtw[(int64_t)n * a.M + lane] : 0.f;
-    const float dot = wave_sum(t * dv);
-    if (lane < a.M) {
-      dl[lane] = t * (dv - dot);
-      w.dlogit[(int64_t)n * a.M + lane] = dl[lane];
-    }
-  }
-  __syncthreads();
-  if (!a.dtext_moe) return;
-  const unsigned key = (!a.text_moe && a.thr16 && a.key_dev) ? *a.key_dev : 0u;
-  for (int k4 = tid * 4; k4 < a.K; k4 += 1024) {
-    f32x4 s = {0.f, 0.f, 0.f, 0.f};
-    for (int m = 0; m < a.M; ++m) s += *(const f32x4*)(a.h.moe_w[m] + k4) * dl[m];
-    if (!a.text_moe && a.thr16) {
-      bool kp[4];
-      keep4(key, (unsigned long long)n * (unsigned)a.K + (unsigned)k4, a.thr16, kp);
-#pragma unroll
-      for (int e = 0; e < 4; ++e) s[e] = kp[e] ? s[e] * a.drop_scale : 0.f;
-    }
-    *(f32x4*)(a.dtext_moe + (int64_t)n * a.K + k4) = s;
-  }
+  th_moe_bwd_row(a, w, blockIdx.x - row_blocks, dl);
 }
 
 __device__ __forceinline__ void tn_load(float (&b)[16], const float* __restrict__ G, int64_t ldg, int N, int l31, int h) {
@@ -365,17 +399,52 @@
   for (int r = 0; r < 16; ++r) out[(int64_t)((r & 3) + 8 * (r >> 2) + 4 * h) * ldo + l31] = acc[r];
 }
 
-__global__ __launch_bounds__(TH_T) void th_bwd2_kernel(ThArgs a) {
-  extern __shared__ __attribute__((aligned(16))) unsigned char th_smem_raw[];
-  ThSmem& sm = *(ThSmem*)th_smem_raw;
+template <bool FOLD>
+__device__ __forceinline__ void th_bwd2_block(const ThArgs& a, const unsigned bid, ThSmem& sm) {
   const int tid = threadIdx.x, lane = tid & 63, wave = tid >> 6, l31 = lane & 31, h = lane >> 5;
   const int ct = a.d / 32;
-  const int m = blockIdx.x / ct, j0 = (blockIdx.x % ct) * 32;
+  if (FOLD && bid >= (unsigned)(a.M * ct)) {
+    th_moe_bwd_row(a, th_layout(a.ws, a.N, a.M, a.d), (int)bid - a.M * ct, sm.colv[0]);
+    return;
+  }
+  const int m = bid / ct, j0 = (bid % ct) * 32;
   const ThWs w = th_layout(a.ws, a.N, a.M, a.d);
   const int n = tid >> 5, j = tid & 31, col = j0 + j;
   const int64_t p = ((int64_t)n * a.M + m) * a.d + col;
   const bool live = n < a.N;
-  const float dzv = live ? w.dz[p] : 0.f;
+  float dzv = 0.f;
+  if constexpr (FOLD) {
+    float oe = 0.f, ge = 0.f, sge = 0.f, ye = 0.f;
+    if (live) {
+      oe = w.o[p];
+      ge = a.de[(((int64_t)(n / a.C) * a.M + m) * a.C + n % a.C) * a.d + col];
+      sge = w.sg[p];
+      ye = w.y[p];
+    }
+    f32x4 ro[2][4], rg[2][4];
+#pragma unroll
+    for (int q = 0; q < 2; ++q) {
+      const int nq = min(2 * wave + q, a.N - 1);
+      const int64_t src = ((int64_t)nq * a.M + m) * a.d, dst = (((int64_t)(nq / a.C) * a.M + m) * a.C + nq % a.C) * a.d;
+#pragma unroll
+      for (int c = 0; c < 4; ++c) {
+        const int cc = c * 256 + lane * 4;
+        ro[q][c] = rg[q][c] = (f32x4){0.f, 0.f, 0.f, 0.f};
+        if (cc < a.d) {
+          ro[q][c] = *(const f32x4*)(w.o + src + cc);
+          rg[q][c] = *(const f32x4*)(a.de + dst + cc);
+        }
+      }
+    }
+    float inv[2], proj[2];
+    th_row_scalars(ro[0], rg[0], inv[0], proj[0]);
+    th_row_scalars(ro[1], rg[1], inv[1], proj[1]);
+    float dyv;
+    th_gate_bwd(ge, oe, proj[h], inv[h], sge, ye, dyv, dzv);
+    if (live) w.dyg[p] = dyv;
+  } else {
+    dzv = live ? w.dz[p] : 0.f;
+  }
   float dx = dzv;
   const bool gw2 = a.h.g_w2[m] != nullptr;
   float yb0[16], yb1[16];
@@ -416,6 +485,15 @@
   }
 }
 
+__global__ __launch_bounds__(TH_T) void th_bwd2_kernel(ThArgs a) {
+  extern __shared__ __attribute__((aligned(16))) unsigned char th_smem_raw[];
+  th_bwd2_block<false>(a, blockIdx.x, *(ThSmem*)th_smem_raw);
+}
+__global__ __launch_bounds__(TH_T) void th_bwd12_kernel(ThArgs a) {
+  extern __shared__ __attribute__((aligned(16))) unsigned char th_smem_raw[];
+  th_bwd2_block<true>(a, blockIdx.x, *(ThSmem*)th_smem_raw);
+}
+
 __global__ __launch_bounds__(TH_T) void th_bwd3_kernel(ThArgs a) {
   extern __shared__ __attribute__((aligned(16))) unsigned char th_smem_raw[];
   ThSmem& sm = *(ThSmem*)th_smem_raw;
@@ -503,7 +581,8 @@
   static bool done = false;
   if (done) return 0;
   const void* fns[] = {(const void*)th_fwd1_kernel, (const void*)th_fwd2_kernel, (const void*)th_bwd2_kernel,
-                       (const void*)th_bwd3_kernel, (const void*)th_fwd1_plan_kernel, (const void*)th_fwd2_cast_kernel};
+                       (const void*)th_bwd3_kernel, (const void*)th_fwd1_plan_kernel, (const void*)th_fwd2_cast_kernel,
+                       (const void*)th_bwd12_kernel};
   for (const void* f : fns) {
     hipError_t rc = hipFuncSetAttribute(f, hipFuncAttributeMaxDynamicSharedMemorySize, (int)sizeof(ThSmem));
     if (rc != hipSuccess) return (int)rc;
@@ -583,8 +662,12 @@
   a.de = dtext_embds; a.tw = text_weights; a.dtw = dtext_weights; a.dtext_moe = dtext_moe;
   const bool moe = text_weights && dtext_weights;
   const int gemm_blocks = M * (d / 32);
-  hipLaunchKernelGGL(th_bwd1_kernel, dim3((N * M + 3) / 4 + (moe ? N : 0)), dim3(256), 0, s, a);
-  hipLaunchKernelGGL(th_bwd2_kernel, dim3(gemm_blocks), dim3(TH_T), sizeof(ThSmem), s, a);
+  if (opts && opts->fold_bwd) {
+    hipLaunchKernelGGL(th_bwd12_kernel, dim3(gemm_blocks + (moe ? N : 0)), dim3(TH_T), sizeof(ThSmem), s, a);
+  } else {
+    hipLaunchKernelGGL(th_bwd1_kernel, dim3((N * M + 3) / 4 + (moe ? N : 0)), dim3(256), 0, s, a);
+    hipLaunchKernelGGL(th_bwd2_kernel, dim3(gemm_blocks), dim3(TH_T), sizeof(ThSmem), s, a);
+  }
   const int kb_n = (K + 4 * TH_T - 1) / (4 * TH_T);
   hipLaunchKernelGGL(th_bwd3_kernel, dim3(gemm_blocks + (moe ? M * kb_n : 0)), dim3(TH_T), sizeof(ThSmem), s, a);
   return (int)hipGetLastError();
diff --git a/mmt_amd/model.py b/mmt_amd/model.py
--- a/mmt_amd/model.py
+++ b/mmt_amd/model.py
@@ -75,17 +75,19 @@
 class _ReadoutFn(torch.autograd.Function):
 
   @staticmethod
-  def forward(ctx, last, agg_row, bm, compact=False, stash=None):
+  def forward(ctx, last, agg_row, bm, compact=False, stash=None, defer=False):
     ctx.compact = compact
     d = last.shape[1]
     out = torch.empty(bm, d, device=last.device, dtype=torch.float32)
     inv = torch.empty(bm, device=last.device, dtype=torch.float32)
-    check(_lib.lib().mmt_readout_fwd(ops._p(last), ops._p(agg_row), bm, d, ops._p(out), ops._p(inv), ops._stream()),
-          'mmt_readout_fwd')
+    if stash is not None:
+      stash.update(readout_inv=inv, readout_rows=None if compact else agg_row, readout_compact=compact,
+                   readout_out=out, readout_agg=agg_row, readout_pending=bool(defer))
+    if not defer:
+      check(_lib.lib().mmt_readout_fwd(ops._p(last), ops._p(agg_row), bm, d, ops._p(out), ops._p(inv), ops._stream()),
+            'mmt_readout_fwd')
     ctx.save_for_backward(out, inv, agg_row)
     ctx.shape = last.shape
-    if stash is not None:
-      stash.update(readout_inv=inv, readout_rows=None if compact else agg_row, readout_compact=compact)
     return out
 
   @staticmethod
@@ -94,7 +96,16 @@
     dlast = (torch.empty if ctx.compact else torch.zeros)(ctx.shape, device=out.device, dtype=torch.float32)
     check(_lib.lib().mmt_readout_bwd(ops._p(out), ops._p(inv), ops._p(dout.contiguous()), ops._p(agg_row),
                                      out.shape[0], out.shape[1], ops._p(dlast), ops._stream()), 'mmt_readout_bwd')
-    return dlast, None, None, None, None
+    return dlast, None, None, None, None, None
+
+
+def finish_readout(stash):
+  if stash is None or not stash.get('readout_pending'):
+    return
+  last, out = stash['last'], stash['readout_out']
+  check(_lib.lib().mmt_readout_fwd(ops._p(last), ops._p(stash['readout_agg']), out.shape[0], out.shape[1], ops._p(out),
+                                   ops._p(stash['readout_inv']), ops._stream()), 'mmt_readout_fwd')
+  stash['readout_pending'] = False
 
 
 class _SimsFn(torch.autograd.Function):
@@ -519,12 +530,14 @@
     batch.live_rows_hint = int(hint or 0) if self.pack_tokens else 0
     last = self.vid_bert.run_engine(batch, feats)
     self._stages = dict(plan=plan, feats=feats, batch=batch, last=last) if last.requires_grad else None
+    defer = bool(self.defer_readout and self._stages is not None and last.dtype == torch.float32 and last.is_contiguous() and
+                 _lib.lib().mmt_sims_readout_fast(bsz, bsz, len(mods), self.same_dim))
     if self.vid_bert.compact_output(batch, plan.rows_alloc):
       if plan.compact_rows is None:
         plan.compact_rows = torch.arange(bsz * len(mods), device=dev, dtype=torch.int32)
-      vid = _ReadoutFn.apply(last, plan.compact_rows, bsz * len(mods), True, self._stages)
+      vid = _ReadoutFn.apply(last, plan.compact_rows, bsz * len(mods), True, self._stages, defer)
     else:
-      vid = _ReadoutFn.apply(last, plan.agg_row, bsz * len(mods), False, self._stages)
+      vid = _ReadoutFn.apply(last, plan.agg_row, bsz * len(mods), False, self._stages, defer)
     vid = vid.view(bsz, len(mods), self.same_dim)
     if self._stages is not None:
       self._stages['vid_embds'] = vid
@@ -629,6 +642,8 @@
     return o
 
   _th_key = None
+  defer_readout = False
+  fold_text_heads_bwd = False
   _pending_front = None
   _th_front = None
   front_fuse = True
@@ -695,6 +710,7 @@
     bwd_opts = MmtTextHeadsOpts.from_buffer_copy(opts)
     bwd_opts.num_batches_tracked = None
     bwd_opts.video_front = None
+    bwd_opts.fold_bwd = int(bool(self.fold_text_heads_bwd) and caps == 1)
     check(L.mmt_text_heads_bwd(ctypes.byref(h), ops._p(text), ops._p(text_moe), ctypes.c_void_p(w1_all), n, caps, m, d, k,
                                int(self.txt_pro == 'gbn'), int(training), ops._p(self._th_ws[(n, text.device)]),
                                ops._p(de.contiguous()), ops._p(self._th_tw) if has_moe else None,
diff --git a/mmt_amd/train_step.py b/mmt_amd/train_step.py
--- a/mmt_amd/train_step.py
+++ b/mmt_amd/train_step.py
@@ -7,7 +7,7 @@
 from . import dist as mdist
 from . import _lib
 from .feature_store import RaggedFeatures
-from .model import cross_view_similarity
+from .model import cross_view_similarity, finish_readout
 from .optim import FlatAdam
 
 
@@ -63,6 +63,11 @@
       view = self.flat[o:o + n].view(v.dtype).view(v.shape)
       view.copy_(v)
       out[k] = view
+
+
+def _native_losses():
+  from .loss import InfoNceLoss, MaxMarginRankingLoss
+  return (MaxMarginRankingLoss, InfoNceLoss)
 
 
 def _clone_tree(src):
@@ -318,8 +323,15 @@
   def _forward(self):
     self._upload_branch_begin()
     mb = self.static
-    e = self.model(mb['token_ids'], mb['features'], mb.get('features_t'), mb.get('features_ind'),
-                   mb.get('features_avgpool'), mb.get('features_maxpool'), mb['query_masks'], out='embds')
+    head = (not self._multi and isinstance(self.loss_fn, _native_losses()) and hasattr(self.model, 'defer_readout'))
+    if head:
+      self.model.defer_readout = self.model.fold_text_heads_bwd = True
+    try:
+      e = self.model(mb['token_ids'], mb['features'], mb.get('features_t'), mb.get('features_ind'),
+                     mb.get('features_avgpool'), mb.get('features_maxpool'), mb['query_masks'], out='embds')
+    finally:
+      if head:
+        self.model.defer_readout = False
     self._pack_local(e)
     return e
 
@@ -362,6 +374,7 @@
       loss, outs, grads = fast
       torch.autograd.backward(outs, grads)
       return loss
+    finish_readout(getattr(self.model, '_stages', None))
     leaves = {k: v.detach().requires_grad_(e[k].requires_grad) for k, v in g.items()}
     sims = cross_view_similarity(leaves['vid_embds'], leaves['text_embds'], leaves['vid_weights'],
                                  leaves['text_weights'], 'avg')
@@ -392,10 +405,19 @@
     dev = vid.device
     sims = torch.empty(n, n, device=dev, dtype=torch.float32)
     dots = torch.empty(n, n, m, device=dev, dtype=torch.float32)
-    check(L.mmt_sims_fwd(ops._p(txt), ops._p(vid), ops._p(tw), ops._p(vw), n, n, m, d, ops._p(sims), ops._p(dots),
-                         ops._stream()), 'mmt_sims_fwd')
+    b = e['vid_embds'].shape[0]
+    st = getattr(self.model, '_stages', None)
+    if (st is not None and st.get('readout_pending') and st.get('vid_embds') is e['vid_embds'] and n == b and
+        vid.data_ptr() == st['readout_out'].data_ptr() and L.mmt_sims_readout_fast(n, n, m, d)):
+      check(L.mmt_sims_readout_fwd(ops._p(txt), ops._p(st['last']), ops._p(st['readout_agg']), ops._p(tw), ops._p(vw), n, n, m,
+                                   d, ops._p(vid), ops._p(st['readout_inv']), ops._p(sims), ops._p(dots), ops._stream()),
+            'mmt_sims_readout_fwd')
+      st['readout_pending'] = False
+    else:
+      finish_readout(st)
+      check(L.mmt_sims_fwd(ops._p(txt), ops._p(vid), ops._p(tw), ops._p(vw), n, n, m, d, ops._p(sims), ops._p(dots),
+                           ops._stream()), 'mmt_sims_fwd')
     loss = torch.empty((), device=dev, dtype=torch.float32)
-    b = e['vid_embds'].shape[0]
     sl = slice(self.rank * b, (self.rank + 1) * b)
     if 2 <= n <= L.mmt_simloss_small_max_n():
       kind = 0 if isinstance(self.loss_fn, MaxMarginRankingLoss) else 1
```
